# Shigangli/Ok-Topk

Measured on NVIDIA H100. Metric: train_samples_per_sec_vgg16_oktopk_density0.001, higher is better.
Workload: dtype fp32

## Files before the change

oktopk_b200/config.py:

```python
from __future__ import annotations

import dataclasses
from dataclasses import dataclass, field
from typing import Dict, Optional, Sequence


@dataclass
class OkTopkConfig:
    compressor: str = "oktopk"
    density: float = 0.01
    sparse: bool = True

    bucket_elems: int = 64 * 1024 * 1024

    warmup_iters: int = 0
    local_recompute_interval: int = 32
    global_recompute_interval: int = 32
    repartition_interval: int = 64
    topkaopt_recompute_interval: int = 32

    overselect_guard_num: int = 4
    overselect_guard_den: int = 3
    overselect_guard_factor: float = 1.03
    overselect_guard_loops: int = 5
    overselect_cap: float = 0.0
    overselect_cap_factor: float = 1.19
    overselect_cap_rungs: int = 40
    local_adapt_low: float = 2.0 / 3.0
    local_adapt_high: float = 5.0 / 4.0
    local_adapt_factor: float = 1.012
    global_adapt_low: float = 2.0 / 3.0
    global_adapt_high: float = 4.0 / 3.0
    global_adapt_inc: float = 1.008
    global_adapt_dec: float = 1.008

    throttle: int = 4
    balanced_allgather: bool = False
    dsa_dense_fallback_frac: float = 1.0 / 3.0

    gaussian_low: float = 3.0 / 4.0
    gaussian_high: float = 5.0 / 4.0
    gaussian_factor: float = 1.02
    gaussian_loops: int = 20
    gaussian_mode: str = "vgg"

    sigma_scale: float = 2.5
    norm_clip: Optional[float] = None
    dynamic_densities: Optional[Sequence[float]] = None

    backend: str = "auto"
    fused: bool = True
    deterministic: bool = False
    slot_factor: float = 0.0
    gather_factor: float = 0.0
    dense_switch_density: float = 0.05
    max_redo: int = 12
    redo_factor: float = 1.5
    land_grads: bool = True
    nvls: str = "auto"
    comm_ctas: int = 0
    pull_mode: str = "tma"
    overlap: bool = True
    gselect_mode: str = "auto"
    peer_timeout_s: float = 60.0

    def k_for(self, numel: int, density: Optional[float] = None) -> int:
        d = self.density if density is None else density
        return int(numel * d)

    def replace(self, **kw) -> "OkTopkConfig":
        return dataclasses.replace(self, **kw)

    def to_dict(self) -> Dict:
        return dataclasses.asdict(self)


@dataclass(frozen=True)
class LossScale:
    init_scale: float = 2.0 ** 16
    growth_factor: float = 2.0
    backoff_factor: float = 0.5
    growth_interval: int = 2000

    def __post_init__(self):
        if not (self.init_scale > 0 and self.growth_factor >= 1 and 0 < self.backoff_factor <= 1
                and self.growth_interval >= 1):
            raise ValueError("LossScale: need init_scale > 0, growth_factor >= 1, 0 < backoff_factor <= 1, "
                             "growth_interval >= 1")

    @staticmethod
    def parse(spec) -> Optional["LossScale"]:
        if spec is None or isinstance(spec, LossScale):
            return spec
        if isinstance(spec, str) and spec.strip().lower() == "dynamic":
            return LossScale()
        return LossScale(init_scale=float(spec), growth_factor=1.0, backoff_factor=1.0)


def _vgg() -> OkTopkConfig:
    return OkTopkConfig(
        density=0.02, warmup_iters=512,
        local_recompute_interval=32, global_recompute_interval=32, repartition_interval=64,
        overselect_guard_num=4, overselect_guard_den=3, overselect_guard_loops=5,
        local_adapt_low=2 / 3, local_adapt_high=5 / 4, local_adapt_factor=1.012,
        global_adapt_low=2 / 3, global_adapt_high=4 / 3, global_adapt_inc=1.008, global_adapt_dec=1.008,
        gaussian_mode="vgg", gaussian_factor=1.02, gaussian_loops=20,
        overselect_cap=2.0,
    )


def _lstm() -> OkTopkConfig:
    return OkTopkConfig(
        density=0.02, warmup_iters=128,
        local_recompute_interval=32, global_recompute_interval=32, repartition_interval=64,
        overselect_guard_num=3, overselect_guard_den=2, overselect_guard_loops=5,
        local_adapt_low=3 / 4, local_adapt_high=5 / 4, local_adapt_factor=1.012,
        global_adapt_low=3 / 4, global_adapt_high=5 / 4, global_adapt_inc=1.01, global_adapt_dec=1.008,
        gaussian_mode="lstm", gaussian_factor=1.012, gaussian_loops=50,
        overselect_cap=2.0,
    )


def _bert() -> OkTopkConfig:
    return OkTopkConfig(
        density=0.01, warmup_iters=0,
        local_recompute_interval=128, global_recompute_interval=128, repartition_interval=64,
        overselect_guard_loops=0,
        local_adapt_low=4 / 5, local_adapt_high=5 / 4, local_adapt_factor=1.025,
        global_adapt_low=4 / 5, global_adapt_high=5 / 4, global_adapt_inc=1.036, global_adapt_dec=1.025,
        balanced_allgather=True, sigma_scale=1.0,
        gaussian_mode="bert", gaussian_factor=1.012, gaussian_loops=20,
        overselect_cap=2.0,
    )


PRESETS = {
    "vgg16": _vgg, "vgg": _vgg, "cnn": _vgg,
    "lstm_an4": _lstm, "lstman4": _lstm, "lstm": _lstm,
    "bert_base": _bert, "bert": _bert,
}


def preset(name: str, **overrides) -> OkTopkConfig:
    if name not in PRESETS:
        raise KeyError("unknown preset %r (have %s)" % (name, sorted(PRESETS)))
    return PRESETS[name]().replace(**overrides)


def sigma_scale_for_density(density: float) -> float:
    if density > 0.7:
        return 0.5
    if density > 0.05:
        return 1.5
    if density > 0.01:
        return 2.0
    return 3.0
```

oktopk_b200/csrc/bindings.cpp:

```cpp
#include <pybind11/pybind11.h>
#include <pybind11/stl.h>
#include <cuda.h>
#include <cuda_runtime.h>

#include <unistd.h>

#include <algorithm>
#include <cstring>
#include <stdexcept>
#include <string>
#include <tuple>
#include <vector>

#include "oktopk.cuh"

namespace py = pybind11;
using namespace okt;

static void ck(cudaError_t e, const char* what) {
    if (e != cudaSuccess) throw std::runtime_error(std::string(what) + ": " + cudaGetErrorString(e));
}
template <class T> static T* P_(uint64_t p) { return reinterpret_cast<T*>(p); }
static cudaStream_t S_(uint64_t s) { return reinterpret_cast<cudaStream_t>(s); }

static py::tuple symm_alloc(size_t nbytes) {
    void* p = nullptr;
    ck(cudaMalloc(&p, nbytes), "cudaMalloc(symm)");
    ck(cudaMemset(p, 0, nbytes), "cudaMemset(symm)");
    cudaIpcMemHandle_t h;
    ck(cudaIpcGetMemHandle(&h, p), "cudaIpcGetMemHandle");
    return py::make_tuple((uint64_t)p, py::bytes(reinterpret_cast<const char*>(&h), sizeof(h)));
}
static uint64_t symm_open(const std::string& handle) {
    if (handle.size() != sizeof(cudaIpcMemHandle_t)) throw std::runtime_error("bad IPC handle size");
    cudaIpcMemHandle_t h;
    std::memcpy(&h, handle.data(), sizeof(h));
    void* p = nullptr;
    ck(cudaIpcOpenMemHandle(&p, h, cudaIpcMemLazyEnablePeerAccess), "cudaIpcOpenMemHandle");
    return (uint64_t)p;
}
static void symm_close(uint64_t p) { ck(cudaIpcCloseMemHandle(P_<void>(p)), "cudaIpcCloseMemHandle"); }
static void symm_free(uint64_t p) { ck(cudaFree(P_<void>(p)), "cudaFree(symm)"); }
static uint64_t dev_alloc_zero(size_t nbytes) {
    void* p = nullptr;
    ck(cudaMalloc(&p, nbytes), "cudaMalloc");
    ck(cudaMemset(p, 0, nbytes), "cudaMemset");
    return (uint64_t)p;
}
static void dev_free(uint64_t p) {
    if (p) ck(cudaFree(P_<void>(p)), "cudaFree");
}
static void memset_async(uint64_t p, int value, size_t nbytes, uint64_t stream) {
    ck(cudaMemsetAsync(P_<void>(p), value, nbytes, S_(stream)), "cudaMemsetAsync");
}
static int can_access_peer(int dev, int peer) {
    int ok = 0;
    ck(cudaDeviceCanAccessPeer(&ok, dev, peer), "cudaDeviceCanAccessPeer");
    return ok;
}


namespace drv {
template <class F> static F sym(const char* name) {
    void* fn = nullptr;
    cudaDriverEntryPointQueryResult q;
    cudaError_t e = cudaGetDriverEntryPoint(name, &fn, cudaEnableDefault, &q);
    if (e != cudaSuccess || fn == nullptr || q != cudaDriverEntryPointSuccess)
        throw std::runtime_error(std::string("driver entry point not available: ") + name);
    return reinterpret_cast<F>(fn);
}
static void ckd(CUresult r, const char* what) {
    if (r != CUDA_SUCCESS) throw std::runtime_error(std::string(what) + ": CUresult " + std::to_string((int)r));
}
}

static CUmemAllocationProp vmm_prop(int dev) {
    CUmemAllocationProp prop;
    std::memset(&prop, 0, sizeof(prop));
    prop.type = CU_MEM_ALLOCATION_TYPE_PINNED;
    prop.location.type = CU_MEM_LOCATION_TYPE_DEVICE;
    prop.location.id = dev;
    prop.requestedHandleTypes = CU_MEM_HANDLE_TYPE_POSIX_FILE_DESCRIPTOR;
    return prop;
}

static py::dict vmm_probe(int dev, int ndev) {
    py::dict d;
    d["vmm"] = 0; d["posix_fd"] = 0; d["multicast"] = 0; d["granularity"] = 0; d["mc_granularity"] = 0;
    try {
        auto getattr_ = drv::sym<CUresult (*)(int*, CUdevice_attribute, CUdevice)>("cuDeviceGetAttribute");
        int v = 0;
        if (getattr_(&v, CU_DEVICE_ATTRIBUTE_VIRTUAL_MEMORY_MANAGEMENT_SUPPORTED, dev) == CUDA_SUCCESS) d["vmm"] = v;
        if (getattr_(&v, CU_DEVICE_ATTRIBUTE_HANDLE_TYPE_POSIX_FILE_DESCRIPTOR_SUPPORTED, dev) == CUDA_SUCCESS) d["posix_fd"] = v;
        if (getattr_(&v, CU_DEVICE_ATTRIBUTE_MULTICAST_SUPPORTED, dev) == CUDA_SUCCESS) d["multicast"] = v;
        auto gran = drv::sym<CUresult (*)(size_t*, const CUmemAllocationProp*, CUmemAllocationGranularity_flags)>("cuMemGetAllocationGranularity");
        CUmemAllocationProp prop = vmm_prop(dev);
        size_t g = 0;
        if (gran(&g, &prop, CU_MEM_ALLOC_GRANULARITY_RECOMMENDED) == CUDA_SUCCESS) d["granularity"] = g;
        if (d["multicast"].cast<int>() && ndev > 1) {
            auto mgran = drv::sym<CUresult (*)(size_t*, const CUmulticastObjectProp*, CUmulticastGranularity_flags)>("cuMulticastGetGranularity");
            CUmulticastObjectProp mp;
            std::memset(&mp, 0, sizeof(mp));
            mp.numDevices = ndev; mp.size = 1 << 21; mp.handleTypes = CU_MEM_HANDLE_TYPE_POSIX_FILE_DESCRIPTOR;
            size_t mg = 0;
            if (mgran(&mg, &mp, CU_MULTICAST_GRANULARITY_RECOMMENDED) == CUDA_SUCCESS) d["mc_granularity"] = mg;
        }
    } catch (const std::exception& e) {
        d["error"] = std::string(e.what());
    }
    return d;
}

static py::tuple vmm_create(size_t nbytes, int dev) {
    auto create = drv::sym<CUresult (*)(CUmemGenericAllocationHandle*, size_t, const CUmemAllocationProp*, unsigned long long)>("cuMemCreate");
    auto exp = drv::sym<CUresult (*)(void*, CUmemGenericAllocationHandle, CUmemAllocationHandleType, unsigned long long)>("cuMemExportToShareableHandle");
    CUmemAllocationProp prop = vmm_prop(dev);
    CUmemGenericAllocationHandle h = 0;
    drv::ckd(create(&h, nbytes, &prop, 0), "cuMemCreate");
    int fd = -1;
    drv::ckd(exp(&fd, h, CU_MEM_HANDLE_TYPE_POSIX_FILE_DESCRIPTOR, 0), "cuMemExportToShareableHandle");
    return py::make_tuple((uint64_t)h, fd);
}
static uint64_t vmm_import(int fd) {
    auto imp = drv::sym<CUresult (*)(CUmemGenericAllocationHandle*, void*, CUmemAllocationHandleType)>("cuMemImportFromShareableHandle");
    CUmemGenericAllocationHandle h = 0;
    drv::ckd(imp(&h, reinterpret_cast<void*>(static_cast<uintptr_t>(fd)), CU_MEM_HANDLE_TYPE_POSIX_FILE_DESCRIPTOR), "cuMemImportFromShareableHandle");
    return (uint64_t)h;
}
static uint64_t vmm_map(uint64_t handle, size_t nbytes, int dev, size_t align) {
    auto reserve = drv::sym<CUresult (*)(CUdeviceptr*, size_t, size_t, CUdeviceptr, unsigned long long)>("cuMemAddressReserve");
    auto map = drv::sym<CUresult (*)(CUdeviceptr, size_t, size_t, CUmemGenericAllocationHandle, unsigned long long)>("cuMemMap");
    auto access = drv::sym<CUresult (*)(CUdeviceptr, size_t, const CUmemAccessDesc*, size_t)>("cuMemSetAccess");
    CUdeviceptr va = 0;
    drv::ckd(reserve(&va, nbytes, align, 0, 0), "cuMemAddressReserve");
    drv::ckd(map(va, nbytes, 0, (CUmemGenericAllocationHandle)handle, 0), "cuMemMap");
    CUmemAccessDesc ad;
    std::memset(&ad, 0, sizeof(ad));
    ad.location.type = CU_MEM_LOCATION_TYPE_DEVICE;
    ad.location.id = dev;
    ad.flags = CU_MEM_ACCESS_FLAGS_PROT_READWRITE;
    drv::ckd(access(va, nbytes, &ad, 1), "cuMemSetAccess");
    return (uint64_t)va;
}
static void vmm_unmap(uint64_t va, size_t nbytes) {
    auto unmap = drv::sym<CUresult (*)(CUdeviceptr, size_t)>("cuMemUnmap");
    auto afree = drv::sym<CUresult (*)(CUdeviceptr, size_t)>("cuMemAddressFree");
    unmap((CUdeviceptr)va, nbytes);
    afree((CUdeviceptr)va, nbytes);
}
static void vmm_release(uint64_t handle) {
    auto rel = drv::sym<CUresult (*)(CUmemGenericAllocationHandle)>("cuMemRelease");
    rel((CUmemGenericAllocationHandle)handle);
}
static py::tuple mc_create(size_t nbytes, int ndev) {
    auto create = drv::sym<CUresult (*)(CUmemGenericAllocationHandle*, const CUmulticastObjectProp*)>("cuMulticastCreate");
    auto exp = drv::sym<CUresult (*)(void*, CUmemGenericAllocationHandle, CUmemAllocationHandleType, unsigned long long)>("cuMemExportToShareableHandle");
    CUmulticastObjectProp mp;
    std::memset(&mp, 0, sizeof(mp));
    mp.numDevices = ndev; mp.size = nbytes; mp.handleTypes = CU_MEM_HANDLE_TYPE_POSIX_FILE_DESCRIPTOR;
    CUmemGenericAllocationHandle h = 0;
    drv::ckd(create(&h, &mp), "cuMulticastCreate");
    int fd = -1;
    drv::ckd(exp(&fd, h, CU_MEM_HANDLE_TYPE_POSIX_FILE_DESCRIPTOR, 0), "cuMemExportToShareableHandle(mc)");
    return py::make_tuple((uint64_t)h, fd);
}
static void mc_add_device(uint64_t mc, int dev) {
    auto add = drv::sym<CUresult (*)(CUmemGenericAllocationHandle, CUdevice)>("cuMulticastAddDevice");
    drv::ckd(add((CUmemGenericAllocationHandle)mc, dev), "cuMulticastAddDevice");
}
static void mc_bind(uint64_t mc, uint64_t mem, size_t nbytes) {
    auto bind = drv::sym<CUresult (*)(CUmemGenericAllocationHandle, size_t, CUmemGenericAllocationHandle, size_t, size_t, unsigned long long)>("cuMulticastBindMem");
    drv::ckd(bind((CUmemGenericAllocationHandle)mc, 0, (CUmemGenericAllocationHandle)mem, 0, nbytes, 0), "cuMulticastBindMem");
}

static size_t state_bytes() { return sizeof(OktState); }

static py::dict layout_info(int P, int n, int cap, int gcap) {
    SymmLayout L = make_layout(P, n, cap, gcap);
    py::dict d;
    d["total"] = L.total; d["rs_mbox"] = L.rs_mbox; d["rs_thr"] = L.rs_thr; d["ag_mbox"] = L.ag_mbox;
    d["cut_mbox"] = L.cut_mbox; d["cut_data"] = L.cut_data; d["send_idx"] = L.send_idx; d["send_val"] = L.send_val;
    d["gat_idx"] = L.gat_idx; d["gat_val"] = L.gat_val; d["cap"] = L.cap; d["gcap"] = L.gcap; d["scap"] = L.scap;
    d["done_mbox"] = L.done_mbox; d["tree_mbox"] = L.tree_mbox; d["scale_mbox"] = L.scale_mbox;
    d["chunk"] = kChunk; d["maxp"] = OKT_MAXP; d["threads"] = kThreads;
    return d;
}

static py::dict read_state(uint64_t st, int P, uint64_t stream) {
    static thread_local std::vector<char> host(offsetof(OktState, hist));
    ck(cudaMemcpyAsync(host.data(), P_<void>(st), host.size(), cudaMemcpyDeviceToHost, S_(stream)), "read_state");
    ck(cudaStreamSynchronize(S_(stream)), "read_state sync");
    const OktState* s = reinterpret_cast<const OktState*>(host.data());
    py::dict d;
    d["local_thr"] = s->local_thr; d["local_thr_used"] = s->local_thr_used; d["global_thr"] = s->global_thr;
    d["epoch"] = s->epoch;
    std::vector<int> e(s->edges, s->edges + P + 1);
    d["edges"] = e;
    d["local_count"] = s->stat_local_count; d["global_count"] = s->stat_global_count;
    d["recv_total"] = s->stat_recv_total; d["gather_total"] = s->stat_gather_total;
    d["overflow_send"] = s->stat_overflow_send; d["overflow_gather"] = s->stat_overflow_gather;
    d["redo"] = s->stat_redo; d["dense_fallback"] = s->stat_dense_fallback; d["pack_thr"] = s->pack_thr;
    d["cum_overflow_send"] = s->cum_overflow_send; d["cum_overflow_gather"] = s->cum_overflow_gather;
    d["cum_redo"] = s->cum_redo;
    d["fault"] = s->fault;
    auto us = [&](int a, int b) { return s->t_phase[b] >= s->t_phase[a] ? (double)(s->t_phase[b] - s->t_phase[a]) * 1e-3 : 0.0; };
    py::dict ph;
    ph["local"] = us(5, 0); ph["pack"] = us(0, 1); ph["wait_rs"] = us(1, 6); ph["reduce"] = us(6, 2); ph["gselect"] = us(2, 3);
    ph["wait_ag"] = us(3, 7); ph["final"] = us(7, 4); ph["total"] = us(5, 4);
    d["phase_us"] = ph;
    return d;
}

static py::list read_trace(uint64_t st, uint64_t stream) {
    std::vector<TraceRec> host(kTraceLen);
    ck(cudaMemcpyAsync(host.data(), reinterpret_cast<char*>(P_<OktState>(st)) + offsetof(OktState, trace),
                       sizeof(TraceRec) * kTraceLen, cudaMemcpyDeviceToHost, S_(stream)), "read_trace");
    ck(cudaStreamSynchronize(S_(stream)), "read_trace sync");
    py::list out;
    for (const TraceRec& t : host) {
        if (t.epoch == 0) continue;
        py::dict d;
        d["epoch"] = t.epoch; d["local_count"] = t.local_count; d["global_count"] = t.global_count;
        d["recv_total"] = t.recv_total; d["gather_total"] = t.gather_total; d["overflow_send"] = t.overflow_send;
        d["overflow_gather"] = t.overflow_gather; d["redo"] = t.redo; d["local_thr"] = t.local_thr;
        d["global_thr"] = t.global_thr; d["us_local"] = t.us_local; d["us_pack"] = t.us_pack;
        d["us_wait_rs"] = t.us_wait_rs; d["us_reduce"] = t.us_reduce; d["us_gselect"] = t.us_gselect;
        d["us_wait_ag"] = t.us_wait_ag; d["us_final"] = t.us_final; d["t_begin"] = t.t_begin;
        out.append(d);
    }
    return out;
}

static py::tuple host_flag_alloc() {
    int* h = nullptr;
    ck(cudaHostAlloc(reinterpret_cast<void**>(&h), sizeof(int) * 16, cudaHostAllocMapped), "cudaHostAlloc(flag)");
    for (int i = 0; i < 16; ++i) h[i] = 0;
    void* d = nullptr;
    ck(cudaHostGetDevicePointer(&d, h, 0), "cudaHostGetDevicePointer");
    return py::make_tuple((uint64_t)h, (uint64_t)d);
}
static void host_flag_free(uint64_t h) { if (h) cudaFreeHost(P_<void>(h)); }
static int host_flag_read(uint64_t h) { return h ? *reinterpret_cast<volatile int*>(h) : 0; }
static void host_flag_clear(uint64_t h) { if (h) *reinterpret_cast<volatile int*>(h) = 0; }

static void write_state(uint64_t st, float local_thr, float global_thr, const std::vector<int>& edges, uint64_t stream) {
    std::vector<char> host(offsetof(OktState, hist));
    ck(cudaMemcpyAsync(host.data(), P_<void>(st), host.size(), cudaMemcpyDeviceToHost, S_(stream)), "write_state rd");
    ck(cudaStreamSynchronize(S_(stream)), "write_state sync");
    OktState* s = reinterpret_cast<OktState*>(host.data());
    s->local_thr = local_thr;
    s->global_thr = global_thr;
    if (!edges.empty()) {
        if (edges.size() > OKT_MAXP + 1) throw std::runtime_error("too many region edges");
        for (size_t i = 0; i < edges.size(); ++i) s->edges[i] = edges[i];
    }
    ck(cudaMemcpyAsync(P_<void>(st), host.data(), host.size(), cudaMemcpyHostToDevice, S_(stream)), "write_state wr");
    ck(cudaStreamSynchronize(S_(stream)), "write_state sync2");
}

static void fill_peers(char** dst, const std::vector<uint64_t>& peers) {
    if (peers.size() > OKT_MAXP) throw std::runtime_error("world larger than OKT_MAXP");
    for (int i = 0; i < OKT_MAXP; ++i) dst[i] = nullptr;
    for (size_t i = 0; i < peers.size(); ++i) dst[i] = P_<char>(peers[i]);
}

static void oktopk_run(uint64_t g, uint64_t res, uint64_t st, const std::vector<uint64_t>& peers, int n, int rank,
                       int k, int cap, int gcap, py::dict o, int grid, uint64_t stream) {
    OktParams p;
    std::memset(&p, 0, sizeof(p));
    p.g = P_<float>(g); p.res = P_<float>(res); p.st = P_<OktState>(st);
    if (!o.contains("cand") || !o.contains("ccap")) throw std::runtime_error("oktopk_run: candidate scratch missing");
    p.cand = P_<int>(o["cand"].cast<uint64_t>()); p.ccap = o["ccap"].cast<int>();
    p.cand_mode = o.contains("cand_mode") ? o["cand_mode"].cast<int>() : 1;
    fill_peers(p.peers, peers);
    p.P = (int)peers.size(); p.rank = rank; p.n = n; p.k = k;
    p.L = make_layout(p.P, n, cap, gcap);
    auto geti = [&](const char* key, int dflt) { return o.contains(key) ? o[key].cast<int>() : dflt; };
    auto getf = [&](const char* key, double dflt) { return o.contains(key) ? o[key].cast<double>() : dflt; };
    for (int i = 0; i < OKT_MAXP; ++i) p.peer_g[i] = nullptr;
    if (o.contains("peer_g")) {
        auto pg = o["peer_g"].cast<std::vector<uint64_t>>();
        for (size_t i = 0; i < pg.size() && i < OKT_MAXP; ++i) p.peer_g[i] = P_<float>(pg[i]);
    }
    p.max_redo = geti("max_redo", 12);
    p.redo_factor = (float)getf("redo_factor", 1.5);
    p.dense_nnz_limit = geti("dense_nnz_limit", 0);
    p.host_fault = o.contains("host_fault") ? P_<int>(o["host_fault"].cast<uint64_t>()) : nullptr;
    p.skip = o.contains("skip") ? P_<const int>(o["skip"].cast<uint64_t>()) : nullptr;
    p.trace = geti("trace", 0);
    p.exact_local = geti("exact_local", 0);
    p.repartition = geti("repartition", 0);
    p.uniform_regions = geti("uniform_regions", 0);
    p.residual_mode = geti("residual_mode", RES_OKTOPK);
    p.global_mode = geti("global_mode", GLB_THRESHOLD);
    p.deterministic = geti("deterministic", 0);
    p.pull_tma = geti("pull_tma", 1);
    p.phase_begin = geti("phase_begin", 0);
    p.phase_end = geti("phase_end", PH_END);
    p.guard_loops = geti("guard_loops", 0);
    if (p.guard_loops > kGuardFineMax) p.guard_loops = kGuardFineMax;
    p.cap_limit = geti("cap_limit", 0);
    p.cap_rungs = geti("cap_rungs", 40);
    p.cap_factor = (float)getf("cap_factor", 1.19);
    p.guard_limit = geti("guard_limit", 0);
    p.guard_factor = (float)getf("guard_factor", 1.03);
    p.l_low_cnt = getf("l_low_cnt", 0.0); p.l_high_cnt = getf("l_high_cnt", 1e30);
    p.l_factor = (float)getf("l_factor", 1.012);
    p.g_low_cnt = getf("g_low_cnt", 0.0); p.g_high_cnt = getf("g_high_cnt", 1e30);
    p.g_inc = (float)getf("g_inc", 1.008); p.g_dec = (float)getf("g_dec", 1.008);
    p.prefilter = (float)getf("prefilter", 0.8);
    p.timeout_ns = (unsigned long long)(getf("timeout_s", 0.0) * 1e9);
    if (o.contains("srcs")) {
        auto t = o["srcs"].cast<std::tuple<std::vector<uint64_t>, std::vector<long long>, std::vector<long long>>>();
        const auto& ptr = std::get<0>(t);
        const auto& off = std::get<1>(t);
        const auto& len = std::get<2>(t);
        if (off.size() != ptr.size() || len.size() != ptr.size()) throw std::runtime_error("oktopk_run: srcs table size mismatch");
        if (ptr.size() > (size_t)kSrcSegMax) throw std::runtime_error("oktopk_run: more gradient sources than kSrcSegMax");
        long long end = 0;
        for (size_t i = 0; i < ptr.size(); ++i) {
            if (off[i] < end || (off[i] & 3) || len[i] <= 0 || off[i] + len[i] > n || (ptr[i] & 15))
                throw std::runtime_error("oktopk_run: gradient sources must be 16-byte aligned, in bucket order, "
                                         "non-overlapping, at offsets that are multiples of 4 elements");
            p.src[i] = P_<const float>(ptr[i]);
            p.src_off[i] = (int)off[i];
            p.src_len[i] = (int)len[i];
            end = off[i] + len[i];
        }
        p.nsrc = (int)ptr.size();
        p.zero_g = 0;
    } else {
        if (g & 15) throw std::runtime_error("oktopk_run: the bucket must be 16-byte aligned");
        p.src[0] = P_<const float>(g);
        p.src_off[0] = 0;
        p.src_len[0] = n;
        p.nsrc = 1;
        p.zero_g = 1;
    }
    if (geti("split_phases", 0)) {
        for (int ph = p.phase_begin; ph < p.phase_end; ++ph) {
            OktParams q = p;
            q.phase_begin = ph; q.phase_end = ph + 1;
            ck(launch_oktopk(q, grid, S_(stream)), "oktopk phase launch");
        }
    } else {
        ck(launch_oktopk(p, grid, S_(stream)), "oktopk fused launch");
    }
}

static void gather_run(uint64_t g, uint64_t res, uint64_t st, const std::vector<uint64_t>& peers, int n, int rank,
                       int k, int cap, int gcap, py::dict o, int grid, uint64_t stream) {
    GatherParams p;
    std::memset(&p, 0, sizeof(p));
    p.g = P_<float>(g); p.res = P_<float>(res); p.st = P_<OktState>(st);
    fill_peers(p.peers, peers);
    p.P = (int)peers.size(); p.rank = rank; p.n = n; p.k = k;
    p.L = make_layout(p.P, n, cap, gcap);
    p.reselect = o.contains("reselect") ? o["reselect"].cast<int>() : 0;
    p.clip_max_norm = o.contains("clip_max_norm") ? (float)o["clip_max_norm"].cast<double>() : 0.f;
    p.bitmap = o.contains("bitmap") ? P_<unsigned>(o["bitmap"].cast<uint64_t>()) : nullptr;
    p.cand = o.contains("cand") ? P_<int>(o["cand"].cast<uint64_t>()) : nullptr;
    p.ccap = o.contains("ccap") ? o["ccap"].cast<int>() : 0;
    p.host_fault = o.contains("host_fault") ? P_<int>(o["host_fault"].cast<uint64_t>()) : nullptr;
    p.skip = o.contains("skip") ? P_<const int>(o["skip"].cast<uint64_t>()) : nullptr;
    if (p.reselect && (p.bitmap == nullptr || p.cand == nullptr || p.ccap <= 0))
        throw std::runtime_error("gather_run: TopkA2 needs the bitmap and candidate scratch");
    p.select_mode = o["select_mode"].cast<int>();
    p.exact_now = o.contains("exact_now") ? o["exact_now"].cast<int>() : 0;
    p.gauss_mode = o.contains("gauss_mode") ? o["gauss_mode"].cast<int>() : 0;
    p.gauss_loops = o.contains("gauss_loops") ? o["gauss_loops"].cast<int>() : 20;
    p.gauss_factor = o.contains("gauss_factor") ? (float)o["gauss_factor"].cast<double>() : 1.02f;
    p.density = (float)o["density"].cast<double>();
    p.pull_tma = o.contains("pull_tma") ? o["pull_tma"].cast<int>() : 1;
    p.timeout_ns = o.contains("timeout_s") ? (unsigned long long)(o["timeout_s"].cast<double>() * 1e9) : 0ULL;
    ck(launch_gather_scheme(p, grid, S_(stream)), "gather scheme launch");
}

static void gtopk_run(uint64_t g, uint64_t res, uint64_t st, const std::vector<uint64_t>& peers, int n, int rank,
                      int k, int cap, int gcap, py::dict o, int grid, uint64_t stream) {
    TreeParams p;
    std::memset(&p, 0, sizeof(p));
    p.g = P_<float>(g); p.res = P_<float>(res); p.st = P_<OktState>(st);
    fill_peers(p.peers, peers);
    p.P = (int)peers.size(); p.rank = rank; p.n = n; p.k = k;
    if (p.P & (p.P - 1)) throw std::runtime_error("gTopk needs a power-of-two world size (VGG/allreducer.py:113)");
    p.L = make_layout(p.P, n, cap, gcap);
    p.pull_tma = o.contains("pull_tma") ? o["pull_tma"].cast<int>() : 1;
    p.timeout_ns = o.contains("timeout_s") ? (unsigned long long)(o["timeout_s"].cast<double>() * 1e9) : 0ULL;
    p.clip_max_norm = o.contains("clip_max_norm") ? (float)o["clip_max_norm"].cast<double>() : 0.f;
    p.bitmap = P_<unsigned>(o["bitmap"].cast<uint64_t>());
    p.cand = P_<int>(o["cand"].cast<uint64_t>());
    p.ccap = o["ccap"].cast<int>();
    p.sel_idx = P_<int>(o["sel_idx"].cast<uint64_t>());
    p.sel_val = P_<float>(o["sel_val"].cast<uint64_t>());
    p.selcap = o["selcap"].cast<int>();
    p.host_fault = o.contains("host_fault") ? P_<int>(o["host_fault"].cast<uint64_t>()) : nullptr;
    p.skip = o.contains("skip") ? P_<const int>(o["skip"].cast<uint64_t>()) : nullptr;
    ck(launch_gtopk(p, grid, S_(stream)), "gtopk launch");
}

static void land_grads(const std::vector<uint64_t>& srcs, const std::vector<long long>& offs, const std::vector<int>& numels,
                       uint64_t bucket, uint64_t stream) {
    const size_t T = srcs.size();
    if (offs.size() != T || numels.size() != T) throw std::runtime_error("land_grads: table size mismatch");
    constexpr int per = 8192;
    for (size_t b = 0; b < T; b += kLandMax) {
        LandParams lp;
        std::memset(&lp, 0, sizeof(lp));
        const int cnt = (int)std::min<size_t>(kLandMax, T - b);
        int blk = 0;
        for (int i = 0; i < cnt; ++i) {
            lp.src[i] = P_<const float>(srcs[b + i]);
            lp.dst_off[i] = offs[b + i];
            lp.numel[i] = numels[b + i];
            lp.blk_begin[i] = blk;
            blk += std::max(1, (numels[b + i] + per - 1) / per);
        }
        lp.blk_begin[cnt] = blk;
        lp.count = cnt;
        ck(launch_land(lp, P_<float>(bucket), S_(stream)), "land_grads");
    }
}

static void dense_run(const std::vector<uint64_t>& bufs, const std::vector<uint64_t>& flags, uint64_t epoch, int n,
                      int rank, int grid, uint64_t stream, uint64_t st, double timeout_s, uint64_t mc,
                      uint64_t host_fault, uint64_t skip) {
    DenseParams p;
    std::memset(&p, 0, sizeof(p));
    if (bufs.size() > OKT_MAXP || bufs.size() != flags.size()) throw std::runtime_error("bad peer tables");
    for (size_t i = 0; i < bufs.size(); ++i) { p.bufs[i] = P_<float>(bufs[i]); p.flags[i] = P_<uint64_t>(flags[i]); }
    p.epoch = P_<unsigned long long>(epoch);
    p.n = n; p.P = (int)bufs.size(); p.rank = rank; p.scale = 1.0f / (float)p.P;
    p.fault = st ? &P_<OktState>(st)->fault : nullptr;
    p.timeout_ns = (unsigned long long)(timeout_s * 1e9);
    p.mc = P_<float>(mc);
    p.host_fault = P_<int>(host_fault);
    p.skip = P_<const int>(skip);
    ck(launch_dense_allreduce(p, grid, S_(stream)), "dense allreduce launch");
}

static void kth_abs(uint64_t x, int n, int k, uint64_t st, uint64_t out, int grid, uint64_t stream) {
    ck(launch_kth_abs(P_<float>(x), n, k, P_<OktState>(st), P_<float>(out), grid, S_(stream)), "kth_abs launch");
}

static void fused_sgd(uint64_t p, uint64_t g, uint64_t mom, int n, double momentum, double dampening, double wd,
                      int nesterov, int first, int zero_grad, uint64_t stream, uint64_t scal_ptr, uint64_t fault_ptr,
                      uint64_t skip_ptr) {
    if (scal_ptr == 0) throw std::runtime_error("fused_sgd: scal_ptr must point at the group's device scalars");
    ck(launch_fused_sgd(P_<float>(p), P_<float>(g), P_<float>(mom), n, (float)momentum, (float)dampening, (float)wd,
                        nesterov, first, zero_grad, P_<float>(scal_ptr), P_<int>(fault_ptr), P_<int>(skip_ptr),
                        S_(stream)),
       "fused_sgd");
}
static void fused_bert_adam(uint64_t p, uint64_t g, uint64_t m, uint64_t v, int n, double b1, double b2, double eps,
                            double wd, int zero_grad, uint64_t stream, uint64_t scal_ptr, uint64_t fault_ptr,
                            uint64_t skip_ptr) {
    if (scal_ptr == 0) throw std::runtime_error("fused_bert_adam: scal_ptr must point at the group's device scalars");
    ck(launch_fused_bert_adam(P_<float>(p), P_<float>(g), P_<float>(m), P_<float>(v), n, (float)b1, (float)b2,
                              (float)eps, (float)wd, zero_grad, P_<float>(scal_ptr), P_<int>(fault_ptr), P_<int>(skip_ptr),
                              S_(stream)),
       "fused_bert_adam");
}
static void fused_adam(uint64_t p, uint64_t g, uint64_t m, uint64_t v, int n, double beta1, double beta2, double eps,
                       double wd, int decoupled, int zero_grad, uint64_t stream, uint64_t scal_ptr, uint64_t fault_ptr,
                       uint64_t skip_ptr) {
    if (scal_ptr == 0) throw std::runtime_error("fused_adam: scal_ptr must point at the group's device scalars");
    ck(launch_fused_adam(P_<float>(p), P_<float>(g), P_<float>(m), P_<float>(v), n, beta1, beta2, (float)eps, (float)wd,
                         decoupled, zero_grad, P_<float>(scal_ptr), P_<int>(fault_ptr), P_<int>(skip_ptr), S_(stream)),
       "fused_adam");
}
static BnDtype bn_dtype(int dtype, const char* what) {
    if (dtype < 0 || dtype > 2) throw std::runtime_error(std::string(what) + ": dtype must be 0 (fp32), 1 (bf16) or 2 (fp16)");
    return static_cast<BnDtype>(dtype);
}
static void bn_forward(uint64_t x, uint64_t y, uint64_t arg, uint64_t partial, uint64_t gamma, uint64_t beta, uint64_t cbias,
                       uint64_t save_mean, uint64_t save_invstd, uint64_t rmean, uint64_t rvar, uint64_t nbt, double momentum,
                       double eps, int relu, int M, int C, int W, int slot, int max_ctas, uint64_t stream, int dtype,
                       uint64_t res) {
    if (C % 4 != 0) throw std::runtime_error("bn_forward: channel count must be a multiple of 4");
    if (slot < 0) throw std::runtime_error("bn_forward: negative slot");
    if (res != 0 && (W != 0 || !relu)) throw std::runtime_error("bn_forward: a residual needs relu = 1 and no pool");
    ck(launch_bn_forward(P_<const void>(x), P_<void>(y), P_<unsigned char>(arg), P_<float>(partial), P_<const float>(gamma),
                         P_<const float>(beta), P_<const float>(cbias), P_<float>(save_mean), P_<float>(save_invstd),
                         P_<float>(rmean), P_<float>(rvar), P_<long long>(nbt), (float)momentum, (float)eps, relu, M, C, W, slot,
                         max_ctas, bn_dtype(dtype, "bn_forward"), S_(stream), P_<const void>(res)), "bn_forward");
}
static void bn_backward(uint64_t x, uint64_t dy, uint64_t arg, uint64_t dx, uint64_t partial, uint64_t gamma, uint64_t beta,
                        uint64_t save_mean, uint64_t save_invstd, uint64_t dgamma, uint64_t dbeta, int relu, int M, int C, int W,
                        int slot, int max_ctas, uint64_t stream, int dtype, uint64_t res, uint64_t dres) {
    if (slot < 0) throw std::runtime_error("bn_backward: negative slot");
    if ((res == 0) != (dres == 0)) throw std::runtime_error("bn_backward: res and dres go together");
    if (res != 0 && (W != 0 || !relu)) throw std::runtime_error("bn_backward: a residual needs relu = 1 and no pool");
    ck(launch_bn_backward(P_<const void>(x), P_<const void>(dy), P_<const unsigned char>(arg), P_<void>(dx), P_<float>(partial),
                          P_<const float>(gamma), P_<const float>(beta), P_<const float>(save_mean), P_<const float>(save_invstd),
                          P_<float>(dgamma), P_<float>(dbeta), relu, M, C, W, slot, max_ctas, bn_dtype(dtype, "bn_backward"),
                          S_(stream), P_<const void>(res), P_<void>(dres)), "bn_backward");
}
static void ln_check(const char* what, int R, int H, long long p_keep_thr, uint64_t seed, uint64_t mean, uint64_t rstd,
                     std::initializer_list<uint64_t> vec_ptrs) {
    if (R <= 0 || !ln_supported_h(H)) throw std::runtime_error(std::string(what) + ": needs R > 0 and H in 128, 256, ..., 1024");
    if (p_keep_thr < 0 || p_keep_thr > (1LL << 32)) throw std::runtime_error(std::string(what) + ": p_keep_thr out of range");
    if (p_keep_thr < (1LL << 32) && seed == 0) throw std::runtime_error(std::string(what) + ": dropout needs the seed");
    if (mean == 0 || rstd == 0) throw std::runtime_error(std::string(what) + ": mean and rstd are needed");
    for (uint64_t p : vec_ptrs)
        if (p == 0 || (p & 15)) throw std::runtime_error(std::string(what) + ": tensors must be non-null and 16-byte aligned");
}
static void ln_forward(uint64_t x, uint64_t a, uint64_t y, uint64_t gamma, uint64_t beta, uint64_t mean, uint64_t rstd,
                       uint64_t seed, int R, int H, long long p_keep_thr, double scale, double eps, int a_dtype,
                       uint64_t stream) {
    ln_check("ln_forward", R, H, p_keep_thr, seed, mean, rstd, {x, a, y, gamma, beta});
    ck(launch_ln_forward(P_<const float>(x), P_<const void>(a), P_<float>(y), P_<const float>(gamma), P_<const float>(beta),
                         P_<float>(mean), P_<float>(rstd), P_<const unsigned long long>(seed), R, H, p_keep_thr, (float)scale,
                         (float)eps, bn_dtype(a_dtype, "ln_forward"), S_(stream)), "ln_forward");
}
static void ln_backward(uint64_t x, uint64_t a, uint64_t dy, uint64_t gamma, uint64_t mean, uint64_t rstd, uint64_t seed,
                        uint64_t dx, uint64_t da, uint64_t partial, uint64_t dgamma, uint64_t dbeta, int R, int H,
                        long long p_keep_thr, double scale, int a_dtype, uint64_t stream) {
    ln_check("ln_backward", R, H, p_keep_thr, seed, mean, rstd, {x, a, dy, gamma, dx, da, partial, dgamma, dbeta});
    ck(launch_ln_backward(P_<const float>(x), P_<const void>(a), P_<const float>(dy), P_<const float>(gamma),
                          P_<const float>(mean), P_<const float>(rstd), P_<const unsigned long long>(seed), P_<float>(dx),
                          P_<void>(da), P_<float>(partial), P_<float>(dgamma), P_<float>(dbeta), R, H, p_keep_thr,
                          (float)scale, bn_dtype(a_dtype, "ln_backward"), S_(stream)), "ln_backward");
}
static void xent_check(const char* what, int R, long long V, std::initializer_list<uint64_t> ptrs, uint64_t x, uint64_t t) {
    if (R <= 0 || V <= 0) throw std::runtime_error(std::string(what) + ": needs R > 0 and V > 0");
    for (uint64_t p : ptrs)
        if (p == 0) throw std::runtime_error(std::string(what) + ": null pointer");
    if ((x & 15) || (t & 7)) throw std::runtime_error(std::string(what) + ": logits must be 16-byte aligned, targets 8-byte");
}
static void xent_forward(uint64_t x, uint64_t t, uint64_t lse, uint64_t rowloss, uint64_t loss, int R, long long V,
                         long long ignore_index, int dtype, uint64_t stream) {
    xent_check("xent_forward", R, V, {x, t, lse, rowloss, loss}, x, t);
    ck(launch_xent_forward(P_<const void>(x), P_<const long long>(t), P_<float>(lse), P_<float>(rowloss), P_<float>(loss),
                           R, V, ignore_index, bn_dtype(dtype, "xent_forward"), S_(stream)), "xent_forward");
}
static void xent_backward(uint64_t x, uint64_t t, uint64_t lse, uint64_t g, uint64_t dx, int R, long long V,
                          long long ignore_index, int dtype, uint64_t stream) {
    xent_check("xent_backward", R, V, {x, t, lse, g, dx}, x, t);
    if (dx & 15) throw std::runtime_error("xent_backward: the gradient must be 16-byte aligned");
    ck(launch_xent_backward(P_<const void>(x), P_<const long long>(t), P_<const float>(lse), P_<const float>(g), P_<void>(dx),
                            R, V, ignore_index, bn_dtype(dtype, "xent_backward"), S_(stream)), "xent_backward");
}
static void mlm_select(uint64_t labels, uint64_t rows, uint64_t tgt, uint64_t slot, uint64_t count, uint64_t overflow,
                       int R, int M, long long ignore_index, uint64_t stream) {
    if (R <= 0 || M <= 0) throw std::runtime_error("mlm_select: needs R > 0 and M > 0");
    if (!labels || !rows || !tgt || !slot || !count) throw std::runtime_error("mlm_select: null pointer");
    if ((labels & 7) || (tgt & 7) || (count & 7) || (overflow & 7) || (rows & 3) || (slot & 3))
        throw std::runtime_error("mlm_select: misaligned pointer");
    ck(launch_mlm_select(P_<const long long>(labels), R, ignore_index, M, P_<int>(rows), P_<long long>(tgt),
                         P_<int>(slot), P_<long long>(count), P_<long long>(overflow), S_(stream)), "mlm_select");
}
static void mlm_copy_check(const char* what, int nrows, int H, uint64_t src, uint64_t idx, uint64_t dst, BnDtype dt) {
    if (nrows <= 0 || H <= 0) throw std::runtime_error(std::string(what) + ": needs rows > 0 and H > 0");
    if (!src || !idx || !dst) throw std::runtime_error(std::string(what) + ": null pointer");
    const uint64_t mask = dt == BnDtype::kF32 ? 3 : 1;
    if ((src & mask) || (dst & mask) || (idx & 3)) throw std::runtime_error(std::string(what) + ": misaligned pointer");
}
static void mlm_gather(uint64_t x, uint64_t rows, uint64_t out, int M, int H, int dtype, uint64_t stream) {
    const BnDtype dt = bn_dtype(dtype, "mlm_gather");
    mlm_copy_check("mlm_gather", M, H, x, rows, out, dt);
    ck(launch_mlm_gather(P_<const void>(x), P_<const int>(rows), P_<void>(out), M, H, dt, S_(stream)), "mlm_gather");
}
static void mlm_scatter(uint64_t dout, uint64_t slot, uint64_t dx, int R, int H, int dtype, uint64_t stream) {
    const BnDtype dt = bn_dtype(dtype, "mlm_scatter");
    mlm_copy_check("mlm_scatter", R, H, dout, slot, dx, dt);
    ck(launch_mlm_scatter(P_<const void>(dout), P_<const int>(slot), P_<void>(dx), R, H, dt, S_(stream)), "mlm_scatter");
}
static void lstm_check(const char* what, int T, int N, int H, int u, int rows, BnDtype dtype,
                       std::initializer_list<uint64_t> ptrs, std::initializer_list<uint64_t> vec_ptrs) {
    if (T <= 0 || N <= 0 || H <= 0 || H % 4 || u <= 0 || rows <= 0 || rows > N)
        throw std::runtime_error(std::string(what) + ": needs T, N > 0, H > 0 a multiple of 4, u > 0 and 0 < rows <= N");
    for (uint64_t p : ptrs)
        if (p == 0) throw std::runtime_error(std::string(what) + ": null pointer");
    const uint64_t mask = dtype == BnDtype::kF32 ? 15 : 7;
    for (uint64_t p : vec_ptrs)
        if (p & mask)
            throw std::runtime_error(std::string(what) + ": W_hh and the staged operand must be " +
                                     std::to_string(mask + 1) + "-byte aligned");
}
static void lstm_forward(uint64_t gx, uint64_t whh, uint64_t len, uint64_t y, uint64_t gates, uint64_t cs, uint64_t bar,
                         int T, int N, int H, int u, int rows, uint64_t stream, int dtype) {
    const BnDtype dt = bn_dtype(dtype, "lstm_forward");
    lstm_check("lstm_forward", T, N, H, u, rows, dt, {gx, whh, len, y, gates, cs, bar}, {whh, y});
    ck(launch_lstm_forward(P_<const void>(gx), P_<const void>(whh), P_<const int>(len), P_<void>(y), P_<float>(gates),
                           P_<float>(cs), P_<unsigned long long>(bar), T, N, H, u, rows, S_(stream), dt), "lstm_forward");
}
static void lstm_backward(uint64_t dy, uint64_t gates, uint64_t cs, uint64_t whh, uint64_t len, uint64_t dg, uint64_t bar,
                          int T, int N, int H, int u, int rows, uint64_t stream, int dtype) {
    const BnDtype dt = bn_dtype(dtype, "lstm_backward");
    lstm_check("lstm_backward", T, N, H, u, rows, dt, {dy, gates, cs, whh, len, dg, bar}, {dg});
    ck(launch_lstm_backward(P_<const void>(dy), P_<const float>(gates), P_<const float>(cs), P_<const void>(whh),
                            P_<const int>(len), P_<void>(dg), P_<unsigned long long>(bar), T, N, H, u, rows, S_(stream), dt),
       "lstm_backward");
}
static void maxpool2_fwd(uint64_t x, uint64_t y, uint64_t arg, int N, int H, int W, int C, uint64_t stream) {
    if ((C % 4) || (H % 2) || (W % 2)) throw std::runtime_error("maxpool2_fwd: needs C % 4 == 0 and even H, W");
    ck(launch_maxpool2_fwd(P_<const float>(x), P_<float>(y), P_<unsigned char>(arg), N, H, W, C, S_(stream)), "maxpool2_fwd");
}
static void maxpool2_bwd(uint64_t dy, uint64_t arg, uint64_t dx, int N, int H, int W, int C, uint64_t stream) {
    ck(launch_maxpool2_bwd(P_<const float>(dy), P_<const unsigned char>(arg), P_<float>(dx), N, H, W, C, S_(stream)), "maxpool2_bwd");
}
static void momentum_correct(uint64_t g, uint64_t buf, int n, double momentum, uint64_t stream) {
    ck(launch_momentum_correct(P_<float>(g), P_<float>(buf), n, (float)momentum, S_(stream)), "momentum_correct");
}
static void clip_by_norm(uint64_t x, int n, uint64_t scratch, double max_norm, uint64_t stream) {
    ck(launch_l2norm_sq(P_<float>(x), n, P_<float>(scratch), S_(stream)), "l2norm");
    ck(launch_scale(P_<float>(x), n, P_<float>(scratch), (float)max_norm, S_(stream)), "clip scale");
}

static void unscale_check(const std::vector<uint64_t>& srcs, const std::vector<long long>& lens, uint64_t ls, uint64_t sync,
                          uint64_t st, uint64_t host_fault, const std::vector<uint64_t>& peers, size_t mbox_off, int rank,
                          double timeout_s, uint64_t stream) {
    ScaleParams p;
    std::memset(&p, 0, sizeof(p));
    if (srcs.empty() || srcs.size() != lens.size()) throw std::runtime_error("unscale_check: bad source table");
    if (srcs.size() > (size_t)kSrcSegMax) throw std::runtime_error("unscale_check: more gradient sources than kSrcSegMax");
    if (peers.size() > OKT_MAXP) throw std::runtime_error("world larger than OKT_MAXP");
    int blk = 0;
    for (size_t i = 0; i < srcs.size(); ++i) {
        if ((srcs[i] & 15) || lens[i] <= 0 || lens[i] > (1LL << 31) - 1)
            throw std::runtime_error("unscale_check: sources must be 16-byte aligned and non-empty");
        p.src[i] = P_<float>(srcs[i]);
        p.len[i] = (int)lens[i];
        p.blk_begin[i] = blk;
        blk += (int)((lens[i] + kScalePerCta - 1) / kScalePerCta);
    }
    p.blk_begin[srcs.size()] = blk;
    p.nseg = (int)srcs.size();
    p.ls = P_<LossScaleDev>(ls);
    p.sync = P_<ScaleSync>(sync);
    p.fault = &P_<OktState>(st)->fault;
    p.host_fault = P_<int>(host_fault);
    for (size_t i = 0; i < peers.size(); ++i) p.peers[i] = P_<char>(peers[i]);
    p.mbox_off = mbox_off;
    p.P = (int)peers.size(); p.rank = rank;
    p.timeout_ns = (unsigned long long)(timeout_s * 1e9);
    ck(launch_unscale_check(p, S_(stream)), "unscale_check");
}

PYBIND11_MODULE(_C, m) {
    m.doc() = "oktopk_b200 native extension (sm_90a kernels + symmetric peer memory)";
    m.def("symm_alloc", &symm_alloc);
    m.def("symm_open", &symm_open);
    m.def("symm_close", &symm_close);
    m.def("symm_free", &symm_free);
    m.def("dev_alloc_zero", &dev_alloc_zero);
    m.def("dev_free", &dev_free);
    m.def("memset_async", &memset_async);
    m.def("can_access_peer", &can_access_peer);
    m.def("state_bytes", &state_bytes);
    m.def("layout_info", &layout_info);
    m.def("read_state", &read_state);
    m.def("write_state", &write_state);
    m.def("max_coop_grid", &okt_max_coop_grid);
    m.def("oktopk_run", &oktopk_run);
    m.def("gather_run", &gather_run);
    m.def("dense_run", &dense_run, py::arg("bufs"), py::arg("flags"), py::arg("epoch"), py::arg("n"), py::arg("rank"),
          py::arg("grid"), py::arg("stream"), py::arg("st") = 0, py::arg("timeout_s") = 0.0, py::arg("mc") = 0,
          py::arg("host_fault") = 0, py::arg("skip") = 0);
    m.def("gtopk_run", &gtopk_run);
    m.def("land_grads", &land_grads);
    m.def("read_trace", &read_trace);
    m.def("host_flag_alloc", &host_flag_alloc);
    m.def("host_flag_free", &host_flag_free);
    m.def("host_flag_read", &host_flag_read);
    m.def("host_flag_clear", &host_flag_clear);
    m.def("fault_ptr", [](uint64_t st) { return (uint64_t)&P_<OktState>(st)->fault; });
    m.def("gather_max_coop_grid", &gather_max_coop_grid);
    m.def("gtopk_max_coop_grid", &gtopk_max_coop_grid);
    m.def("vmm_probe", &vmm_probe);
    m.def("vmm_create", &vmm_create);
    m.def("vmm_import", &vmm_import);
    m.def("vmm_map", &vmm_map);
    m.def("vmm_unmap", &vmm_unmap);
    m.def("vmm_release", &vmm_release);
    m.def("mc_create", &mc_create);
    m.def("mc_add_device", &mc_add_device);
    m.def("mc_bind", &mc_bind);
    m.def("close_fd", [](int fd) { if (fd >= 0) ::close(fd); });
    m.def("clear_fault", [](uint64_t st, uint64_t stream) {
        ck(cudaMemsetAsync(&P_<OktState>(st)->fault, 0, sizeof(int), S_(stream)), "clear_fault");
    });
    m.def("kth_abs", &kth_abs);
    m.def("fused_sgd", &fused_sgd, py::arg("p"), py::arg("g"), py::arg("mom"), py::arg("n"), py::arg("momentum"),
          py::arg("dampening"), py::arg("wd"), py::arg("nesterov"), py::arg("first"), py::arg("zero_grad"),
          py::arg("stream"), py::arg("scal_ptr"), py::arg("fault_ptr") = 0, py::arg("skip_ptr") = 0);
    m.def("fused_bert_adam", &fused_bert_adam, py::arg("p"), py::arg("g"), py::arg("m"), py::arg("v"), py::arg("n"),
          py::arg("b1"), py::arg("b2"), py::arg("eps"), py::arg("wd"), py::arg("zero_grad"), py::arg("stream"),
          py::arg("scal_ptr"), py::arg("fault_ptr") = 0, py::arg("skip_ptr") = 0);
    m.def("fused_adam", &fused_adam, py::arg("p"), py::arg("g"), py::arg("m"), py::arg("v"), py::arg("n"),
          py::arg("beta1"), py::arg("beta2"), py::arg("eps"), py::arg("wd"), py::arg("decoupled"), py::arg("zero_grad"),
          py::arg("stream"), py::arg("scal_ptr"), py::arg("fault_ptr") = 0, py::arg("skip_ptr") = 0);
    m.def("momentum_correct", &momentum_correct);
    m.def("unscale_check", &unscale_check);
    m.def("scale_update", [](uint64_t ls, double growth, double backoff, int interval, uint64_t stream) {
        ck(launch_scale_update(P_<LossScaleDev>(ls), growth, backoff, interval, S_(stream)), "scale_update");
    });
    m.def("adam_scalars", [](uint64_t ls, uint64_t hyper, uint64_t scal, int groups, uint64_t stream) {
        ck(launch_adam_scalars(P_<const LossScaleDev>(ls), P_<const double>(hyper), P_<float>(scal), groups, S_(stream)),
           "adam_scalars");
    });
    m.def("carry_residual", [](uint64_t g, uint64_t res, int n, uint64_t skip, uint64_t stream) {
        ck(launch_carry_residual(P_<float>(g), P_<float>(res), n, P_<const int>(skip), S_(stream)), "carry_residual");
    });
    m.attr("LOSS_SCALE_BYTES") = sizeof(LossScaleDev);
    m.attr("SCALE_SYNC_BYTES") = sizeof(ScaleSync);
    m.attr("VERDICT_OFFSET") = offsetof(ScaleSync, verdict);
    m.def("maxpool2_fwd", &maxpool2_fwd);
    m.def("maxpool2_bwd", &maxpool2_bwd);
    m.def("bn_forward", &bn_forward, py::arg("x"), py::arg("y"), py::arg("arg"), py::arg("partial"), py::arg("gamma"),
          py::arg("beta"), py::arg("cbias"), py::arg("save_mean"), py::arg("save_invstd"), py::arg("rmean"), py::arg("rvar"),
          py::arg("nbt"), py::arg("momentum"), py::arg("eps"), py::arg("relu"), py::arg("M"), py::arg("C"), py::arg("W"),
          py::arg("slot"), py::arg("max_ctas"), py::arg("stream"), py::arg("dtype"), py::arg("res") = 0);
    m.def("bn_backward", &bn_backward, py::arg("x"), py::arg("dy"), py::arg("arg"), py::arg("dx"), py::arg("partial"),
          py::arg("gamma"), py::arg("beta"), py::arg("save_mean"), py::arg("save_invstd"), py::arg("dgamma"), py::arg("dbeta"),
          py::arg("relu"), py::arg("M"), py::arg("C"), py::arg("W"), py::arg("slot"), py::arg("max_ctas"), py::arg("stream"),
          py::arg("dtype"), py::arg("res") = 0, py::arg("dres") = 0);
    m.def("bn_tile_rows", &bn_tile_rows);
    m.def("bn_sliced", &bn_sliced, py::arg("M"), py::arg("C"), py::arg("W"));
    m.def("ln_forward", &ln_forward, py::arg("x"), py::arg("a"), py::arg("y"), py::arg("gamma"), py::arg("beta"),
          py::arg("mean"), py::arg("rstd"), py::arg("seed"), py::arg("R"), py::arg("H"), py::arg("p_keep_thr"),
          py::arg("scale"), py::arg("eps"), py::arg("a_dtype"), py::arg("stream"));
    m.def("ln_backward", &ln_backward, py::arg("x"), py::arg("a"), py::arg("dy"), py::arg("gamma"), py::arg("mean"),
          py::arg("rstd"), py::arg("seed"), py::arg("dx"), py::arg("da"), py::arg("partial"), py::arg("dgamma"),
          py::arg("dbeta"), py::arg("R"), py::arg("H"), py::arg("p_keep_thr"), py::arg("scale"), py::arg("a_dtype"),
          py::arg("stream"));
    m.def("ln_bwd_grid", &ln_bwd_grid);
    m.def("ln_supported_h", &ln_supported_h);
    m.def("xent_forward", &xent_forward, py::arg("x"), py::arg("t"), py::arg("lse"), py::arg("rowloss"), py::arg("loss"),
          py::arg("R"), py::arg("V"), py::arg("ignore_index"), py::arg("dtype"), py::arg("stream"));
    m.def("xent_backward", &xent_backward, py::arg("x"), py::arg("t"), py::arg("lse"), py::arg("g"), py::arg("dx"),
          py::arg("R"), py::arg("V"), py::arg("ignore_index"), py::arg("dtype"), py::arg("stream"));
    m.def("mlm_select", &mlm_select, py::arg("labels"), py::arg("rows"), py::arg("tgt"), py::arg("slot"), py::arg("count"),
          py::arg("overflow"), py::arg("R"), py::arg("M"), py::arg("ignore_index"), py::arg("stream"));
    m.def("mlm_gather", &mlm_gather, py::arg("x"), py::arg("rows"), py::arg("out"), py::arg("M"), py::arg("H"),
          py::arg("dtype"), py::arg("stream"));
    m.def("mlm_scatter", &mlm_scatter, py::arg("dout"), py::arg("slot"), py::arg("dx"), py::arg("R"), py::arg("H"),
          py::arg("dtype"), py::arg("stream"));
    m.def("lstm_forward", &lstm_forward, py::arg("gx"), py::arg("whh"), py::arg("len"), py::arg("y"), py::arg("gates"),
          py::arg("cs"), py::arg("bar"), py::arg("T"), py::arg("N"), py::arg("H"), py::arg("u"), py::arg("rows"),
          py::arg("stream"), py::arg("dtype") = 0);
    m.def("lstm_backward", &lstm_backward, py::arg("dy"), py::arg("gates"), py::arg("cs"), py::arg("whh"), py::arg("len"),
          py::arg("dg"), py::arg("bar"), py::arg("T"), py::arg("N"), py::arg("H"), py::arg("u"), py::arg("rows"),
          py::arg("stream"), py::arg("dtype") = 0);
    m.def("clip_by_norm", &clip_by_norm);
    m.attr("MAXP") = OKT_MAXP;
    m.attr("TRACE_LEN") = kTraceLen;
    m.attr("LAND_MAX") = kLandMax;
    m.attr("SRC_SEG_MAX") = kSrcSegMax;
    m.attr("CHUNK") = kChunk;
}
```

oktopk_b200/csrc/oktopk.cu:

```cuda
#include "devlib.cuh"

namespace okt {

__device__ __forceinline__ int region_of(const int* s_edges, int P, int i) {
    int d = 0;
#pragma unroll 1
    for (int r = 1; r < P; ++r) d += (i >= s_edges[r]) ? 1 : 0;
    return d;
}

struct SrcSeg { const float* src; int off, len; };

__device__ __forceinline__ int seg_find(const SrcSeg* s, int ns, int e) {
    int lo = 0, hi = ns - 1, r = -1;
    while (lo <= hi) {
        const int mid = (lo + hi) >> 1;
        if (s[mid].off <= e) { r = mid; lo = mid + 1; } else { hi = mid - 1; }
    }
    return r;
}

__device__ __forceinline__ float grad_at(const SrcSeg* s, int ns, int i) {
    const int q = seg_find(s, ns, i);
    return (q >= 0 && i - s[q].off < s[q].len) ? s[q].src[i - s[q].off] : 0.f;
}

__device__ __forceinline__ float4 grad4_at(const SrcSeg* s, int ns, int v) {
    float4 out = make_float4(0.f, 0.f, 0.f, 0.f);
    const int q = seg_find(s, ns, 4 * v);
    if (q < 0) return out;
    const int r = 4 * v - s[q].off, len = s[q].len;
    const float* src = s[q].src + r;
    if (r + 4 <= len) return ld_stream_f4(reinterpret_cast<const float4*>(src));
    if (r < len) out.x = src[0];
    if (r + 1 < len) out.y = src[1];
    if (r + 2 < len) out.z = src[2];
    return out;
}

__global__ void __launch_bounds__(kThreads, kCtasPerSm) oktopk_fused_kernel(const OktParams p) {
    __shared__ uint32_t s_hist[kHistBins];
    __shared__ int s_w[kWarps + 1];
    __shared__ int s_edges[OKT_MAXP + 1];
    __shared__ int s_cnt[OKT_MAXP];
    __shared__ float s_thr[OKT_MAXP];
    __shared__ int s_misc[OKT_MAXP * 2 + 4];
    __shared__ int s_soff[OKT_MAXP + 1];
    __shared__ float s_lthr[kGuardMax];
    __shared__ int s_lcnt[kGuardMax];
    __shared__ ChunkSrc s_srcs[OKT_MAXP];
    __shared__ float s_sthr[OKT_MAXP];
    __shared__ Seg s_segs[OKT_MAXP];
    __shared__ __align__(128) PullSmem s_pull;
    __shared__ __align__(8) uint64_t s_pk_bar[kPackStages];
    __shared__ __align__(8) uint64_t s_pk_empty[kPackStages];
    __shared__ __align__(8) uint64_t s_sc_bar[kScanStages];
    __shared__ SrcSeg s_src[kSrcSegMax];
    __shared__ int s_tail_v[kSrcSegMax], s_tail_q[kSrcSegMax];
    __shared__ int s_ntail;
    extern __shared__ __align__(128) float4 dyn_pk[];

    if (verdict_set(p.skip)) return;
    OktState* st = p.st;
    const int tid = threadIdx.x, lane = tid & 31, warp = tid >> 5;
    const int gtid = blockIdx.x * kThreads + tid;
    const int gthreads = gridDim.x * kThreads;
    const int P = p.P, rank = p.rank, n = p.n;
    char* me = p.peers[rank];
    const uint32_t epoch = st->epoch + 1u;
    const int par = epoch & 1u;
    const float thr_in = st->local_thr;
    const bool exact_local = p.exact_local || thr_in == 0.f;
    const bool two_pass = exact_local || p.repartition;
    uint32_t pipe_it = 0;

    for (int b = tid; b < kHistBins; b += kThreads) s_hist[b] = 0;
    if (blockIdx.x == 0 && tid == 0) st->t_phase[5] = globaltimer_ns();
    const SpinGuard sg_rs{&st->fault, p.timeout_ns, FAULT_RS_TIMEOUT, p.host_fault};
    const SpinGuard sg_ag{&st->fault, p.timeout_ns, FAULT_AG_TIMEOUT, p.host_fault};
    const SpinGuard sg_cut{&st->fault, p.timeout_ns, FAULT_CUT_TIMEOUT, p.host_fault};
    const SpinGuard sg_done{&st->fault, p.timeout_ns, FAULT_DONE_TIMEOUT, p.host_fault};
    if (tid == 0) {
        mbar_init(&s_pull.bar[0], 1);
        mbar_init(&s_pull.bar[1], 1);
        for (int q = 0; q < kPackStages; ++q) { mbar_init(&s_pk_bar[q], 1); mbar_init(&s_pk_empty[q], kWarps); }
        for (int q = 0; q < kScanStages; ++q) mbar_init(&s_sc_bar[q], 1);
        mbar_fence_init();
    }
    const int n4 = n >> 2;
    const int nsrc = p.nsrc;
    for (int q = tid; q < nsrc; q += kThreads) s_src[q] = SrcSeg{p.src[q], p.src_off[q], p.src_len[q]};
    if (warp == 0) {
        int cnt = 0;
        for (int q0 = 0; q0 < nsrc; q0 += 32) {
            const int q = q0 + lane;
            const int end = q < nsrc ? p.src_off[q] + p.src_len[q] : 0;
            const bool part = q < nsrc && (end & 3) != 0 && (end >> 2) < n4;
            const unsigned m = __ballot_sync(0xffffffffu, part);
            if (part) { const int t = cnt + __popc(m & ((1u << lane) - 1u)); s_tail_v[t] = end >> 2; s_tail_q[t] = q; }
            cnt += __popc(m);
        }
        if (lane == 0) s_ntail = cnt;
    }
    __syncthreads();
    const int ntail = s_ntail;

    float4* g4 = reinterpret_cast<float4*>(p.g);
    float4* r4 = reinterpret_cast<float4*>(p.res);

    if (p.phase_begin <= PH_LOCAL && PH_LOCAL < p.phase_end && two_pass) {
        const float thr0 = thr_in;
        const LadderCfg lcl = ladder_cfg(p, !exact_local);
        ladder_build(s_lthr, s_lcnt, lcl, thr0);

        auto visit = [&](float x) {
            if (exact_local) {
                hist_add(s_hist, x, 0, 0u);
            } else {
                float ax = fabsf(x);
                if (ax > thr0) atomicAdd(&s_lcnt[ladder_rung(s_lthr, lcl.n_total, ax)], 1);
            }
        };
        const float cut = (exact_local && thr0 > 0.f) ? thr0 * p.prefilter : -1.f;
        const bool prefilter = cut > 0.f;
        constexpr int kLocTile = 4;
        for (int base = blockIdx.x * kThreads * kLocTile; base < n4; base += gridDim.x * kThreads * kLocTile) {
            float4 a[kLocTile], r[kLocTile];
            bool in[kLocTile];
#pragma unroll
            for (int u = 0; u < kLocTile; ++u) {
                const int v = base + u * kThreads + tid;
                in[u] = v < n4;
                if (in[u]) { a[u] = grad4_at(s_src, nsrc, v); r[u] = ld_stream_f4(r4 + v); }
                else { a[u] = make_float4(0.f, 0.f, 0.f, 0.f); r[u] = a[u]; }
            }
#pragma unroll
            for (int u = 0; u < kLocTile; ++u) {
                const int v = base + u * kThreads + tid;
                a[u].x += r[u].x; a[u].y += r[u].y; a[u].z += r[u].z; a[u].w += r[u].w;
                if (in[u]) st_stream_f4(r4 + v, a[u]);
                const float xs[4] = {a[u].x, a[u].y, a[u].z, a[u].w};
                if (!prefilter) {
                    if (in[u]) { visit(xs[0]); visit(xs[1]); visit(xs[2]); visit(xs[3]); }
                    continue;
                }
                unsigned bits = 0u;
                int tot = 0;
#pragma unroll
                for (int c = 0; c < 4; ++c) {
                    const bool pd = in[u] && fabsf(xs[c]) > cut;
                    if (pd) bits |= 1u << c;
                    tot += __popc(__ballot_sync(0xffffffffu, pd));
                }
                if (tot == 0) continue;
                int run = 0;
                if (lane == 0) run = atomicAdd(&st->cand_cursor, tot);
                run = __shfl_sync(0xffffffffu, run, 0);
#pragma unroll
                for (int c = 0; c < 4; ++c) {
                    const bool pd = (bits >> c) & 1u;
                    const unsigned m = __ballot_sync(0xffffffffu, pd);
                    if (pd) {
                        const int pos = run + __popc(m & ((1u << lane) - 1u));
                        if (pos < p.ccap) p.cand[pos] = 4 * v + c;
                    }
                    run += __popc(m);
                }
            }
        }
        if (blockIdx.x == 0) {
            for (int i = n4 * 4 + tid; i < n; i += kThreads) {
                float a = grad_at(s_src, nsrc, i) + p.res[i];
                p.res[i] = a;
                if (prefilter) {
                    if (fabsf(a) > cut) { int pos = atomicAdd(&st->cand_cursor, 1); if (pos < p.ccap) p.cand[pos] = i; }
                } else {
                    visit(a);
                }
            }
        }
        if (exact_local) {
            float thr;
            bool done = false;
            if (prefilter) {
                grid_sync(&st->bar);
                const int ncand = *reinterpret_cast<volatile int*>(&st->cand_cursor);
                if (ncand >= p.k && ncand <= p.ccap) {
                    Seg seg{p.res, ncand, p.cand};
                    thr = grid_kth_abs(&seg, 1, false, (uint32_t)p.k, st, s_hist, s_w, 0);
                    done = true;
                }
            }
            if (!done) {
                if (!prefilter) hist_flush(st, s_hist);
                Seg seg{p.res, n, nullptr};
                thr = grid_kth_abs(&seg, 1, false, (uint32_t)p.k, st, s_hist, s_w, prefilter ? 0 : 1);
            }
            if (blockIdx.x == 0 && tid == 0) { st->local_thr_used = thr; st->cand_cursor = 0; }
        } else {
            ladder_flush(st, s_lcnt);
            grid_sync(&st->bar);
            if (blockIdx.x == 0 && tid == 0) {
                int cnt;
                st->local_thr_used = ladder_pick(st, lcl, thr0, p.guard_limit, p.cap_limit, &cnt);
            }
        }
        grid_sync(&st->bar);

        if (p.repartition) {
            const float thr = st->local_thr_used;
            const int W = gridDim.x * kWarps;
            const int Lw = (((n + W - 1) / W) + 31) / 32 * 32;
            {
                const int gw = blockIdx.x * kWarps + warp;
                const long long lo = (long long)gw * Lw;
                const long long hi = min((long long)n, lo + Lw);
                int cnt = 0;
                for (long long base = lo; base < hi; base += 32) {
                    long long i = base + lane;
                    float x = (i < hi) ? __ldcg(p.res + i) : 0.f;
                    cnt += __popc(__ballot_sync(0xffffffffu, fabsf(x) > thr));
                }
                if (lane == 0) st->wcounts[gw] = cnt;
            }
            grid_sync(&st->bar);
            if (blockIdx.x == 0) {
                const int per = (W + kThreads - 1) / kThreads;
                int mysum = 0;
                for (int j = 0; j < per; ++j) {
                    int w = tid * per + j;
                    if (w < W) mysum += st->wcounts[w];
                }
                int M;
                int excl = block_excl_scan(mysum, s_w, &M);
                const int chunkM = M / P;
                if (M > 0) {
                    for (int j = 1; j < P; ++j) {
                        int target = chunkM * j;
                        if (excl <= target && target < excl + mysum) {
                            int run = excl;
                            for (int q = 0; q < per; ++q) {
                                int w = tid * per + q;
                                int c = (w < W) ? st->wcounts[w] : 0;
                                if (target < run + c) { s_misc[2 * j] = w; s_misc[2 * j + 1] = target - run; break; }
                                run += c;
                            }
                        }
                    }
                }
                __syncthreads();
                if (warp >= 1 && warp < P) {
                    const int j = warp;
                    int cut;
                    if (M > 0) {
                        const int gw = s_misc[2 * j];
                        int want = s_misc[2 * j + 1];
                        const long long lo = (long long)gw * Lw;
                        const long long hi = min((long long)n, lo + Lw);
                        cut = (int)lo;
                        for (long long base = lo; base < hi; base += 32) {
                            long long i = base + lane;
                            float x = (i < hi) ? __ldcg(p.res + i) : 0.f;
                            unsigned m = __ballot_sync(0xffffffffu, fabsf(x) > thr);
                            int c = __popc(m);
                            if (want < c) { cut = (int)base + (int)__fns(m, 0, want + 1); break; }
                            want -= c;
                        }
                    } else {
                        cut = (n / P) * j;
                    }
                    if (lane == 0) st->cuts[j - 1] = cut;
                }
                __syncthreads();
                if (tid < P) {
                    int* dst = cut_data(p.peers[tid], p.L, par, rank);
                    for (int j = 0; j < P - 1; ++j) st_relaxed_sys_u32(reinterpret_cast<uint32_t*>(dst + j), (uint32_t)st->cuts[j]);
                    st_release_sys_u64(cut_mbox(p.peers[tid], p.L, par, rank), make_mail(epoch, 1u));
                }
                if (tid < P) wait_mailbox(cut_mbox(me, p.L, par, tid), epoch, sg_cut);
                __syncthreads();
                if (tid < P - 1) {
                    long long sum = 0;
                    for (int s = 0; s < P; ++s)
                        sum += (long long)ld_relaxed_sys_u32(reinterpret_cast<uint32_t*>(cut_data(me, p.L, par, s) + tid));
                    s_misc[tid] = (int)(sum / P);
                }
                __syncthreads();
                if (tid == 0) {
                    int prev = 0;
                    st->edges[0] = 0;
                    for (int j = 0; j < P - 1; ++j) {
                        int c = s_misc[j];
                        c = max(prev, min(c, n));
                        st->edges[j + 1] = c;
                        prev = c;
                    }
                    st->edges[P] = n;
                }
            }
            grid_sync(&st->bar);
        }
    }

    if (tid <= P) s_edges[tid] = st->edges[tid];
    __syncthreads();
    if (tid <= P) s_soff[tid] = (tid < P) ? slot_off(p.L, s_edges, tid) : (p.L.cap > 0 ? P * p.L.cap : slot_off(p.L, s_edges, P));
    __syncthreads();
    int* const my_sidx = send_idx_base(me, p.L);
    float* const my_sval = send_val_base(me, p.L);
    auto stamp = [&](int slot) { if (blockIdx.x == 0 && tid == 0) st->t_phase[slot] = globaltimer_ns(); };
    stamp(0);

    if (p.phase_begin <= PH_PACK && PH_PACK < p.phase_end) {
        float thr_sel = two_pass ? st->local_thr_used : thr_in;
        const bool bounded = p.L.cap > 0;
        const bool can_redo = bounded && p.residual_mode == RES_OKTOPK && p.max_redo > 0;
        float redo_f = p.redo_factor > 1.f ? p.redo_factor : 1.5f;
        int attempt = 0;
        int dropped = 0;
        if (blockIdx.x == 0 && tid == 0) { st->stat_global_count = 0; st->stat_recv_total = 0; st->stat_dense_fallback = 0; }

        float4* pk_r = dyn_pk;
        float4* pk_g = dyn_pk + kPackStages * kTileV;
        const int ntiles = (n4 + kTileV - 1) / kTileV;
        const int G = gridDim.x;
        const int nmine = (ntiles > (int)blockIdx.x) ? (ntiles - (int)blockIdx.x + G - 1) / G : 0;
        int ring_it = 0;

        while (true) {
            const bool res_only = two_pass || attempt > 0;
            const bool ladder_on = !two_pass;
            const LadderCfg lc = ladder_cfg(p, ladder_on);
            ladder_build(s_lthr, s_lcnt, lc, thr_sel);
            dropped = 0;

            auto emit = [&](int i, float x, bool inrange) {
                const float ax = fabsf(x);
                const bool pred = inrange && ax > thr_sel;
                unsigned todo = __ballot_sync(0xffffffffu, pred);
                if (todo == 0) return;
                int d = 0;
                if (pred) {
                    d = region_of(s_edges, P, i);
                    atomicAdd(&s_lcnt[lc.n_total > 1 ? ladder_rung(s_lthr, lc.n_total, ax) : 0], 1);
                }
                while (todo) {
                    const int leader = __ffs(todo) - 1;
                    const int dl = __shfl_sync(0xffffffffu, d, leader);
                    const bool mine = pred && d == dl;
                    const unsigned m = __ballot_sync(0xffffffffu, mine);
                    int base = 0;
                    if (lane == leader) base = atomicAdd(&st->send_cursor[dl], __popc(m));
                    base = __shfl_sync(0xffffffffu, base, leader);
                    if (mine) {
                        const int pos = base + __popc(m & ((1u << lane) - 1u));
                        if (pos < s_soff[dl + 1] - s_soff[dl]) {
                            my_sidx[s_soff[dl] + pos] = i - s_edges[dl];
                            my_sval[s_soff[dl] + pos] = x;
                            if (p.residual_mode != RES_OKTOPK) p.res[i] = 0.f;
                        } else {
                            dropped++;
                        }
                    }
                    todo &= ~m;
                }
            };

            auto arm = [&](int j) {
                const int tile = blockIdx.x + j * G;
                const int stg = (ring_it + j) % kPackStages;
                const uint32_t bytes = (uint32_t)min(kTileV, n4 - tile * kTileV) * 16u;
                fence_proxy_async_all();
                mbar_expect_tx(&s_pk_bar[stg], res_only ? bytes : 2u * bytes);
                tma_load_1d(pk_r + stg * kTileV, r4 + (size_t)tile * kTileV, bytes, &s_pk_bar[stg]);
                if (res_only) return;
                float4* dst = pk_g + stg * kTileV;
                const int e0 = tile * kTileV * 4, e1 = e0 + (int)(bytes >> 2);
                int lo = 0, hi = nsrc;
                while (lo < hi) {
                    const int mid = (lo + hi) >> 1;
                    if (s_src[mid].off + (s_src[mid].len & ~3) <= e0) lo = mid + 1; else hi = mid;
                }
                int q = lo, e = e0;
                while (e < e1) {
                    if (q < nsrc && s_src[q].off <= e) {
                        const int stop = min(e1, s_src[q].off + (s_src[q].len & ~3));
                        if (stop > e) {
                            tma_load_1d(dst + ((e - e0) >> 2), s_src[q].src + (e - s_src[q].off), (uint32_t)(stop - e) * 4u,
                                        &s_pk_bar[stg]);
                            e = stop;
                        }
                        ++q;
                    } else {
                        const int stop = q < nsrc ? min(e1, s_src[q].off) : e1;
                        tma_load_1d(dst + ((e - e0) >> 2), p.g + e, (uint32_t)(stop - e) * 4u, &s_pk_bar[stg]);
                        e = stop;
                    }
                }
            };
            if (tid == 0)
                for (int j = 0; j < min(nmine, kPackStages - 1); ++j) {
                    const int q = ring_it + j;
                    if (q >= kPackStages) mbar_wait(&s_pk_empty[q % kPackStages], (uint32_t)(q / kPackStages - 1) & 1u);
                    arm(j);
                }
            for (int j = 0; j < nmine; ++j) {
                if (tid == 0 && j + kPackStages - 1 < nmine) {
                    const int q = ring_it + j + kPackStages - 1;
                    if (q >= kPackStages) mbar_wait(&s_pk_empty[q % kPackStages], (uint32_t)(q / kPackStages - 1) & 1u);
                    arm(j + kPackStages - 1);
                }
                const int qj = ring_it + j;
                const int stg = qj % kPackStages;
                mbar_wait(&s_pk_bar[stg], (uint32_t)(qj / kPackStages) & 1u);
                const int base = (blockIdx.x + j * G) * kTileV;
                float4 a[kPackTile];
                bool in[kPackTile];
#pragma unroll
                for (int u = 0; u < kPackTile; ++u) {
                    const int v = base + u * kThreads + tid;
                    in[u] = v < n4;
                    a[u] = make_float4(0.f, 0.f, 0.f, 0.f);
                    if (in[u]) {
                        a[u] = pk_r[stg * kTileV + u * kThreads + tid];
                        if (!res_only) {
                            float4 gq = pk_g[stg * kTileV + u * kThreads + tid];
                            for (int t = 0; t < ntail; ++t)
                                if (s_tail_v[t] == v) {
                                    const SrcSeg sg = s_src[s_tail_q[t]];
                                    const float* src = sg.src + (sg.len & ~3);
                                    const int c = sg.len & 3;
                                    gq.x = src[0];
                                    if (c > 1) gq.y = src[1];
                                    if (c > 2) gq.z = src[2];
                                }
                            a[u].x += gq.x; a[u].y += gq.y; a[u].z += gq.z; a[u].w += gq.w;
                            st_stream_f4(r4 + v, a[u]);
                        }
                        if (attempt == 0 && p.zero_g) st_stream_f4(g4 + v, make_float4(0.f, 0.f, 0.f, 0.f));
                    }
                }
                __syncwarp();
                if (lane == 0) mbar_arrive(&s_pk_empty[stg]);
                unsigned msk[kPackTile * 4];
                unsigned mybits = 0u;
                int tot = 0;
#pragma unroll
                for (int u = 0; u < kPackTile; ++u) {
                    const float xs[4] = {a[u].x, a[u].y, a[u].z, a[u].w};
#pragma unroll
                    for (int c = 0; c < 4; ++c) {
                        const bool pred = in[u] && fabsf(xs[c]) > thr_sel;
                        if (p.residual_mode == RES_LOCAL_GE && in[u] && xs[c] != 0.f && fabsf(xs[c]) == thr_sel &&
                            atomicAdd(&st->tie_cursor, 1) < (int)__ldcg(&st->sel_krem))
                            p.res[4 * (base + u * kThreads + tid) + c] = 0.f;
                        const unsigned m = __ballot_sync(0xffffffffu, pred);
                        msk[u * 4 + c] = m;
                        tot += __popc(m);
                        if (pred) mybits |= 1u << (u * 4 + c);
                    }
                }
                if (tot == 0) continue;
                if (lc.n_total > 1) {
#pragma unroll
                    for (int u = 0; u < kPackTile; ++u) {
                        const float xs[4] = {a[u].x, a[u].y, a[u].z, a[u].w};
#pragma unroll
                        for (int c = 0; c < 4; ++c)
                            if (mybits & (1u << (u * 4 + c)))
                                atomicAdd(&s_lcnt[ladder_rung(s_lthr, lc.n_total, fabsf(xs[c]))], 1);
                    }
                } else if (lane == 0) {
                    atomicAdd(&s_lcnt[0], tot);
                }
                const int e_first = 4 * (base + (warp << 5));
                const int e_last = min(n - 1, 4 * (base + (kPackTile - 1) * kThreads + (warp << 5) + 31) + 3);
                const int dlo = region_of(s_edges, P, e_first), dhi = region_of(s_edges, P, e_last);
                for (int d = dlo; d <= dhi; ++d) {
                    unsigned md[kPackTile * 4];
                    unsigned mine = mybits;
                    int cnt = 0;
                    if (dlo == dhi) {
#pragma unroll
                        for (int q = 0; q < kPackTile * 4; ++q) { md[q] = msk[q]; cnt += __popc(md[q]); }
                    } else {
                        const int lo_d = s_edges[d], hi_d = s_edges[d + 1];
                        mine = 0u;
#pragma unroll
                        for (int u = 0; u < kPackTile; ++u) {
#pragma unroll
                            for (int c = 0; c < 4; ++c) {
                                const int i = 4 * (base + u * kThreads + tid) + c;
                                const bool pd = ((mybits >> (u * 4 + c)) & 1u) && i >= lo_d && i < hi_d;
                                md[u * 4 + c] = __ballot_sync(0xffffffffu, pd);
                                cnt += __popc(md[u * 4 + c]);
                                if (pd) mine |= 1u << (u * 4 + c);
                            }
                        }
                    }
                    if (cnt == 0) continue;
                    int run = 0;
                    if (lane == 0) run = atomicAdd(&st->send_cursor[d], cnt);
                    run = __shfl_sync(0xffffffffu, run, 0);
                    const int scap_d = s_soff[d + 1] - s_soff[d];
                    int* sidx = my_sidx + s_soff[d];
                    float* sval = my_sval + s_soff[d];
                    const int off_d = s_edges[d];
                    const unsigned lt = (1u << lane) - 1u;
#pragma unroll
                    for (int u = 0; u < kPackTile; ++u) {
                        const float xs[4] = {a[u].x, a[u].y, a[u].z, a[u].w};
#pragma unroll
                        for (int c = 0; c < 4; ++c) {
                            const int q = u * 4 + c;
                            if ((mine >> q) & 1u) {
                                const int pos = run + __popc(md[q] & lt);
                                const int i = 4 * (base + u * kThreads + tid) + c;
                                if (pos < scap_d) {
                                    sidx[pos] = i - off_d;
                                    sval[pos] = xs[c];
                                    if (p.residual_mode != RES_OKTOPK) p.res[i] = 0.f;
                                } else {
                                    dropped++;
                                }
                            }
                            run += __popc(md[q]);
                        }
                    }
                }
            }
            ring_it += nmine;
            if (blockIdx.x == 0 && warp == 0 && (n & 3)) {
                int i = n4 * 4 + lane;
                bool in = i < n;
                float a = 0.f;
                if (in) {
                    a = res_only ? p.res[i] : (grad_at(s_src, nsrc, i) + p.res[i]);
                    if (!res_only) p.res[i] = a;
                    if (p.zero_g) p.g[i] = 0.f;
                }
                emit(i, a, in);
            }
            if (p.residual_mode == RES_LOCAL_GE && blockIdx.x == 0 && (n & 3)) {
                for (int i = n4 * 4 + tid; i < n; i += kThreads) {
                    float x = p.res[i];
                    if (x != 0.f && fabsf(x) == thr_sel && atomicAdd(&st->tie_cursor, 1) < (int)__ldcg(&st->sel_krem))
                        p.res[i] = 0.f;
                }
            }
            ladder_flush(st, s_lcnt);
            if (!can_redo) break;
            grid_sync(&st->bar);
            bool over = false;
            for (int d = 0; d < P; ++d) over = over || (__ldcg(&st->send_cursor[d]) > s_soff[d + 1] - s_soff[d]);
            if (!over || attempt >= p.max_redo) break;
            grid_sync(&st->bar);
            if (blockIdx.x == 0 && tid == 0) {
                for (int d = 0; d < P; ++d) st->send_cursor[d] = 0;
                for (int q = 0; q < kGuardMax; ++q) st->guard_counts[q] = 0;
                st->cum_redo += 1ULL;
            }
            thr_sel = fmaxf(thr_sel, 1e-30f) * redo_f;
            redo_f = fminf(redo_f * redo_f, 1e6f);
            ++attempt;
            grid_sync(&st->bar);
        }
        {
            int dsum = warp_sum(dropped);
            if (lane == 0 && dsum) atomicAdd(&st->cum_overflow_send, (unsigned long long)dsum);
        }
        const bool publisher = can_redo ? (blockIdx.x == 0) : last_cta_ticket(&st->tick[0]);
        if (publisher) {
            if (tid == 0) {
                int cnt;
                const float t = ladder_pick(st, ladder_cfg(p, !two_pass), thr_sel, p.guard_limit, p.cap_limit, &cnt);
                st->local_thr_used = t;
                st->pack_thr = thr_sel;
                st->stat_local_count = cnt;
                st->tie_cursor = 0;
                float nt = t;
                if ((double)cnt < p.l_low_cnt) nt = t / p.l_factor;
                else if ((double)cnt > p.l_high_cnt) nt = t * p.l_factor;
                st->local_thr = nt;
                s_thr[0] = t;
                __threadfence();
            }
            __syncthreads();
            if (tid < P) {
                const int c = min(__ldcg(&st->send_cursor[tid]), s_soff[tid + 1] - s_soff[tid]);
                st_relaxed_sys_u32(reinterpret_cast<uint32_t*>(rs_thr(p.peers[tid], p.L, par, rank)), __float_as_uint(s_thr[0]));
                st_release_sys_u64(rs_mbox(p.peers[tid], p.L, par, rank), make_mail(epoch, (uint32_t)c));
            }
            __syncthreads();
        }
        stamp(1);
    }

    if (p.phase_begin <= PH_REDUCE && PH_REDUCE < p.phase_end) {
        if (tid < P) {
            s_cnt[tid] = (int)wait_mailbox(rs_mbox(me, p.L, par, tid), epoch, sg_rs);
            s_thr[tid] = __uint_as_float(ld_relaxed_sys_u32(reinterpret_cast<uint32_t*>(rs_thr(me, p.L, par, tid))));
        }
        __syncthreads();
        stamp(6);
        const int off_me = s_edges[rank];
        const int len_me = s_edges[rank + 1] - off_me;
        float* greg = p.g + off_me;
        int pulled = 0;
        auto add = [&](int s_local, int idx, float val, const float* thr_of) {
            const bool ok = fabsf(val) > thr_of[s_local] && (unsigned)idx < (unsigned)len_me;
            if (p.cand_mode) {
                float old = 1.f;
                if (ok) old = atomicAdd(greg + idx, val);
                const bool first = ok && old == 0.f;
                const int pos = warp_append_active(&st->cand_cursor, first);
                if (first && pos < p.ccap) p.cand[pos] = idx;
            } else if (ok) {
                red_add_f32(greg + idx, val);
            }
            pulled++;
        };
        const int my_soff = s_soff[rank];
        if (!p.deterministic) {
            if (tid < P) {
                const int s = (rank + tid) % P;
                s_srcs[tid].idx = send_idx_base(p.peers[s], p.L) + my_soff;
                s_srcs[tid].val = send_val_base(p.peers[s], p.L) + my_soff;
                s_srcs[tid].count = s_cnt[s];
                s_sthr[tid] = s_thr[s];
            }
            __syncthreads();
            pull_chunks(s_srcs, P, p.pull_tma != 0, &s_pull, pipe_it,
                        [&](int sl, int idx, float val) { add(sl, idx, val, s_sthr); });
        } else {
            for (int s = 0; s < P; ++s) {
                ChunkSrc src{send_idx_base(p.peers[s], p.L) + my_soff, send_val_base(p.peers[s], p.L) + my_soff, s_cnt[s]};
                float thr1 = s_thr[s];
                pull_chunks(&src, 1, p.pull_tma != 0, &s_pull, pipe_it,
                            [&](int, int idx, float val) { add(0, idx, val, &thr1); });
                grid_sync(&st->bar);
            }
        }
        int psum = warp_sum(pulled);
        if (lane == 0 && psum) atomicAdd(&st->stat_recv_total, psum);
        if (PH_REDUCE + 1 < p.phase_end) grid_sync(&st->bar);
        stamp(2);
    }

    if (p.phase_begin <= PH_GSELECT && PH_GSELECT < p.phase_end) {
        const float gthr = st->global_thr;
        const int lo = s_edges[rank], hi = s_edges[rank + 1];
        const int gcap = p.L.gcap;
        int* gi = gat_idx(me, p.L, par);
        float* gv = gat_val(me, p.L, par);
        const bool keep_in_place = p.global_mode == GLB_ALL_NONZERO;
        int dropped = 0;
        if (p.cand_mode) {
            const int ncand = min(*reinterpret_cast<volatile int*>(&st->cand_cursor), p.ccap);
            const int ncr = (ncand + 31) / 32 * 32;
            for (int c = gtid; c < ncr; c += gthreads) {
                const bool in = c < ncand;
                const int i = in ? __ldcg(p.cand + c) : 0;
                const float v = in ? (keep_in_place ? __ldcg(p.g + lo + i) : atomicExch(p.g + lo + i, 0.f)) : 0.f;
                const bool nz = in && v != 0.f;
                const bool sel = (p.global_mode == GLB_THRESHOLD) ? (nz && fabsf(v) > gthr) : nz;
                const int pos = warp_append(&st->gather_cursor, sel);
                if (sel) {
                    if (pos < gcap) { gi[pos] = lo + i; gv[pos] = v; }
                    else { dropped++; if (keep_in_place) p.g[lo + i] = 0.f; }
                }
            }
        } else {
            auto visit1 = [&](int i, bool in) {
                const float v = in ? __ldcg(p.g + i) : 0.f;
                const bool nz = in && v != 0.f;
                const bool sel = (p.global_mode == GLB_THRESHOLD) ? (nz && fabsf(v) > gthr) : nz;
                const int pos = warp_append(&st->gather_cursor, sel);
                bool lost = false;
                if (sel) {
                    if (pos < gcap) { gi[pos] = i; gv[pos] = v; }
                    else { dropped++; lost = true; }
                }
                if (nz && (!keep_in_place || lost)) p.g[i] = 0.f;
            };
            const int first = min(hi, (lo + 3) & ~3), last = max(first, hi & ~3);
            if (blockIdx.x == 0 && warp == 0) {
                visit1(lo + lane, lo + lane < first);
                visit1(last + lane, last + lane < hi);
            }
            const int nv = (last - first) >> 2;
            const float4* gv4 = reinterpret_cast<const float4*>(p.g + first);
            tma_stream_tiles<kScanStages>(gv4, nv, dyn_pk, s_sc_bar, [&](const float4* tile, int q0) {
                float4 a[kPackTile];
                unsigned nzbits = 0u, selbits = 0u, lostbits = 0u;
                int tot = 0;
#pragma unroll
                for (int u = 0; u < kPackTile; ++u) {
                    const bool in = q0 + u * kThreads + tid < nv;
                    a[u] = in ? tile[u * kThreads + tid] : make_float4(0.f, 0.f, 0.f, 0.f);
                    const float xs[4] = {a[u].x, a[u].y, a[u].z, a[u].w};
#pragma unroll
                    for (int c = 0; c < 4; ++c) {
                        const bool nz = in && xs[c] != 0.f;
                        const bool sel = (p.global_mode == GLB_THRESHOLD) ? (nz && fabsf(xs[c]) > gthr) : nz;
                        if (nz) nzbits |= 1u << (u * 4 + c);
                        if (sel) selbits |= 1u << (u * 4 + c);
                        tot += __popc(__ballot_sync(0xffffffffu, sel));
                    }
                }
                if (__ballot_sync(0xffffffffu, nzbits != 0u) == 0u) return;
                int run = 0;
                if (tot != 0) {
                    if (lane == 0) run = atomicAdd(&st->gather_cursor, tot);
                    run = __shfl_sync(0xffffffffu, run, 0);
                }
                const unsigned lt = (1u << lane) - 1u;
#pragma unroll
                for (int u = 0; u < kPackTile; ++u) {
                    const float xs[4] = {a[u].x, a[u].y, a[u].z, a[u].w};
#pragma unroll
                    for (int c = 0; c < 4; ++c) {
                        const bool sel = (selbits >> (u * 4 + c)) & 1u;
                        const unsigned m = __ballot_sync(0xffffffffu, sel);
                        if (sel) {
                            const int pos = run + __popc(m & lt);
                            if (pos < gcap) {
                                gi[pos] = first + 4 * (q0 + u * kThreads + tid) + c;
                                gv[pos] = xs[c];
                            } else {
                                dropped++;
                                lostbits |= 1u << (u * 4 + c);
                            }
                        }
                        run += __popc(m);
                    }
                    if (!keep_in_place) {
                        if ((nzbits >> (u * 4)) & 0xfu)
                            *reinterpret_cast<float4*>(p.g + first + 4 * (q0 + u * kThreads + tid)) = make_float4(0.f, 0.f, 0.f, 0.f);
                    } else if ((lostbits >> (u * 4)) & 0xfu) {
#pragma unroll
                        for (int c = 0; c < 4; ++c)
                            if ((lostbits >> (u * 4 + c)) & 1u) p.g[first + 4 * (q0 + u * kThreads + tid) + c] = 0.f;
                    }
                }
            });
        }
        int dsum = warp_sum(dropped);
        if (lane == 0 && dsum) atomicAdd(&st->cum_overflow_gather, (unsigned long long)dsum);
        stamp(3);
        if (last_cta_ticket(&st->tick[1])) {
            if (tid == 0) s_misc[0] = min(__ldcg(&st->gather_cursor), p.L.gcap);
            __syncthreads();
            if (tid < P) st_release_sys_u64(ag_mbox(p.peers[tid], p.L, par, rank), make_mail(epoch, (uint32_t)s_misc[0]));
            __syncthreads();
        }
    }

    if (p.phase_begin <= PH_FINAL && PH_FINAL < p.phase_end) {
        if (tid < P) s_cnt[tid] = (int)wait_mailbox(ag_mbox(me, p.L, par, tid), epoch, sg_ag);
        __syncthreads();
        stamp(7);
        int T = 0;
        for (int s = 0; s < P; ++s) T += s_cnt[s];
        const float fP = (float)P;
        const bool dense_path = p.global_mode == GLB_ALL_NONZERO && p.dense_nnz_limit > 0 && T >= p.dense_nnz_limit &&
                                P > 1 && p.peer_g[0] != nullptr;
        int kept_cnt = 0;
        if (dense_path) {
            const float inv = 1.f / fP;
            for (int t = 1; t < P; ++t) {
                const int s = (rank + t) % P;
                const int lo_s = s_edges[s], hi_s = s_edges[s + 1];
                const float* src = p.peer_g[s];
                const int first = min(hi_s, (lo_s + 3) & ~3), last = max(first, hi_s & ~3);
                for (int i = lo_s + gtid; i < first; i += gthreads) p.g[i] = ld_peer_f32(src + i) * inv;
                for (int i = last + gtid; i < hi_s; i += gthreads) p.g[i] = ld_peer_f32(src + i) * inv;
                const int nv = (last - first) >> 2;
                const int4* s4 = reinterpret_cast<const int4*>(src + first);
                float4* d4 = reinterpret_cast<float4*>(p.g + first);
                for (int v = gtid; v < nv; v += gthreads) {
                    const int4 r = ld_peer_i4(s4 + v);
                    st_stream_f4(d4 + v, make_float4(__int_as_float(r.x) * inv, __int_as_float(r.y) * inv,
                                                     __int_as_float(r.z) * inv, __int_as_float(r.w) * inv));
                }
            }
            grid_sync(&st->bar);
            if (blockIdx.x == 0 && tid < P) st_release_sys_u64(done_mbox(p.peers[tid], p.L, par, rank), make_mail(epoch, 1u));
            if (tid < P) wait_mailbox(done_mbox(me, p.L, par, tid), epoch, sg_done);
            __syncthreads();
            const int lo = s_edges[rank], hi = s_edges[rank + 1];
            for (int i = lo + gtid; i < hi; i += gthreads) p.g[i] = __ldcg(p.g + i) * inv;
            if (blockIdx.x == 0 && tid == 0) { st->stat_dense_fallback = 1; st->stat_global_count = T; }
        } else {
            float gsel = 0.f;
            if (p.global_mode == GLB_EXACT_TOPK) {
                if (tid < P) { s_segs[tid].ptr = gat_val(p.peers[tid], p.L, par); s_segs[tid].count = s_cnt[tid]; s_segs[tid].idx = nullptr; }
                __syncthreads();
                const uint32_t kk = (uint32_t)min(T, p.k);
                gsel = (kk > 0) ? grid_kth_abs(s_segs, P, true, kk, st, s_hist, s_w, 0) : 0.f;
                if (blockIdx.x == 0 && tid == 0) st->global_thr = gsel;
            } else if (p.global_mode == GLB_THRESHOLD && blockIdx.x == 0 && tid == 0) {
                float gt = st->global_thr;
                if ((double)T < p.g_low_cnt) gt = gt / p.g_inc;
                else if ((double)T > p.g_high_cnt) gt = gt * p.g_dec;
                st->global_thr = gt;
            }
            const float thr_used = st->local_thr_used;
            if (tid < P) {
                const int s = (rank + tid) % P;
                s_srcs[tid].idx = gat_idx(p.peers[s], p.L, par);
                s_srcs[tid].val = gat_val(p.peers[s], p.L, par);
                s_srcs[tid].count = s_cnt[s];
            }
            __syncthreads();
            const bool exact = p.global_mode == GLB_EXACT_TOPK;
            pull_chunks(s_srcs, P, p.pull_tma != 0, &s_pull, pipe_it, [&](int sl, int idx, float val) {
                if ((unsigned)idx >= (unsigned)n) return;
                bool keep = exact ? (fabsf(val) >= gsel) : true;
                if (!keep) return;
                kept_cnt++;
                p.g[idx] = val / fP;
                if (p.residual_mode == RES_OKTOPK) {
                    float r = p.res[idx];
                    if (fabsf(r) > thr_used) p.res[idx] = 0.f;
                }
            });
            int ksum = warp_sum(kept_cnt);
            if (lane == 0 && ksum) atomicAdd(&st->stat_global_count, ksum);
        }
        if (last_cta_ticket(&st->tick[2]) && tid == 0) {
            const unsigned long long t_end = globaltimer_ns();
            st->epoch = epoch;
            st->t_phase[4] = t_end;
            st->stat_gather_total = T;
            for (int d = 0; d < P; ++d) st->send_cursor[d] = 0;
            st->gather_cursor = 0;
            st->cand_cursor = 0;
            const unsigned long long os = *reinterpret_cast<volatile unsigned long long*>(&st->cum_overflow_send);
            const unsigned long long og = *reinterpret_cast<volatile unsigned long long*>(&st->cum_overflow_gather);
            const unsigned long long rd = *reinterpret_cast<volatile unsigned long long*>(&st->cum_redo);
            st->stat_overflow_send = (int)min(os - st->snap_overflow_send, 0x7fffffffULL);
            st->stat_overflow_gather = (int)min(og - st->snap_overflow_gather, 0x7fffffffULL);
            st->stat_redo = (int)(rd - st->snap_redo);
            st->snap_overflow_send = os; st->snap_overflow_gather = og; st->snap_redo = rd;
            TraceRec& tr = st->trace[epoch % kTraceLen];
            auto us = [&](int a, int b) {
                const unsigned long long ta = *reinterpret_cast<volatile unsigned long long*>(&st->t_phase[a]);
                const unsigned long long tb = *reinterpret_cast<volatile unsigned long long*>(&st->t_phase[b]);
                return tb >= ta ? (float)(tb - ta) * 1e-3f : 0.f;
            };
            tr.epoch = epoch;
            tr.local_count = st->stat_local_count;
            tr.global_count = *reinterpret_cast<volatile int*>(&st->stat_global_count);
            tr.recv_total = *reinterpret_cast<volatile int*>(&st->stat_recv_total);
            tr.gather_total = T;
            tr.overflow_send = st->stat_overflow_send;
            tr.overflow_gather = st->stat_overflow_gather;
            tr.redo = st->stat_redo;
            tr.local_thr = st->local_thr_used;
            tr.global_thr = st->global_thr;
            tr.us_local = us(5, 0); tr.us_pack = us(0, 1); tr.us_wait_rs = us(1, 6); tr.us_reduce = us(6, 2);
            tr.us_gselect = us(2, 3); tr.us_wait_ag = us(3, 7); tr.us_final = us(7, 4);
            tr.t_begin = st->t_phase[5];
        }
    }
}

__global__ void __launch_bounds__(kThreads, 2) kth_abs_kernel(const float* x, int n, int k, OktState* st, float* out) {
    __shared__ uint32_t s_hist[kHistBins];
    __shared__ int s_w[kWarps + 1];
    for (int b = threadIdx.x; b < kHistBins; b += kThreads) s_hist[b] = 0;
    __syncthreads();
    Seg seg{x, n, nullptr};
    float t = grid_kth_abs(&seg, 1, false, (uint32_t)k, st, s_hist, s_w, 0);
    if (blockIdx.x == 0 && threadIdx.x == 0) *out = t;
}

int okt_max_coop_grid(int device) {
    int sms = 0, per = 0;
    cudaDeviceGetAttribute(&sms, cudaDevAttrMultiProcessorCount, device);
    cudaFuncSetAttribute(oktopk_fused_kernel, cudaFuncAttributeMaxDynamicSharedMemorySize, kPackSmemBytes);
    cudaOccupancyMaxActiveBlocksPerMultiprocessor(&per, oktopk_fused_kernel, kThreads, kPackSmemBytes);
    if (per < 1) per = 1;
    if (per > kCtasPerSm) per = kCtasPerSm;
    return sms * per;
}

cudaError_t launch_oktopk(const OktParams& p, int grid, cudaStream_t stream) {
    static bool attr_set[64] = {false};
    int dev = 0;
    cudaGetDevice(&dev);
    if (dev >= 0 && dev < 64 && !attr_set[dev]) {
        cudaError_t e = cudaFuncSetAttribute(oktopk_fused_kernel, cudaFuncAttributeMaxDynamicSharedMemorySize, kPackSmemBytes);
        if (e != cudaSuccess) return e;
        attr_set[dev] = true;
    }
    void* args[] = {(void*)&p};
    return cudaLaunchCooperativeKernel((void*)oktopk_fused_kernel, dim3(grid), dim3(kThreads), args, kPackSmemBytes, stream);
}

cudaError_t launch_kth_abs(const float* x, int n, int k, OktState* st, float* out_thr, int grid, cudaStream_t stream) {
    void* args[] = {(void*)&x, (void*)&n, (void*)&k, (void*)&st, (void*)&out_thr};
    return cudaLaunchCooperativeKernel((void*)kth_abs_kernel, dim3(grid), dim3(kThreads), args, 0, stream);
}

}
```

oktopk_b200/csrc/oktopk.cuh:

```cuda
#pragma once
#include <cuda_runtime.h>
#include <stdint.h>
#include <stddef.h>

#ifndef OKT_MAXP
#define OKT_MAXP 16
#endif

namespace okt {

constexpr int kThreads = 512;
constexpr int kWarps = kThreads / 32;
constexpr int kChunk = 1024;
constexpr int kHistBins = 2048;
constexpr int kMaxWarpsTotal = 16384;
constexpr int kGuardMax = 64;
constexpr int kGuardFineMax = 15;
constexpr int kCtasPerSm = 1;
constexpr int kPackTile = 2;
constexpr int kPackStages = 4;
constexpr int kPackSmemBytes = kPackStages * 2 * kPackTile * kThreads * 16;
constexpr int kScanStages = 2 * kPackStages;
constexpr int kStrideGridMax = 132 * 8;

constexpr int kTraceLen = 256;
struct TraceRec {
    uint32_t epoch;
    int local_count, global_count, recv_total, gather_total, overflow_send, overflow_gather, redo;
    float local_thr, global_thr;
    float us_local, us_pack, us_wait_rs, us_reduce, us_gselect, us_wait_ag, us_final;
    unsigned long long t_begin;
};

struct OktState {
    unsigned long long bar;
    unsigned int tick[4];
    float local_thr;
    float local_thr_used;
    float global_thr;
    uint32_t epoch;
    int edges[OKT_MAXP + 1];
    int send_cursor[OKT_MAXP];
    int gather_cursor;
    int cand_cursor;
    int guard_counts[kGuardMax];
    uint32_t sel_prefix;
    uint32_t sel_krem;
    int tie_cursor;
    int cuts[OKT_MAXP];
    int stat_local_count;
    int stat_global_count;
    int stat_recv_total;
    int stat_gather_total;
    int stat_overflow_send;
    int stat_overflow_gather;
    int stat_redo;
    int stat_dense_fallback;
    int stat_mode;
    int fault;
    float pack_thr;
    unsigned long long cum_overflow_send;
    unsigned long long cum_overflow_gather;
    unsigned long long cum_redo;
    unsigned long long snap_overflow_send;
    unsigned long long snap_overflow_gather;
    unsigned long long snap_redo;
    unsigned long long t_phase[8];
    double gs_sum, gs_sumsq;
    double clip_sumsq;
    uint32_t hist[kHistBins];
    int wcounts[kMaxWarpsTotal];
    TraceRec trace[kTraceLen];
};

struct SymmLayout {
    size_t rs_mbox;
    size_t rs_thr;
    size_t ag_mbox;
    size_t cut_mbox;
    size_t cut_data;
    size_t done_mbox;
    size_t tree_mbox;
    size_t scale_mbox;
    size_t send_idx;
    size_t send_val;
    size_t gat_idx;
    size_t gat_val;
    size_t total;
    int cap;
    int scap;
    int gcap;
};

inline size_t align_up(size_t x, size_t a) { return (x + a - 1) / a * a; }

inline SymmLayout make_layout(int P, int n, int cap, int gcap) {
    SymmLayout L;
    size_t o = 0;
    L.rs_mbox = o;  o += sizeof(uint64_t) * 2 * OKT_MAXP;
    L.rs_thr = o;   o += sizeof(float) * 2 * OKT_MAXP;
    L.ag_mbox = o;  o += sizeof(uint64_t) * 2 * OKT_MAXP;
    L.cut_mbox = o; o += sizeof(uint64_t) * 2 * OKT_MAXP;
    L.cut_data = o; o += sizeof(int) * 2 * OKT_MAXP * OKT_MAXP;
    L.done_mbox = o; o += sizeof(uint64_t) * 2 * OKT_MAXP;
    L.tree_mbox = o; o += sizeof(uint64_t) * 2 * OKT_MAXP;
    L.scale_mbox = o; o += sizeof(uint64_t) * 2 * OKT_MAXP;
    o = align_up(o, 1024);
    const size_t scap = cap > 0 ? (size_t)P * cap : align_up((size_t)n, 4) + 4 * (size_t)OKT_MAXP + 1024;
    L.send_idx = o; o += sizeof(int) * scap;   o = align_up(o, 1024);
    L.send_val = o; o += sizeof(float) * scap; o = align_up(o, 1024);
    L.gat_idx = o;  o += sizeof(int) * 2 * (size_t)gcap;      o = align_up(o, 1024);
    L.gat_val = o;  o += sizeof(float) * 2 * (size_t)gcap;    o = align_up(o, 1024);
    L.total = o;
    L.cap = cap;
    L.scap = (int)scap;
    L.gcap = gcap;
    return L;
}

enum Phase : int {
    PH_LOCAL = 0,
    PH_PACK = 1,
    PH_PUBLISH_RS = 2,
    PH_REDUCE = 3,
    PH_GSELECT = 4,
    PH_PUBLISH_AG = 5,
    PH_FINAL = 6,
    PH_END = 7
};

enum ResidualMode : int { RES_OKTOPK = 0, RES_LOCAL_GT = 1, RES_LOCAL_GE = 2 };
enum GlobalMode : int { GLB_THRESHOLD = 0, GLB_EXACT_TOPK = 1, GLB_ALL_NONZERO = 2 };

constexpr int kSrcSegMax = 160;

struct OktParams {
    float* g;
    float* res;
    OktState* st;
    int* cand;
    int ccap;
    int cand_mode;
    float prefilter;
    char* peers[OKT_MAXP];
    float* peer_g[OKT_MAXP];
    SymmLayout L;
    int n, P, rank, k;
    int exact_local, repartition, uniform_regions;
    int residual_mode, global_mode;
    int deterministic, pull_tma;
    int phase_begin, phase_end;
    int guard_loops, guard_limit;
    float guard_factor;
    int cap_limit, cap_rungs;
    float cap_factor;
    double l_low_cnt, l_high_cnt;
    float l_factor;
    double g_low_cnt, g_high_cnt;
    float g_inc, g_dec;
    unsigned long long timeout_ns;
    int max_redo;
    float redo_factor;
    int dense_nnz_limit;
    int* host_fault;
    const int* skip;
    int trace;
    int zero_g;
    int nsrc;
    int src_off[kSrcSegMax];
    int src_len[kSrcSegMax];
    const float* src[kSrcSegMax];
};
static_assert(sizeof(OktParams) <= 4096, "OktParams must fit the 4 KB kernel-parameter limit");

enum GatherSelect : int { GS_THRESHOLD_REUSE = 0, GS_GAUSSIAN = 1, GS_EXACT_TOPK = 2 };

struct GatherParams {
    float* g;
    float* res;
    OktState* st;
    char* peers[OKT_MAXP];
    SymmLayout L;
    int n, P, rank, k;
    int select_mode;
    int exact_now;
    int gauss_mode;
    int gauss_loops;
    float gauss_factor;
    float density;
    int pull_tma;
    unsigned long long timeout_ns;
    int reselect;
    float clip_max_norm;
    unsigned* bitmap;
    int* cand;
    int ccap;
    int* host_fault;
    const int* skip;
};

struct TreeParams {
    float* g;
    float* res;
    OktState* st;
    char* peers[OKT_MAXP];
    SymmLayout L;
    int n, P, rank, k;
    int pull_tma;
    unsigned long long timeout_ns;
    float clip_max_norm;
    unsigned* bitmap;
    int* cand;
    int ccap;
    int* sel_idx;
    float* sel_val;
    int selcap;
    int* host_fault;
    const int* skip;
};

struct DenseParams {
    float* bufs[OKT_MAXP];
    uint64_t* flags[OKT_MAXP];
    unsigned long long* epoch;
    int n, P, rank;
    float scale;
    int* fault;
    unsigned long long timeout_ns;
    float* mc;
    int* host_fault;
    const int* skip;
};

int okt_max_coop_grid(int device);
cudaError_t launch_oktopk(const OktParams& p, int grid, cudaStream_t stream);
cudaError_t launch_gather_scheme(const GatherParams& p, int grid, cudaStream_t stream);
cudaError_t launch_gtopk(const TreeParams& p, int grid, cudaStream_t stream);
int gtopk_max_coop_grid(int device);
int gather_max_coop_grid(int device);
cudaError_t launch_dense_allreduce(const DenseParams& p, int grid, cudaStream_t stream);
cudaError_t launch_kth_abs(const float* x, int n, int k, OktState* st, float* out_thr, int grid, cudaStream_t stream);
cudaError_t launch_fused_sgd(float* p, float* g, float* mom, int n, float momentum, float dampening, float weight_decay,
                             int nesterov, int first_step, int zero_grad, const float* scal, const int* fault,
                             const int* skip, cudaStream_t stream);
cudaError_t launch_fused_bert_adam(float* p, float* g, float* m, float* v, int n, float b1, float b2, float eps,
                                   float weight_decay, int zero_grad, const float* scal, const int* fault,
                                   const int* skip, cudaStream_t stream);
cudaError_t launch_fused_adam(float* p, float* g, float* m, float* v, int n, double beta1, double beta2, float eps,
                              float weight_decay, int decoupled, int zero_grad, const float* scal, const int* fault,
                              const int* skip, cudaStream_t stream);

struct LossScaleDev {
    float scale;
    float inv_scale;
    int growth_tracker;
    int found_inf;
    long long skipped;
    long long adam_step;
};
struct ScaleSync {
    int flag;
    unsigned int ticket;
    unsigned int epoch;
    int verdict;
};
constexpr int kScaleThreads = 256;
constexpr int kScalePerCta = 8192;
struct ScaleParams {
    LossScaleDev* ls;
    ScaleSync* sync;
    int* fault;
    int* host_fault;
    char* peers[OKT_MAXP];
    size_t mbox_off;
    int P, rank;
    unsigned long long timeout_ns;
    int nseg;
    int len[kSrcSegMax];
    int blk_begin[kSrcSegMax + 1];
    float* src[kSrcSegMax];
};
static_assert(sizeof(ScaleParams) <= 4096, "ScaleParams must fit the 4 KB kernel-parameter limit");
cudaError_t launch_unscale_check(const ScaleParams& p, cudaStream_t stream);
cudaError_t launch_scale_update(LossScaleDev* ls, double growth_factor, double backoff_factor, int growth_interval,
                                cudaStream_t stream);
cudaError_t launch_adam_scalars(const LossScaleDev* ls, const double* hyper, float* scal, int groups, cudaStream_t stream);
cudaError_t launch_carry_residual(float* g, float* res, int n, const int* skip, cudaStream_t stream);
constexpr int kLandMax = 96;
struct LandParams {
    const float* src[kLandMax];
    long long dst_off[kLandMax];
    int numel[kLandMax];
    int blk_begin[kLandMax + 1];
    int count;
};
cudaError_t launch_land(const LandParams& lp, float* bucket, cudaStream_t stream);
enum class BnDtype : int { kF32 = 0, kBF16 = 1, kF16 = 2 };
int bn_tile_rows(int M, int C);
bool bn_sliced(int M, int C, int W);
cudaError_t launch_bn_forward(const void* x, void* y, unsigned char* arg, float* partial, const float* gamma, const float* beta,
                              const float* cbias, float* save_mean, float* save_invstd, float* rmean, float* rvar, long long* nbt,
                              float momentum, float eps, int relu, int M, int C, int W, int slot, int max_ctas, BnDtype dtype,
                              cudaStream_t stream, const void* res = nullptr);
cudaError_t launch_bn_backward(const void* x, const void* dy, const unsigned char* arg, void* dx, float* partial,
                               const float* gamma, const float* beta, const float* save_mean, const float* save_invstd,
                               float* dgamma, float* dbeta, int relu, int M, int C, int W, int slot, int max_ctas, BnDtype dtype,
                               cudaStream_t stream, const void* res = nullptr, void* dres = nullptr);
cudaError_t launch_maxpool2_fwd(const float* x, float* y, unsigned char* arg, int N, int H, int W, int C, cudaStream_t stream);
cudaError_t launch_maxpool2_bwd(const float* dy, const unsigned char* arg, float* dx, int N, int H, int W, int C,
                                cudaStream_t stream);
bool ln_supported_h(int H);
int ln_bwd_grid(int R);
cudaError_t launch_ln_forward(const float* x, const void* a, float* y, const float* gamma, const float* beta, float* mean,
                              float* rstd, const unsigned long long* seed, int R, int H, long long keep_thr, float scale,
                              float eps, BnDtype a_dtype, cudaStream_t stream);
cudaError_t launch_ln_backward(const float* x, const void* a, const float* dy, const float* gamma, const float* mean,
                               const float* rstd, const unsigned long long* seed, float* dx, void* da, float* partial,
                               float* dgamma, float* dbeta, int R, int H, long long keep_thr, float scale, BnDtype a_dtype,
                               cudaStream_t stream);
cudaError_t launch_xent_forward(const void* x, const long long* t, float* lse, float* rowloss, float* loss, int R,
                                long long V, long long ignore_index, BnDtype dtype, cudaStream_t stream);
cudaError_t launch_xent_backward(const void* x, const long long* t, const float* lse, const float* g, void* dx, int R,
                                 long long V, long long ignore_index, BnDtype dtype, cudaStream_t stream);
cudaError_t launch_mlm_select(const long long* labels, int R, long long ignore_index, int M, int* rows, long long* tgt,
                              int* slot, long long* count, long long* overflow, cudaStream_t stream);
cudaError_t launch_mlm_gather(const void* x, const int* rows, void* out, int M, int H, BnDtype dtype, cudaStream_t stream);
cudaError_t launch_mlm_scatter(const void* dout, const int* slot, void* dx, int R, int H, BnDtype dtype,
                               cudaStream_t stream);
cudaError_t launch_lstm_forward(const void* gx, const void* whh, const int* len, void* y, float* gates, float* cs,
                                unsigned long long* bar, int T, int N, int H, int u, int rows, cudaStream_t stream,
                                BnDtype dtype);
cudaError_t launch_lstm_backward(const void* dy, const float* gates, const float* cs, const void* whh, const int* len,
                                 void* dg, unsigned long long* bar, int T, int N, int H, int u, int rows,
                                 cudaStream_t stream, BnDtype dtype);
cudaError_t launch_momentum_correct(float* g, float* buf, int n, float momentum, cudaStream_t stream);
cudaError_t launch_l2norm_sq(const float* x, int n, float* out, cudaStream_t stream);
cudaError_t launch_scale(float* x, int n, const float* norm_sq, float max_norm, cudaStream_t stream);

}
```

oktopk_b200/optimizer.py:

```python
from __future__ import annotations

import math
import warnings
from typing import Dict, Iterable, List, Optional

import torch

from .compression import NoneCompressor, compressors, resolve_compressor
from .config import LossScale, OkTopkConfig
from .ops import ext
from .parallel.allreducer import AllReducer
from .parallel.buckets import Bucket, attach, build_buckets
from .parallel.world import World, world as _world


class _ScaleState:

    def __init__(self, ls: LossScale, device: torch.device):
        self.cfg = ls
        self.buf = torch.zeros(32, dtype=torch.uint8, device=device)
        self.f32 = self.buf[0:8].view(torch.float32)
        self.i32 = self.buf[8:16].view(torch.int32)
        self.i64 = self.buf[16:32].view(torch.int64)
        self.native = device.type == "cuda" and ext.available()
        self.reset()

    @property
    def ptr(self) -> int:
        return self.buf.data_ptr()

    @property
    def found_ptr(self) -> int:
        return self.buf.data_ptr() + 12

    def reset(self, scale: Optional[float] = None, growth_tracker: int = 0, skipped: int = 0, adam_step: int = 0) -> None:
        from .parallel.oracle import inv_scale_of
        scale = self.cfg.init_scale if scale is None else scale
        vals = torch.zeros(32, dtype=torch.uint8)
        vals[0:8].view(torch.float32).copy_(torch.tensor([scale, inv_scale_of(scale)], dtype=torch.float32))
        vals[8:16].view(torch.int32).copy_(torch.tensor([growth_tracker, 0], dtype=torch.int32))
        vals[16:32].view(torch.int64).copy_(torch.tensor([skipped, adam_step], dtype=torch.int64))
        self.buf.copy_(vals)

    def scale(self) -> torch.Tensor:
        return self.f32[0]

    def state(self) -> Dict:
        h = self.buf.cpu()
        f, i, q = h[0:8].view(torch.float32), h[8:16].view(torch.int32), h[16:32].view(torch.int64)
        return {"scale": float(f[0]), "growth_tracker": int(i[0]), "skipped_steps": int(q[0]), "adam_step": int(q[1]),
                "found_inf": int(i[1])}

    def found_host(self) -> bool:
        return bool(self.i32[1].item())

    def check_host(self, flat: torch.Tensor, world: World) -> bool:
        with torch.no_grad():
            bad = (~torch.isfinite(flat)).any().to(torch.int32).reshape(1)
            flat.mul_(self.f32[1])
            world.all_reduce_sum(bad)
            skip = bool(bad.item())
            if skip:
                self.i32[1].fill_(1)
        return skip

    def update(self) -> None:
        c = self.cfg
        if self.native:
            ext.require().scale_update(self.ptr, float(c.growth_factor), float(c.backoff_factor), int(c.growth_interval),
                                       torch.cuda.current_stream().cuda_stream)
            return
        from .parallel.oracle import update_scale
        st = self.state()
        found = bool(st["found_inf"])
        scale, tracker = update_scale(st["scale"], st["growth_tracker"], found, c)
        self.reset(scale, tracker, st["skipped_steps"] + int(found), st["adam_step"] + int(not found))


class _BucketedComm:

    def _okt_setup(self, named_parameters, allreducer: AllReducer, flatten_params: bool = True,
                   loss_scale: Optional[LossScale] = None) -> None:
        if named_parameters is not None:
            named_parameters = list(named_parameters)
            if any(not isinstance(p, tuple) for p in named_parameters):
                raise ValueError("named_parameters should be a sequence of (name, parameter) tuples, "
                                 "usually produced by model.named_parameters().")
            names = {v: k for k, v in named_parameters}
        else:
            names = {}
        i = 0
        for g in self.param_groups:
            for p in g["params"]:
                if p not in names:
                    names[p] = "allreduce.noname.%d" % i
                i += 1
        self._parameter_names = names
        self._allreducer = allreducer
        self._cfg: OkTopkConfig = allreducer.cfg
        self.local = False
        self._synced = False
        self._ls: Optional[_ScaleState] = None
        self.momentum_correction = False
        self._buckets: List[Bucket] = build_buckets(self.param_groups, names, self._cfg.bucket_elems)
        self._bucket_of: Dict[torch.nn.Parameter, Bucket] = {}
        self._flat_state: Dict[int, Dict[str, torch.Tensor]] = {}
        self._next_launch = 0
        self._hook_handles = []
        self._comm_stream = None
        self._use_streams = False
        self._land = False
        for b in self._buckets:
            dev = b.params[0].device
            grad = allreducer.register_bucket(b.name, b.numel, dev)
            attach(b, grad, flatten_params)
            if dev.type == "cuda" and self._cfg.land_grads and ext.available():
                self._land = True
            b.pending = len(b.params)
            b.dirty = False
            if dev.type == "cuda":
                self._use_streams = self._cfg.overlap
                b.event = torch.cuda.Event()
            for p in b.params:
                self._bucket_of[p] = b
                self._hook_handles.append(p.register_post_accumulate_grad_hook(self._make_hook(p)))
        if self._update is _AdamUpdate:
            if not (ext.available() and all(b.flat_param is not None and b.grad.is_cuda for b in self._buckets)):
                self._update = None
        self._direct = (self._land and self._update is not None and allreducer.compressor.name == "oktopk"
                        and all(b.flat_param is not None for b in self._buckets))
        if self._use_streams:
            self._comm_stream = torch.cuda.Stream(priority=-1)
        allreducer.add_resync_hook(self._resync_replicas)
        if loss_scale is not None:
            allreducer.enable_loss_scaling()
            self._ls = _ScaleState(loss_scale, self._buckets[0].params[0].device if self._buckets else torch.device("cpu"))
        self._lr_dev = self._hyper_dev = None
        self._lr_pin, self._lr_ev, self._lr_ring, self._lr_last = [], [], 0, None
        dev0 = self._buckets[0].params[0].device if self._buckets else torch.device("cpu")
        if dev0.type == "cuda" and ext.available() and self._update is not None:
            groups = max(len(self.param_groups), 1)
            self._lr_dev = torch.zeros(groups * self._update.n_scalars, dtype=torch.float32, device=dev0)
            stage = self._lr_dev
            if self._ls is not None and self._update is _AdamUpdate:
                stage = self._hyper_dev = torch.zeros(groups * 4, dtype=torch.float64, device=dev0)
            self._lr_pin = [torch.zeros_like(stage, device="cpu").pin_memory() for _ in range(8)]
            self._lr_ev = [None] * len(self._lr_pin)

    def _resync_replicas(self) -> None:
        w = self._allreducer.world
        if w.size == 1:
            return
        for b in self._buckets:
            if b.flat_param is not None:
                w.broadcast(b.flat_param, 0)
            else:
                for p in b.params:
                    w.broadcast(p.data, 0)
            for t in self._flat_state.get(b.index, {}).values():
                if torch.is_tensor(t):
                    w.broadcast(t, 0)

    @property
    def _okt_adam(self) -> bool:
        return self._update is _AdamUpdate

    def refresh_lr(self) -> None:
        if self._lr_dev is None or self._update is None:
            return
        vals = [self._update.scalars(self, g) for g in self.param_groups]
        if vals == self._lr_last:
            return
        self._lr_ring = (self._lr_ring + 1) % len(self._lr_pin)
        pin = self._lr_pin[self._lr_ring]
        if self._lr_ev[self._lr_ring] is not None:
            self._lr_ev[self._lr_ring].synchronize()
        n = len(vals[0]) if vals else 0
        for gi, sc in enumerate(vals):
            for j, v in enumerate(sc):
                pin[gi * n + j] = v
        (self._hyper_dev if self._hyper_dev is not None else self._lr_dev).copy_(pin, non_blocking=True)
        ev = torch.cuda.Event()
        ev.record()
        self._lr_ev[self._lr_ring] = ev
        self._lr_last = vals

    def _lr_ptr(self, gi: int) -> int:
        return self._lr_dev.data_ptr() + 4 * self._update.n_scalars * gi

    def _maybe_refresh_lr(self) -> None:
        if self._lr_dev is not None and not torch.cuda.is_current_stream_capturing():
            self.refresh_lr()

    def _make_hook(self, p):
        def hook(param):
            b = self._bucket_of[p]
            b.dirty = True
            if self.local:
                return
            b.pending -= 1
            if b.pending == 0:
                self._launch_ready()
        return hook

    def _launch_ready(self) -> None:
        while self._next_launch < len(self._buckets) and self._buckets[self._next_launch].pending <= 0:
            self._launch(self._buckets[self._next_launch])
            self._next_launch += 1

    def _land_bucket(self, b: Bucket) -> None:
        srcs, offs, numels = [], [], []
        for p, o, v in zip(b.params, b.offsets, b.grad_views):
            g = p.grad
            if g is None:
                srcs.append(0)
                offs.append(o)
                numels.append(p.numel())
            elif g.data_ptr() == v.data_ptr():
                continue
            elif g.dtype == torch.float32 and g.is_cuda and g.stride() == v.stride():
                srcs.append(g.data_ptr())
                offs.append(o)
                numels.append(g.numel())
            else:
                v.copy_(g)
            p.grad = v
        if srcs:
            ext.require().land_grads(srcs, offs, numels, b.grad.data_ptr(), torch.cuda.current_stream().cuda_stream)

    def _source_table(self, b: Bucket):
        ptrs, offs, lens, held = [], [], [], []
        for p, o, v in zip(b.params, b.offsets, b.grad_views):
            g = p.grad
            if g is None or g.numel() == 0:
                continue
            if (g.data_ptr() == v.data_ptr() or g.dtype != torch.float32 or not g.is_cuda or g.stride() != v.stride()
                    or g.data_ptr() % 16):
                return None
            ptrs.append(g.data_ptr())
            offs.append(o)
            lens.append(g.numel())
            held.append(g)
        if len(ptrs) > ext.require().SRC_SEG_MAX:
            return None
        for p, v in zip(b.params, b.grad_views):
            p.grad = v
        b.held = held
        return ptrs, offs, lens

    def _launch(self, b: Bucket) -> None:
        if b.launched:
            return
        b.launched = True
        srcs = None
        if self._direct and not self.momentum_correction and self._allreducer.reads_sources(b.name):
            srcs = self._source_table(b)
        if srcs is None and self._land:
            self._land_bucket(b)
        if self.momentum_correction:
            self._apply_momentum_correction(b)
        if self._comm_stream is not None:
            ev = torch.cuda.Event()
            ev.record(torch.cuda.current_stream())
            self._comm_stream.wait_event(ev)
            with torch.cuda.stream(self._comm_stream):
                self._allreducer.reduce_bucket(b.name, b.grad, stream=self._comm_stream, srcs=srcs, scale=self._ls)
                b.event.record(self._comm_stream)
        else:
            self._allreducer.reduce_bucket(b.name, b.grad, srcs=srcs, scale=self._ls)

    def _apply_momentum_correction(self, b: Bucket) -> None:
        fs = self._flat_state.setdefault(b.index, {})
        buf = fs.get("mc_buf")
        if buf is None:
            buf = fs["mc_buf"] = torch.zeros_like(b.grad)
        if b.grad.is_cuda and ext.available():
            ext.require().momentum_correct(b.grad.data_ptr(), buf.data_ptr(), b.numel, 0.9,
                                           torch.cuda.current_stream().cuda_stream)
        else:
            buf.mul_(0.9).add_(b.grad)
            b.grad.copy_(buf)

    @property
    def momentum_correction(self) -> bool:
        return self._momentum_correction

    @momentum_correction.setter
    def momentum_correction(self, on: bool) -> None:
        if on and getattr(self, "_ls", None) is not None:
            raise ValueError("loss_scale cannot be combined with momentum_correction: the momentum buffer would absorb "
                             "the gradient of a skipped step")
        self._momentum_correction = bool(on)

    def scale_loss(self, loss: torch.Tensor) -> torch.Tensor:
        if self._ls is None:
            return loss
        return loss * self._ls.scale()

    def loss_scale_state(self) -> Optional[Dict]:
        if self._ls is None:
            return None
        st = self._ls.state()
        return {k: st[k] for k in ("scale", "growth_tracker", "skipped_steps")}

    def _scale_state_dict(self) -> Optional[Dict]:
        if self._ls is None:
            return None
        st = self._ls.state()
        st.pop("found_inf")
        return st

    def _load_scale_state(self, sd: Optional[Dict], adam_step: int) -> None:
        if self._ls is None:
            return
        if sd is None:
            self._ls.reset(adam_step=adam_step)
        else:
            self._ls.reset(sd["scale"], sd["growth_tracker"], sd["skipped_steps"], sd.get("adam_step", adam_step))

    def synchronize(self) -> None:
        if self._synced:
            return
        for b in self._buckets:
            b.pending = 0
        self._launch_ready()
        if self._comm_stream is not None:
            cur = torch.cuda.current_stream()
            for b in self._buckets:
                cur.wait_event(b.event)
        for b in self._buckets:
            b.held = None
        self._synced = True

    def _after_step(self) -> None:
        for b in self._buckets:
            b.pending = len(b.params)
            b.launched = False
        self._next_launch = 0
        self._synced = False
        self._allreducer.poll_faults()

    def _clear_buckets(self) -> None:
        if self._direct:
            with torch.no_grad():
                for b in self._buckets:
                    b.grad.zero_()

    def zero_grad(self, set_to_none: bool = False) -> None:
        if self._land:
            for b in self._buckets:
                for p in b.params:
                    p.grad = None
                b.dirty = False
            return
        for b in self._buckets:
            if b.dirty:
                b.grad.zero_()
                b.dirty = False

    def stop(self) -> None:
        self._allreducer.stop()

    def add_train_epoch(self) -> None:
        self._allreducer.train_epoch += 1

    def get_current_density(self) -> float:
        return self._allreducer.get_current_density()

    def comm_stats(self) -> Dict:
        return self._allreducer.stats()

    def check_faults(self) -> None:
        self._allreducer.check_faults()

    def close(self) -> None:
        for h in self._hook_handles:
            h.remove()
        self._hook_handles = []
        self._allreducer.close()

    def step(self, closure=None):
        loss = None
        if closure is not None:
            with torch.enable_grad():
                loss = closure()
        if not self.local:
            self.synchronize()
        host_skip = self._ls is not None and not self._device_update() and self._ls.found_host()
        if self._update is None:
            if not host_skip:
                super().step()
            for b in self._buckets:
                b.dirty = True
        else:
            self._maybe_refresh_lr()
            if self._hyper_dev is not None and self._update is _AdamUpdate:
                ext.require().adam_scalars(self._ls.ptr, self._hyper_dev.data_ptr(), self._lr_dev.data_ptr(),
                                           len(self.param_groups), torch.cuda.current_stream().cuda_stream)
            with torch.no_grad():
                for b in self._buckets:
                    self._fused_update(b, host_skip)
            self.counter += 1
        if self._ls is not None:
            self._ls.update()
        self._after_step()
        return loss

    def _device_update(self) -> bool:
        return self._update is not None and self._lr_dev is not None and all(
            b.grad.is_cuda and b.flat_param is not None for b in self._buckets)

    def _flat_buffers(self, b: Bucket) -> Dict[str, torch.Tensor]:
        fs = self._flat_state.setdefault(b.index, {})
        for k in self._update.keys:
            if k not in fs:
                fs[k] = torch.zeros_like(b.grad)
                for p, v in zip(b.params, b.views(fs[k])):
                    self.state[p][k] = v
        return fs

    def _fused_update(self, b: Bucket, host_skip: bool = False) -> None:
        first = self._update.keys[0] not in self._flat_state.get(b.index, {})
        fs = self._flat_buffers(b)
        on_gpu = b.grad.is_cuda and b.flat_param is not None and ext.available()
        zero_grad = 0 if self._land and not self._direct else 1
        skip_ptr = self._ls.found_ptr if self._ls is not None else 0
        for gi, s, e in b.group_slices:
            def launch(fn, *hyper):
                fn(b.flat_param.data_ptr() + 4 * s, b.grad.data_ptr() + 4 * s,
                   *(fs[k].data_ptr() + 4 * s for k in self._update.keys), e - s, *hyper, zero_grad,
                   torch.cuda.current_stream().cuda_stream, self._lr_ptr(gi), self._allreducer.fault_ptr(b.name),
                   skip_ptr)
            if on_gpu or not host_skip:
                self._update.update(self, b, self.param_groups[gi], s, e, fs, first, launch if on_gpu else None)
            if not on_gpu:
                b.grad[s:e].zero_()
        b.dirty = False

    def _adopt_state(self, counter: Optional[int] = None) -> None:
        keys = self._update.keys
        have = {p for b in self._buckets for p in b.params if self.state.get(p, {}).get(keys[0]) is not None}
        if counter is None:
            steps = {float(self.state[p]["step"]) for p in have if "step" in self.state[p]}
            if len(steps) > 1:
                warnings.warn("DistributedOptimizer: the loaded Adam state has unequal step counts per parameter %s; "
                              "using torch's Adam step from now on" % sorted(steps))
                self._update = None
                self._clear_buckets()
                self._direct = False
                for b in self._buckets:
                    for k in keys:
                        self._flat_state.get(b.index, {}).pop(k, None)
                return
            counter = int(steps.pop()) if steps else 0
        self.counter = counter
        loaded = {(p, k): self.state[p][k] for p in have for k in keys}
        with torch.no_grad():
            for b in self._buckets:
                for p in b.params:
                    self.state.get(p, {}).pop("step", None)
                if not any(p in have for p in b.params):
                    for k in keys:
                        self._flat_state.get(b.index, {}).pop(k, None)
                    continue
                fs = self._flat_buffers(b)
                for k in keys:
                    for p, v in zip(b.params, b.views(fs[k])):
                        if p in have:
                            v.copy_(loaded[p, k])
                        else:
                            v.zero_()
                        self.state[p][k] = v


class _SGDUpdate:
    keys = ("momentum_buffer",)
    n_scalars = 1

    @staticmethod
    def scalars(opt, g):
        return (float(g["lr"]),)

    @staticmethod
    def update(opt, b, g, s, e, fs, first, launch):
        lr, m, damp, wd, nest = g["lr"], g.get("momentum", 0.0), g.get("dampening", 0.0), \
            g.get("weight_decay", 0.0), bool(g.get("nesterov", False))
        if opt.momentum_correction:
            m = 0.0
        if launch is not None:
            launch(ext.require().fused_sgd, m, damp, wd, int(nest), int(first))
            return
        gs, ms = b.grad[s:e], fs["momentum_buffer"][s:e]
        if b.flat_param is not None:
            _SGDUpdate.math(b.flat_param[s:e], gs, ms, lr, m, damp, wd, nest, first)
        else:
            for p, o in zip(b.params, b.offsets):
                if s <= o < e:
                    _SGDUpdate.math(p.data.view(-1), gs[o - s:o - s + p.numel()], ms[o - s:o - s + p.numel()],
                                    lr, m, damp, wd, nest, first)

    @staticmethod
    def math(p, g, mom, lr, m, damp, wd, nest, first) -> None:
        d = g.add(p, alpha=wd) if wd != 0 else g.clone()
        if m != 0:
            if first:
                mom.copy_(d)
            else:
                mom.mul_(m).add_(d, alpha=1 - damp)
            d = d.add(mom, alpha=m) if nest else mom
        p.add_(d, alpha=-lr)


class _AdamUpdate:
    keys = ("exp_avg", "exp_avg_sq")
    n_scalars = 3

    @staticmethod
    def scalars(opt, g):
        if opt._hyper_dev is not None:
            return (float(g["lr"]), float(g["weight_decay"]), float(g["betas"][0]), float(g["betas"][1]))
        lr, (b1, b2), t = float(g["lr"]), g["betas"], float(opt.counter + 1)
        return (1 - lr * g["weight_decay"], (lr / (1 - b1 ** t)) * -1, (1 - b2 ** t) ** 0.5)

    @staticmethod
    def update(opt, b, g, s, e, fs, first, launch):
        launch(ext.require().fused_adam, g["betas"][0], g["betas"][1], g["eps"], g["weight_decay"],
               int(bool(g["decoupled_weight_decay"])))


class _BertAdamUpdate:
    keys = ("next_m", "next_v")
    n_scalars = 1

    @staticmethod
    def scalars(opt, g):
        return (float(opt._scheduled_lr(g, opt.counter)),)

    @staticmethod
    def update(opt, b, g, s, e, fs, first, launch):
        if opt.clip_reduced and g["max_grad_norm"] > 0:
            for p, o in zip(b.params, b.offsets):
                if s <= o < e:
                    gv = b.grad[o:o + p.numel()]
                    nrm = float(gv.norm())
                    if nrm > g["max_grad_norm"]:
                        gv.mul_(g["max_grad_norm"] / (nrm + 1e-6))
        if launch is not None:
            launch(ext.require().fused_bert_adam, g["b1"], g["b2"], g["e"], g["weight_decay"])
            return
        lr = opt._scheduled_lr(g, opt.counter)
        gs, ms, vs = b.grad[s:e], fs["next_m"][s:e], fs["next_v"][s:e]
        ms.mul_(g["b1"]).add_(gs, alpha=1 - g["b1"])
        vs.mul_(g["b2"]).addcmul_(gs, gs, value=1 - g["b2"])
        upd = ms / (vs.sqrt() + g["e"])
        if b.flat_param is not None:
            ps = b.flat_param[s:e]
            if g["weight_decay"] > 0.0:
                upd += g["weight_decay"] * ps
            ps.add_(upd, alpha=-lr)
        else:
            for p, o in zip(b.params, b.offsets):
                if s <= o < e:
                    u = upd[o - s:o - s + p.numel()].view_as(p)
                    if g["weight_decay"] > 0.0:
                        u = u + g["weight_decay"] * p.data
                    p.data.add_(u, alpha=-lr)


class _DistributedOptimizerMixin(_BucketedComm):
    def state_dict(self):
        sd = super().state_dict()
        scale = self._scale_state_dict()
        if self._update is _AdamUpdate:
            params = [p for g in self.param_groups for p in g["params"]]
            steps = scale["adam_step"] if scale is not None else self.counter
            for i, st in list(sd["state"].items()):
                sd["state"][i] = dict(st, step=torch.tensor(float(steps), dtype=torch.float32, device=params[i].device))
        sd["oktopk"] = self._allreducer.state_dict()
        if scale is not None:
            sd["loss_scale"] = scale
        return sd

    def load_state_dict(self, state_dict):
        state_dict = dict(state_dict)
        okt = state_dict.pop("oktopk", None)
        scale = state_dict.pop("loss_scale", None)
        super().load_state_dict(state_dict)
        if self._update is not None:
            self._adopt_state()
        self._load_scale_state(scale, getattr(self, "counter", 0))
        if okt is not None:
            self._allreducer.load_state_dict(okt)
        self._clear_buckets()


def DistributedOptimizer(optimizer: torch.optim.Optimizer, named_parameters=None, compression=NoneCompressor,
                         is_sparse: bool = False, err_handler=None, layerwise_times=None, sigma_scale: float = 2.5,
                         density: float = 0.1, norm_clip: Optional[float] = None, writer=None,
                         cfg: Optional[OkTopkConfig] = None, world: Optional[World] = None,
                         backend: Optional[str] = None, flatten_params: bool = True,
                         loss_scale: Optional[LossScale] = None):
    base_cls = optimizer.__class__
    cls = type(base_cls.__name__, (_DistributedOptimizerMixin, base_cls), {})
    obj = cls.__new__(cls)
    base_cls.__init__(obj, optimizer.param_groups)
    obj.state.update(optimizer.state)
    ar = AllReducer(compression=compression, sparse=is_sparse, density=density, cfg=cfg, world=world,
                    backend=backend, err_callback=err_handler, layerwise_times=layerwise_times,
                    sigma_scale=sigma_scale, norm_clip=norm_clip, writer=writer)
    if isinstance(optimizer, torch.optim.SGD):
        obj._update = _SGDUpdate
    elif _fused_adam_applies(optimizer):
        obj._update = _AdamUpdate
    else:
        obj._update = None
    if obj._update is not None:
        obj.counter = 0
    obj._okt_setup(named_parameters, ar, flatten_params=flatten_params, loss_scale=loss_scale)
    if obj._update is not None and obj.state:
        obj._adopt_state()
        obj._load_scale_state(None, obj.counter)
    return obj


def _fused_adam_applies(opt: torch.optim.Optimizer) -> bool:
    if not isinstance(opt, torch.optim.Adam):
        return False
    for g in opt.param_groups:
        if g.get("fused") is not True or g.get("amsgrad") or g.get("maximize") or g.get("differentiable"):
            return False
        if torch.is_tensor(g["lr"]) or any(torch.is_tensor(b) for b in g["betas"]):
            return False
        if any(not p.is_cuda or p.dtype != torch.float32 for p in g["params"]):
            return False
    return True


def rank() -> int:
    return _world().rank


def size() -> int:
    return _world().size


def broadcast_parameters(model_or_params, root_rank: int = 0, world: Optional[World] = None) -> None:
    w = world or _world()
    if w.size == 1:
        return
    if isinstance(model_or_params, torch.nn.Module):
        tensors = list(model_or_params.state_dict().values())
    else:
        tensors = [p.data if isinstance(p, torch.nn.Parameter) else p for p in model_or_params]
    for t in tensors:
        if torch.is_tensor(t):
            w.broadcast(t, root_rank)
    w.barrier()


def warmup_cosine(x, warmup=0.002):
    if x < warmup:
        return x / warmup
    return 0.5 * (1.0 + math.cos(math.pi * x))


def warmup_constant(x, warmup=0.002):
    if x < warmup:
        return x / warmup
    return 1.0


def warmup_linear(x, warmup=0.002):
    if x < warmup:
        return x / warmup
    return max((x - 1.0) / (warmup - 1.0), 0.0)


def warmup_poly(x, warmup=0.002, degree=0.5):
    if x < warmup:
        return x / warmup
    return (1.0 - x) ** degree


SCHEDULES = {
    "warmup_cosine": warmup_cosine,
    "warmup_constant": warmup_constant,
    "warmup_linear": warmup_linear,
    "warmup_poly": warmup_poly,
}


class BertAdam(_BucketedComm, torch.optim.Optimizer):

    def __init__(self, params, lr=1e-3, warmup=-1, t_total=-1, schedule="warmup_linear", b1=0.9, b2=0.999, e=1e-6,
                 weight_decay=0.01, max_grad_norm=1.0, density=1.0, compressor="none", rank=-1, named_parameters=None,
                 cfg: Optional[OkTopkConfig] = None, world: Optional[World] = None, backend: Optional[str] = None,
                 clip_reduced: bool = False, flatten_params: bool = True, loss_scale: Optional[LossScale] = None,
                 **_ignored):
        if lr < 0.0:
            raise ValueError("Invalid learning rate: {} - should be >= 0.0".format(lr))
        if schedule not in SCHEDULES:
            raise ValueError("Invalid schedule parameter: {}".format(schedule))
        if not 0.0 <= warmup < 1.0 and not warmup == -1:
            raise ValueError("Invalid warmup: {} - should be in [0.0, 1.0[ or -1".format(warmup))
        if not 0.0 <= b1 < 1.0 or not 0.0 <= b2 < 1.0 or not e >= 0.0:
            raise ValueError("Invalid Adam hyper-parameters")
        defaults = dict(lr=lr, schedule=schedule, warmup=warmup, t_total=t_total, b1=b1, b2=b2, e=e,
                        weight_decay=weight_decay, max_grad_norm=max_grad_norm)
        torch.optim.Optimizer.__init__(self, params, defaults)
        self.rank = rank
        self.counter = 0
        self.clip_reduced = clip_reduced
        self._update = _BertAdamUpdate
        base = cfg if cfg is not None else OkTopkConfig(
            warmup_iters=0, local_recompute_interval=128, global_recompute_interval=128, overselect_guard_loops=0,
            local_adapt_low=4 / 5, local_adapt_high=5 / 4, local_adapt_factor=1.025, global_adapt_low=4 / 5,
            global_adapt_high=5 / 4, global_adapt_inc=1.036, global_adapt_dec=1.025, balanced_allgather=True)
        ar = AllReducer(compression=compressor, sparse=(compressor != "none"), density=density,
                        cfg=base.replace(density=density), world=world, backend=backend)
        self._okt_setup(named_parameters, ar, flatten_params=flatten_params, loss_scale=loss_scale)

    def get_lr(self) -> List[float]:
        out = []
        for g in self.param_groups:
            out.append(self._scheduled_lr(g, self.counter))
        return out if self.counter > 0 else [0]

    @staticmethod
    def _scheduled_lr(g: dict, step: int) -> float:
        if g["t_total"] != -1:
            return g["lr"] * SCHEDULES[g["schedule"]](step / g["t_total"], g["warmup"])
        return g["lr"]

    def state_dict(self):
        sd = torch.optim.Optimizer.state_dict(self)
        for i, st in list(sd["state"].items()):
            sd["state"][i] = dict(st, step=self.counter)
        sd["oktopk"] = self._allreducer.state_dict()
        sd["counter"] = self.counter
        scale = self._scale_state_dict()
        if scale is not None:
            sd["loss_scale"] = scale
        return sd

    def load_state_dict(self, state_dict):
        state_dict = dict(state_dict)
        okt = state_dict.pop("oktopk", None)
        counter = state_dict.pop("counter", 0)
        scale = state_dict.pop("loss_scale", None)
        torch.optim.Optimizer.load_state_dict(self, state_dict)
        self._adopt_state(counter)
        self._load_scale_state(scale, counter)
        if okt is not None:
            self._allreducer.load_state_dict(okt)
        self._clear_buckets()
```

oktopk_b200/parallel/allreducer.py:

```python
from __future__ import annotations

import time
from typing import Dict, Optional

import torch

from ..compression import Compressor, resolve_compressor
from ..config import OkTopkConfig
from ..ops import ext
from . import algorithms
from .state import SparseState
from .world import World, world as _world


def _capturing() -> bool:
    return torch.cuda.is_available() and torch.cuda.is_current_stream_capturing()


class AllReducer:
    def __init__(self, compression="oktopk", sparse: bool = True, density: float = 0.01, train_epoch: int = 0,
                 cfg: Optional[OkTopkConfig] = None, world: Optional[World] = None, backend: Optional[str] = None,
                 named_parameters=None, err_callback=None, layerwise_times=None, sigma_scale: float = 2.5,
                 norm_clip: Optional[float] = None, writer=None, **_ignored):
        base = cfg if cfg is not None else OkTopkConfig()
        self.compressor: Compressor = resolve_compressor(compression, base)
        over = {"sparse": bool(sparse) and self.compressor.name != "none", "compressor": self.compressor.name}
        if cfg is None:
            over.update(density=density, sigma_scale=sigma_scale, norm_clip=norm_clip)
        self.cfg = base.replace(**over)
        if backend is not None:
            self.cfg = self.cfg.replace(backend=backend)
        self.compressor.cfg = self.cfg
        self.world = world if world is not None else _world()
        self.train_epoch = train_epoch
        self.err_callback = err_callback
        self.writer = writer
        self._dist_states: Dict[str, SparseState] = {}
        self._engines: Dict[str, "object"] = {}
        self._timers: Dict[str, list] = {}
        self._running = True
        self.profile_records: list = []
        self._profiling_norms: list = []
        self._prof_calls: Dict[str, int] = {}

    def get_current_density(self) -> float:
        dd = self.cfg.dynamic_densities
        if dd:
            return float(dd[min(self.train_epoch, len(dd) - 1)])
        return float(self.cfg.density)

    def _use_cuda(self, device: torch.device) -> bool:
        if device.type != "cuda" or self.cfg.backend == "dist":
            return False
        if not ext.available():
            if self.cfg.backend == "cuda" or device.type == "cuda":
                ext.require()
            return False
        return True

    def register_bucket(self, name: str, numel: int, device: torch.device) -> torch.Tensor:
        if self._use_cuda(device):
            from .gpu_engine import CudaBucketEngine
            eng = CudaBucketEngine(numel, self.cfg, self.world, name=name)
            self._engines[name] = eng
            return eng.grad
        self._dist_states[name] = SparseState(numel, self.world.size)
        return torch.zeros(numel, dtype=torch.float32, device=device)

    def reads_sources(self, name: str) -> bool:
        from ..utils import settings
        eng = self._engines.get(name)
        if eng is None or settings.PROFILING_GRAD or settings.PROFILING_NORM:
            return False
        return eng.reads_sources(self.compressor.name, self.get_current_density())

    def reduce_bucket(self, name: str, flat: torch.Tensor, stream=None, srcs=None, scale=None) -> torch.Tensor:
        skip = 0
        if scale is not None:
            eng = self._engines.get(name)
            if eng is not None:
                eng.unscale_check(scale.ptr, stream, srcs)
                skip = eng.verdict_ptr
            elif scale.check_host(flat, self.world):
                st = self._dist_states.get(name)
                if st is None:
                    st = self._dist_states[name] = SparseState(flat.numel(), self.world.size)
                st.counter += 1
                return flat
        density = self.get_current_density()
        from ..utils import settings
        if settings.PROFILING_GRAD and self.cfg.sparse:
            self._dump_grad(name, flat, density)
        if settings.PROFILING_NORM and self.cfg.sparse:
            return self._reduce_profiled(name, flat, stream, density, skip)
        if name in self._engines:
            out = self._engines[name].reduce(self.compressor.name, density, stream=stream, g=flat, srcs=srcs,
                                             skip=skip)
            if settings.PROFILING:
                self._profile_iteration(name)
            return out
        st = self._dist_states.get(name)
        if st is None:
            st = self._dist_states[name] = SparseState(flat.numel(), self.world.size)
        t0 = time.perf_counter()
        out = algorithms.sparse_allreduce(self.compressor.name, flat, st, self.cfg, self.world, density)
        self._timers.setdefault(name, []).append(time.perf_counter() - t0)
        return out

    def _profile_iteration(self, name: str) -> None:
        eng = self._engines[name]
        if _capturing():
            return
        st = eng.stats()
        c = self._prof_calls[name] = self._prof_calls.get(name, 0) + 1
        if self.world.rank == 0:
            print("counter: %d rank: %d mode: %s local topk elements: %d localtopk threshold: %.6g global topk elements: %d "
                  "globaltopk threshold: %.6g overflow: %d/%d redo: %d" % (
                      st["counter"], self.world.rank, st["mode"], st["local_count"], st["local_thr_used"], st["global_count"],
                      st["global_thr"], st["overflow_send"], st["overflow_gather"], st.get("redo", 0)), flush=True)
        if c % 50 == 0:
            self._print_profiling(name)

    def _print_profiling(self, name: Optional[str] = None) -> Dict[str, Dict[str, float]]:
        out = {}
        for nm, eng in self._engines.items():
            if name is not None and nm != name:
                continue
            recs = eng.trace()[-50:]
            if not recs:
                continue
            keys = [k for k in recs[0] if k.startswith("us_")]
            means = {k: sum(r[k] for r in recs) / len(recs) for k in keys}
            out[nm] = means
            if self.world.rank == 0:
                print("[rank:%d]%s[%d]: " % (self.world.rank, nm[:24], eng.n) +
                      ", ".join("%s %.1f" % (k[3:], v) for k, v in means.items()) + " (us, mean of %d calls)" % len(recs),
                      flush=True)
        return out

    def _dump_grad(self, name: str, flat: torch.Tensor, density: float) -> None:
        import os
        import numpy as np
        from ..compression import gen_threshold_from_normal_distribution
        from ..utils import settings
        if _capturing():
            return
        eng = self._engines.get(name)
        st = self._dist_states.get(name)
        counter = eng.host.counter if eng is not None else (st.counter if st is not None else 0)
        spec = os.environ.get("OKTOPK_GRAD_DUMP_ITERS", "3991-3995,12991-12995")
        hit = False
        for part in spec.split(","):
            lo, _, hi = part.partition("-")
            if lo.strip() and int(lo) <= counter <= int(hi or lo):
                hit = True
        res = eng.residual if eng is not None else (st.residual if st is not None else None)
        with torch.no_grad():
            acc = flat.detach().clone()
            if res is not None and res.numel() == acc.numel():
                acc += res
            k = max(int(acc.numel() * density), 1)
            gk_thr = float(gen_threshold_from_normal_distribution(1.0 - density, float(acc.mean()), float(acc.std()))[1])
            gk_topk = int((acc.abs() > gk_thr).sum())
            ok_thr = float(eng.stats()["local_thr"]) if eng is not None else float(getattr(st, "local_thr", 0.0))
        if self.world.rank == 0:
            print("counter: %d rank: %d ok_gk_local_thrds: [%.6g %.6g] gk_localtopk_value: %d" %
                  (counter, self.world.rank, ok_thr, gk_thr, gk_topk), flush=True)
            if hit:
                d = settings.PREFIX or "."
                os.makedirs(d, exist_ok=True)
                np.save(os.path.join(d, "localgrad%d_k%d.npy" % (counter, k)), acc.cpu().numpy())
                np.save(os.path.join(d, "localthrds%d_k%d.npy" % (counter, k)), np.asarray([ok_thr, gk_thr], dtype="float32"))

    def save_profiling_norms(self, directory: str, epoch: int) -> None:
        import os
        import numpy as np
        if not self._profiling_norms:
            return
        os.makedirs(directory, exist_ok=True)
        cols = list(zip(*self._profiling_norms))
        for nm, col in zip(("gtopknorm", "randknorm", "upbound", "xnorm", "densestd"), cols):
            np.save(os.path.join(directory, "%s-rank%d-epoch%d.npy" % (nm, self.world.rank, epoch)), np.asarray(col))
        self._profiling_norms = []

    def _reduce_profiled(self, name: str, flat: torch.Tensor, stream, density: float, skip: int = 0) -> torch.Tensor:
        from ..utils.metrics import sparsification_error
        eng = self._engines.get(name)
        st = self._dist_states.get(name)
        res = eng.residual if eng is not None else (st.residual if st is not None else None)
        with torch.no_grad():
            acc = flat.detach().clone()
            if res is not None and res.numel() == acc.numel():
                acc += res
            if self.world.size > 1:
                self.world.all_reduce_sum(acc)
            acc /= self.world.size
        if eng is not None:
            out = eng.reduce(self.compressor.name, density, stream=stream, g=flat, skip=skip)
            if flat.is_cuda:
                torch.cuda.synchronize()
        else:
            if st is None:
                st = self._dist_states[name] = SparseState(flat.numel(), self.world.size)
            out = algorithms.sparse_allreduce(self.compressor.name, flat, st, self.cfg, self.world, density)
        k = max(int(flat.numel() * density), 1)
        rec = sparsification_error(acc, out, k)
        rec["bucket"], rec["density"] = name, density
        self.profile_records.append(rec)
        with torch.no_grad():
            n = acc.numel()
            rk = torch.randperm(n, device=acc.device)[:k]
            randk = torch.zeros_like(acc)
            randk[rk] = acc[rk]
            xnorm = float(acc.norm())
            self._profiling_norms.append((float((acc - out).norm()), float((acc - randk).norm()),
                                          1.0 * (n - k) / n * xnorm, xnorm, float(acc.std())))
        if self.writer is not None and hasattr(self.writer, "add_scalars"):
            self.writer.add_scalars("profiling_norm/" + name, {k2: v for k2, v in rec.items() if isinstance(v, (int, float))},
                                    len(self.profile_records))
        return out

    def run(self, flat_tensor: torch.Tensor, name: str = "flat") -> torch.Tensor:
        assert flat_tensor.dim() == 1 and flat_tensor.dtype == torch.float32
        if name not in self._engines and name not in self._dist_states and self._use_cuda(flat_tensor.device):
            from .gpu_engine import CudaBucketEngine
            self._engines[name] = CudaBucketEngine(flat_tensor.numel(), self.cfg, self.world, name=name)
        return self.reduce_bucket(name, flat_tensor)

    def add_tensor(self, name: str, tensor: torch.Tensor):
        return name

    def get_result(self, name: str):
        raise RuntimeError("results are written in place into the gradient bucket")

    def stop(self) -> None:
        self._running = False

    def stats(self, name: Optional[str] = None) -> Dict:
        out = {}
        for nm, eng in self._engines.items():
            out[nm] = eng.stats()
        for nm, st in self._dist_states.items():
            out[nm] = {"counter": st.counter, "local_thr": st.local_thr, "global_thr": st.global_thr,
                       "local_count": st.last_local_count, "global_count": st.last_global_count,
                       "volume_elems": st.last_volume_elems, "mode": st.last_mode,
                       "edges": st.region_offsets + [st.numel]}
        return out if name is None else out[name]

    def enable_loss_scaling(self) -> None:
        for eng in self._engines.values():
            eng.enable_loss_scaling()

    def fault_ptr(self, name: str) -> int:
        eng = self._engines.get(name)
        return int(eng.fault_ptr) if eng is not None else 0

    def poll_faults(self) -> None:
        if not self._engines:
            return
        if _capturing():
            return
        for eng in self._engines.values():
            if eng.poll_fault():
                self.check_faults()
                return

    def trace(self) -> Dict[str, list]:
        return {nm: eng.trace() for nm, eng in self._engines.items()}

    def resync_hooks(self) -> list:
        return getattr(self, "_resync_hooks", [])

    def add_resync_hook(self, fn) -> None:
        self._resync_hooks = self.resync_hooks() + [fn]

    def check_faults(self) -> None:
        for eng in self._engines.values():
            try:
                eng.check_fault()
            except RuntimeError:
                if self.err_callback is None:
                    raise
                self.err_callback(self.world.size, self.world.rank)
                for e2 in self._engines.values():
                    e2.reset_sparse_state()
                    e2.clear_fault()
                for fn in self.resync_hooks():
                    fn()
                return

    def state_dict(self) -> Dict:
        sd = {"train_epoch": self.train_epoch, "buckets": {}}
        for nm, eng in self._engines.items():
            sd["buckets"][nm] = eng.state_dict()
        for nm, st in self._dist_states.items():
            sd["buckets"][nm] = st.state_dict()
        return sd

    def load_state_dict(self, sd: Dict) -> None:
        self.train_epoch = sd.get("train_epoch", 0)
        for nm, b in sd.get("buckets", {}).items():
            if nm in self._engines:
                self._engines[nm].load_state_dict(b)
            elif nm in self._dist_states:
                dev = self._dist_states[nm].residual.device if self._dist_states[nm].residual is not None else None
                self._dist_states[nm].load_state_dict(b, dev)
            else:
                import warnings
                warnings.warn("checkpoint holds sparse state for bucket %r which is not registered (yet): ignored" % nm)

    def close(self) -> None:
        for eng in self._engines.values():
            eng.close()
        self._engines.clear()


def dense_allreduce(tensor: torch.Tensor, world: Optional[World] = None) -> torch.Tensor:
    return algorithms.dense_allreduce(tensor, world or _world())


def topk_sparse_allreduce(tensor: torch.Tensor, density: float, world: Optional[World] = None, state=None):
    w = world or _world()
    st = state or SparseState(tensor.numel(), w.size)
    return algorithms.topka_allreduce(tensor, st, OkTopkConfig(density=density), w, density)


def gtopk_sparse_allreduce(tensor: torch.Tensor, density: float, world: Optional[World] = None, state=None):
    w = world or _world()
    st = state or SparseState(tensor.numel(), w.size)
    return algorithms.gtopk_allreduce(tensor, st, OkTopkConfig(density=density), w, density)
```

oktopk_b200/parallel/gpu_engine.py:

```python
from __future__ import annotations

from typing import Dict, List, Optional

import torch

from ..config import OkTopkConfig
from ..ops import ext
from .state import CallPlan, SparseState, plan_call, uniform_boundaries, offsets_of
from .symm import SymmBlock, make_symm_block
from .world import World

RES_OKTOPK, RES_LOCAL_GT, RES_LOCAL_GE = 0, 1, 2
GLB_THRESHOLD, GLB_EXACT_TOPK, GLB_ALL_NONZERO = 0, 1, 2
GS_THRESHOLD_REUSE, GS_GAUSSIAN, GS_EXACT_TOPK = 0, 1, 2

_CLASSIC_RESIDUAL = {"topkSA", "topkDSA", "gaussiankSA"}


def _round_up(x: int, m: int) -> int:
    return (int(x) + m - 1) // m * m


class PeerTimeoutError(RuntimeError):
    """A rank of the peer group did not reach a handshake in time (device-side failure detection)."""


class CudaBucketEngine:
    def __init__(self, numel: int, cfg: OkTopkConfig, world: World, name: str = "bucket",
                 max_density: Optional[float] = None, dense_grid: int = 0):
        self.C = ext.require()
        C = self.C
        self.cfg = cfg
        self.world = world
        self.name = name
        self.P = world.size
        self.rank = world.rank
        if self.P > C.MAXP:
            raise ValueError("world size %d exceeds OKT_MAXP=%d" % (self.P, C.MAXP))
        self.n = int(numel)
        self.device = torch.device("cuda", torch.cuda.current_device())
        dmax = max_density if max_density is not None else cfg.density
        if cfg.dynamic_densities:
            dmax = max(dmax, max(cfg.dynamic_densities))
        kmax = max(int(self.n * dmax), 1)
        self.kmax = kmax
        chunk = C.CHUNK
        nmax = _round_up(self.n, chunk)
        if cfg.slot_factor > 0:
            self.cap = min(nmax, _round_up(max(cfg.slot_factor * kmax / self.P, chunk), chunk)) + chunk
        else:
            self.cap = 0
        if cfg.gather_factor > 0 and cfg.compressor not in _CLASSIC_RESIDUAL:
            self.gcap = min(nmax, _round_up(max(cfg.gather_factor * kmax / self.P, 2 * kmax, chunk), chunk)) + chunk
        else:
            self.gcap = nmax + chunk
        info = C.layout_info(self.P, self.n, self.cap, self.gcap)
        self.layout = info
        self.grid = C.max_coop_grid(self.device.index)
        self.gather_grid = C.gather_max_coop_grid(self.device.index)
        self.tree_grid = C.gtopk_max_coop_grid(self.device.index)
        if cfg.comm_ctas > 0:
            self.grid = min(self.grid, cfg.comm_ctas)
            self.gather_grid = min(self.gather_grid, cfg.comm_ctas)
            self.tree_grid = min(self.tree_grid, cfg.comm_ctas)
        sms = torch.cuda.get_device_properties(self.device).multi_processor_count
        self.dense_grid = dense_grid or (min(sms, cfg.comm_ctas) if cfg.comm_ctas > 0 else sms)
        self.grad_bytes = _round_up(self.n * 4, 4096)
        self.comm_off = self.grad_bytes
        self.flags_off = self.comm_off + _round_up(info["total"], 4096)
        flags_bytes = 8 * 2 * self.dense_grid * C.MAXP
        self.block = make_symm_block(self.flags_off + _round_up(flags_bytes, 4096), world, cfg.nvls)
        self.grad = self.block.tensor(0, self.n, "float32")
        self.peer_comm = [p + self.comm_off for p in self.block.ptrs]
        self.peer_grad = [p for p in self.block.ptrs]
        self.peer_flags = [p + self.flags_off for p in self.block.ptrs]
        self.mc_grad = int(getattr(self.block, "mc_ptr", 0) or 0)
        self.state_ptr = C.dev_alloc_zero(C.state_bytes())
        self.fault_ptr = C.fault_ptr(self.state_ptr)
        self.host_flag, self.host_flag_dev = C.host_flag_alloc()
        self.dense_epoch_ptr = C.dev_alloc_zero(8 * self.dense_grid)
        self.scale_sync_ptr = 0
        self.residual = torch.zeros(self.n, dtype=torch.float32, device=self.device)
        if self.cap == 0:
            self.ccap = _round_up(self.n, 32)
        else:
            self.ccap = int(min(_round_up(self.n, 32), max(self.P * self.cap, 32 * kmax + chunk)))
        self.cand = torch.zeros(self.ccap, dtype=torch.int32, device=self.device)
        self._bitmap: Optional[torch.Tensor] = None
        self._sel: Optional[tuple] = None
        self.host = SparseState(self.n, self.P)
        self._write_edges(self.host.region_offsets + [self.n])
        self.last_mode = ""
        self._res_clean = False
        self._skip = 0

    def _stream(self, stream: Optional[torch.cuda.Stream]) -> int:
        return (stream or torch.cuda.current_stream()).cuda_stream

    def _write_edges(self, edges: List[int], local_thr: float = 0.0, global_thr: float = 0.0) -> None:
        self.C.write_state(self.state_ptr, float(local_thr), float(global_thr), [int(e) for e in edges],
                           torch.cuda.current_stream().cuda_stream)

    def k_now(self, density: Optional[float] = None) -> int:
        d = self.cfg.density if density is None else density
        return max(int(self.n * d), 1)

    def _plan(self, compressor: str, density: Optional[float]) -> CallPlan:
        return plan_call(self.cfg, compressor, self.host.counter, density, self.P)

    def reads_sources(self, compressor: str, density: Optional[float] = None) -> bool:
        return compressor == "oktopk" and self._plan(compressor, density).kind == "fused"

    def enable_loss_scaling(self) -> None:
        if not self.scale_sync_ptr:
            self.scale_sync_ptr = self.C.dev_alloc_zero(self.C.SCALE_SYNC_BYTES)

    @property
    def verdict_ptr(self) -> int:
        self.enable_loss_scaling()
        return self.scale_sync_ptr + self.C.VERDICT_OFFSET

    def unscale_check(self, loss_scale_ptr: int, stream: Optional[torch.cuda.Stream] = None,
                      srcs: Optional[tuple] = None) -> None:
        self.enable_loss_scaling()
        if srcs is not None and len(srcs[0]):
            ptrs, lens = list(srcs[0]), list(srcs[2])
        else:
            ptrs, lens = [self.grad.data_ptr()], [self.n]
        self.C.unscale_check(ptrs, lens, loss_scale_ptr, self.scale_sync_ptr, self.state_ptr, self.host_flag_dev,
                             self.peer_comm, self.layout["scale_mbox"], self.rank, float(self.cfg.peer_timeout_s),
                             self._stream(stream))

    def reduce(self, compressor: str, density: Optional[float] = None,
               stream: Optional[torch.cuda.Stream] = None, g: Optional[torch.Tensor] = None,
               srcs: Optional[tuple] = None, skip: int = 0) -> torch.Tensor:
        ext_g = g is not None and g.data_ptr() != self.grad.data_ptr()
        plan = self._plan(compressor, density)
        if srcs is not None and (ext_g or compressor != "oktopk" or plan.kind != "fused"):
            raise ValueError("gradient sources are only read by an Ok-Topk call on the engine's own bucket")
        s = self._stream(stream)
        self._skip = int(skip)
        out = g if ext_g else self.grad
        if plan.kind in ("dense", "dense_switch"):
            if ext_g:
                self.grad.copy_(g)
            if plan.kind == "dense_switch":
                if self._skip:
                    self.C.carry_residual(self.grad.data_ptr(), self.residual.data_ptr(), self.n, self._skip, s)
                elif not self._res_clean:
                    self.grad.add_(self.residual)
                    self.residual.zero_()
                    self._res_clean = True
            self._dense(s)
            if ext_g:
                g.copy_(self.grad)
            self.last_mode = "dense" if plan.kind == "dense" else "dense(auto)"
        else:
            self._res_clean = False
            if plan.kind == "fused":
                self._fused(compressor, plan, density, s, out, srcs)
            elif plan.kind == "gather":
                self._gather(compressor, plan, density, s, out)
            else:
                self._tree(compressor, density, s, out)
        self.host.counter += 1
        return out

    def _dense(self, s: int) -> None:
        if self.P == 1:
            return
        self.C.dense_run(self.peer_grad, self.peer_flags, self.dense_epoch_ptr, self.n, self.rank,
                         self.dense_grid, s, self.state_ptr, float(self.cfg.peer_timeout_s), self.mc_grad,
                         self.host_flag_dev, self._skip)

    def _fused(self, compressor: str, plan: CallPlan, density: Optional[float], s: int, g: torch.Tensor,
               srcs: Optional[tuple] = None) -> None:
        cfg = self.cfg
        k = self.k_now(density)
        o: Dict = {"pull_tma": 1 if cfg.pull_mode == "tma" else 0, "deterministic": int(cfg.deterministic),
                   "split_phases": 0 if cfg.fused else 1, "timeout_s": float(cfg.peer_timeout_s),
                   "cand": self.cand.data_ptr(), "ccap": self.ccap, "host_fault": self.host_flag_dev,
                   "max_redo": int(cfg.max_redo), "redo_factor": float(cfg.redo_factor),
                   "cand_mode": int(cfg.gselect_mode == "list" or (cfg.gselect_mode == "auto" and k * 200 <= self.n))}
        if compressor == "oktopk":
            o.update(
                exact_local=int(plan.exact_local),
                repartition=int(plan.repartition),
                residual_mode=RES_OKTOPK,
                global_mode=GLB_EXACT_TOPK if plan.exact_global else GLB_THRESHOLD,
                guard_loops=cfg.overselect_guard_loops,
                guard_limit=cfg.overselect_guard_num * k // cfg.overselect_guard_den,
                guard_factor=cfg.overselect_guard_factor,
                cap_limit=int(cfg.overselect_cap * k) if cfg.overselect_cap > 0 else 0,
                cap_rungs=int(cfg.overselect_cap_rungs), cap_factor=float(cfg.overselect_cap_factor),
                l_low_cnt=cfg.local_adapt_low * k, l_high_cnt=cfg.local_adapt_high * k, l_factor=cfg.local_adapt_factor,
                g_low_cnt=cfg.global_adapt_low * k, g_high_cnt=cfg.global_adapt_high * k,
                g_inc=cfg.global_adapt_inc, g_dec=cfg.global_adapt_dec,
            )
        else:
            o.update(exact_local=1, repartition=0,
                     residual_mode=RES_LOCAL_GT if compressor == "gaussiankSA" else RES_LOCAL_GE,
                     global_mode=GLB_ALL_NONZERO, guard_loops=0, guard_limit=0)
            if compressor in ("topkDSA", "topkSA") and g.data_ptr() == self.grad.data_ptr() and self.P > 1 \
                    and cfg.dsa_dense_fallback_frac > 0:
                o["dense_nnz_limit"] = max(int(self.n * cfg.dsa_dense_fallback_frac), 1)
                o["peer_g"] = self.peer_grad
        if srcs is not None:
            o["srcs"] = srcs
        if self._skip:
            o["skip"] = self._skip
        self.C.oktopk_run(g.data_ptr(), self.residual.data_ptr(), self.state_ptr, self.peer_comm, self.n,
                          self.rank, k, self.cap, self.gcap, o, self.grid, s)
        self.last_mode = compressor

    def _gather(self, compressor: str, plan: CallPlan, density: Optional[float], s: int, g: torch.Tensor) -> None:
        cfg = self.cfg
        d = cfg.density if density is None else density
        k = self.k_now(density)
        o: Dict = {"density": d, "pull_tma": 1 if cfg.pull_mode == "tma" else 0, "timeout_s": float(cfg.peer_timeout_s),
                   "host_fault": self.host_flag_dev}
        if cfg.norm_clip is not None and compressor in ("topkA", "topkA2"):
            o["clip_max_norm"] = float((1.0 / self.P) ** 0.5 * cfg.norm_clip)
        if compressor in ("topkA", "topkA2"):
            o["select_mode"] = GS_EXACT_TOPK
            if compressor == "topkA2":
                o.update(reselect=1, bitmap=self._bitmap_ptr(), cand=self.cand.data_ptr(), ccap=self.ccap)
        elif compressor == "topkAopt":
            o["select_mode"] = GS_THRESHOLD_REUSE
            o["exact_now"] = int(plan.exact_local)
        else:
            o["select_mode"] = GS_GAUSSIAN
            o["gauss_mode"] = {"vgg": 0, "lstm": 1, "bert": 2}[cfg.gaussian_mode]
            o["gauss_loops"] = cfg.gaussian_loops
            o["gauss_factor"] = cfg.gaussian_factor
        if self._skip:
            o["skip"] = self._skip
        self.C.gather_run(g.data_ptr(), self.residual.data_ptr(), self.state_ptr, self.peer_comm, self.n,
                          self.rank, k, self.cap, self.gcap, o, self.gather_grid, s)
        self.last_mode = compressor

    def _bitmap_ptr(self) -> int:
        if self._bitmap is None:
            self._bitmap = torch.zeros((self.n + 31) // 32 + 32, dtype=torch.int32, device=self.device)
        return self._bitmap.data_ptr()

    def _tree(self, compressor: str, density: Optional[float], s: int, g: torch.Tensor) -> None:
        cfg = self.cfg
        k = self.k_now(density)
        if self._sel is None:
            selcap = int(min(_round_up(self.n, 32), 2 * self.kmax + self.C.CHUNK))
            self._sel = (torch.zeros(selcap, dtype=torch.int32, device=self.device),
                         torch.zeros(selcap, dtype=torch.float32, device=self.device), selcap)
        o: Dict = {"pull_tma": 1 if cfg.pull_mode == "tma" else 0, "timeout_s": float(cfg.peer_timeout_s),
                   "host_fault": self.host_flag_dev, "bitmap": self._bitmap_ptr(), "cand": self.cand.data_ptr(),
                   "ccap": self.ccap, "sel_idx": self._sel[0].data_ptr(), "sel_val": self._sel[1].data_ptr(),
                   "selcap": self._sel[2]}
        if cfg.norm_clip is not None:
            o["clip_max_norm"] = float((1.0 / self.P) ** 0.5 * cfg.norm_clip)
        if self._skip:
            o["skip"] = self._skip
        self.C.gtopk_run(g.data_ptr(), self.residual.data_ptr(), self.state_ptr, self.peer_comm, self.n,
                         self.rank, k, self.cap, self.gcap, o, self.tree_grid, s)
        self.last_mode = compressor

    def stats(self) -> Dict:
        d = self.C.read_state(self.state_ptr, self.P, torch.cuda.current_stream().cuda_stream)
        d["counter"] = self.host.counter
        d["mode"] = self.last_mode
        d["cap"], d["gcap"], d["grid"] = self.cap, self.gcap, self.grid
        d["lossless"] = self.cap == 0
        d["nvls"] = bool(self.mc_grad)
        d["volume_elems"] = 2 * (d["recv_total"] + d["gather_total"])
        return d

    def trace(self) -> List[Dict]:
        recs = list(self.C.read_trace(self.state_ptr, torch.cuda.current_stream().cuda_stream))
        recs.sort(key=lambda r: r["epoch"])
        return recs

    def poll_fault(self) -> int:
        return int(self.C.host_flag_read(self.host_flag))

    def check_fault(self) -> None:
        code = int(self.stats().get("fault", 0))
        if code:
            names = {1: "reduce-scatter mailbox", 2: "allgather mailbox", 3: "region-cut mailbox", 4: "dense barrier",
                     5: "gTopk tree mailbox", 6: "dense-fallback done flags",
                     7: "loss-scale verdict mailbox"}
            raise PeerTimeoutError("bucket %s: peer wait timed out in the %s (fault %d, timeout %.1fs)"
                                   % (self.name, names.get(code, "?"), code, self.cfg.peer_timeout_s))

    def clear_fault(self) -> None:
        self.C.clear_fault(self.state_ptr, torch.cuda.current_stream().cuda_stream)
        self.C.host_flag_clear(self.host_flag)

    def reset_sparse_state(self) -> None:
        self.residual.zero_()
        self.grad.zero_()
        self.host.counter = self.cfg.warmup_iters if self.host.counter >= self.cfg.warmup_iters else self.host.counter
        self._write_edges(offsets_of(uniform_boundaries(self.n, self.P)) + [self.n], 0.0, 0.0)

    def state_dict(self) -> Dict:
        d = self.stats()
        return {"numel": self.n, "world": self.P, "counter": self.host.counter, "local_thr": d["local_thr"],
                "global_thr": d["global_thr"], "boundaries": [d["edges"][i + 1] - d["edges"][i] for i in range(self.P)],
                "region_offsets": d["edges"][:-1], "residual": self.residual.detach().cpu().clone()}

    def load_state_dict(self, sd: Dict) -> None:
        assert sd["numel"] == self.n
        self.host.counter = int(sd["counter"])
        if sd.get("residual") is not None:
            self.residual.copy_(sd["residual"].to(self.device))
            self._res_clean = False
        if sd["world"] == self.P:
            edges = list(sd["region_offsets"]) + [self.n]
        else:
            edges = offsets_of(uniform_boundaries(self.n, self.P)) + [self.n]
        self._write_edges(edges, sd["local_thr"], sd["global_thr"])

    def close(self) -> None:
        if getattr(self, "_closed", False):
            return
        self._closed = True
        self.block.close()
        try:
            self.C.host_flag_free(self.host_flag)
        except Exception:
            pass
        self.host_flag = 0
        for attr in ("state_ptr", "dense_epoch_ptr", "scale_sync_ptr"):
            ptr = getattr(self, attr, 0)
            if ptr:
                try:
                    self.C.dev_free(ptr)
                except Exception:
                    pass
                setattr(self, attr, 0)
```

Measured before the change: 13820.

## Pack Ok-Topk bucket segments early while backward pass still produces gradients

Adds an early-pack path. Once enough parameters in a bucket have finished their gradients, a small segment kernel runs the residual-accumulate and threshold-pack stage for those ranges, and the final fused launch then only packs the remaining ranges. The pack loop is factored into a reusable templated pack_stream that works over a tile map of arbitrary ranges. The aim is to overlap selection work with backward compute and shorten the tail after the last gradient arrives. In exchange it adds extra launches, planner bookkeeping and competition for SMs with backward kernels.

```diff
diff --git a/oktopk_b200/config.py b/oktopk_b200/config.py
--- a/oktopk_b200/config.py
+++ b/oktopk_b200/config.py
@@ -61,6 +61,9 @@
     comm_ctas: int = 0
     pull_mode: str = "tma"
     overlap: bool = True
+    early_pack: bool = True
+    early_pack_frac: float = 0.85
+    early_pack_ctas: int = 32
     gselect_mode: str = "auto"
     peer_timeout_s: float = 60.0
 
diff --git a/oktopk_b200/csrc/bindings.cpp b/oktopk_b200/csrc/bindings.cpp
--- a/oktopk_b200/csrc/bindings.cpp
+++ b/oktopk_b200/csrc/bindings.cpp
@@ -336,6 +336,29 @@
         p.src_len[0] = n;
         p.nsrc = 1;
         p.zero_g = 1;
+    }
+    if (o.contains("pack_ranges")) {
+        auto rs = o["pack_ranges"].cast<std::vector<std::pair<long long, long long>>>();
+        if (rs.size() > (size_t)kPackRangeMax) throw std::runtime_error("oktopk_run: more pack ranges than kPackRangeMax");
+        long long end = 0;
+        for (size_t i = 0; i < rs.size(); ++i) {
+            const long long lo = rs[i].first, hi = rs[i].second;
+            if (lo < end || hi < lo || (lo & 3) || (hi & 3) || hi > ((long long)n & ~3LL))
+                throw std::runtime_error("oktopk_run: pack ranges must be ordered, disjoint, at multiples of 4 elements, "
+                                         "inside the bucket's whole vectors");
+            p.pk_lo[i] = (int)(lo >> 2);
+            p.pk_hi[i] = (int)(hi >> 2);
+            end = hi;
+        }
+        p.pk_mode = 1;
+        p.pk_nr = (int)rs.size();
+        if (geti("segment", 0)) {
+            if (rs.empty() || p.zero_g || p.L.cap > 0 || p.residual_mode != RES_OKTOPK)
+                throw std::runtime_error("oktopk_run: a segment launch takes ranges of an Ok-Topk bucket read from its "
+                                         "sources in the lossless layout");
+            ck(launch_oktopk_segment(p, geti("seg_ctas", 32), S_(stream)), "oktopk segment launch");
+            return;
+        }
     }
     if (geti("split_phases", 0)) {
         for (int ph = p.phase_begin; ph < p.phase_end; ++ph) {
@@ -748,5 +771,6 @@
     m.attr("TRACE_LEN") = kTraceLen;
     m.attr("LAND_MAX") = kLandMax;
     m.attr("SRC_SEG_MAX") = kSrcSegMax;
+    m.attr("PACK_RANGE_MAX") = kPackRangeMax;
     m.attr("CHUNK") = kChunk;
 }
diff --git a/oktopk_b200/csrc/oktopk.cu b/oktopk_b200/csrc/oktopk.cu
--- a/oktopk_b200/csrc/oktopk.cu
+++ b/oktopk_b200/csrc/oktopk.cu
@@ -36,6 +36,239 @@
     if (r + 1 < len) out.y = src[1];
     if (r + 2 < len) out.z = src[2];
     return out;
+}
+
+__device__ __forceinline__ void load_src_table(const OktParams& p, SrcSeg* s_src, int* s_tail_v, int* s_tail_q, int* s_ntail) {
+    const int tid = threadIdx.x, lane = tid & 31, warp = tid >> 5;
+    const int nsrc = p.nsrc, n4 = p.n >> 2;
+    for (int q = tid; q < nsrc; q += blockDim.x) s_src[q] = SrcSeg{p.src[q], p.src_off[q], p.src_len[q]};
+    if (warp == 0) {
+        int cnt = 0;
+        for (int q0 = 0; q0 < nsrc; q0 += 32) {
+            const int q = q0 + lane;
+            const int end = q < nsrc ? p.src_off[q] + p.src_len[q] : 0;
+            const bool part = q < nsrc && (end & 3) != 0 && (end >> 2) < n4;
+            const unsigned m = __ballot_sync(0xffffffffu, part);
+            if (part) { const int t = cnt + __popc(m & ((1u << lane) - 1u)); s_tail_v[t] = end >> 2; s_tail_q[t] = q; }
+            cnt += __popc(m);
+        }
+        if (lane == 0) *s_ntail = cnt;
+    }
+    __syncthreads();
+}
+
+struct TileMap { const int* lo; const int* hi; const int* first; int nr; };
+
+__device__ __forceinline__ TileMap tile_map_build(int nr, const int* lo_in, const int* hi_in, int* lo, int* hi, int* first) {
+    if (threadIdx.x == 0) {
+        int t = 0;
+        for (int r = 0; r < nr; ++r) {
+            lo[r] = lo_in[r]; hi[r] = hi_in[r]; first[r] = t;
+            t += (hi[r] - lo[r] + kTileV - 1) / kTileV;
+        }
+        first[nr] = t;
+    }
+    __syncthreads();
+    return TileMap{lo, hi, first, nr};
+}
+
+__device__ __forceinline__ void tile_at(const TileMap& m, int t, int* base, int* end) {
+    int r = 0;
+    while (t >= m.first[r + 1]) ++r;
+    *base = m.lo[r] + (t - m.first[r]) * kTileV;
+    *end = min(*base + kTileV, m.hi[r]);
+}
+
+struct PackRing { float4* r; float4* g; uint64_t* full; uint64_t* empty; };
+struct PackSrc { const SrcSeg* seg; int nseg; const int* tail_v; const int* tail_q; int ntail; };
+struct PackSel {
+    float thr; LadderCfg lc; const float* lthr; int* lcnt;
+    const int* edges; const int* soff; int* sidx; float* sval; int P;
+};
+
+template <int STAGES>
+__device__ __forceinline__ int pack_stream(const OktParams& p, const TileMap& tm, const PackRing& ring, int ring_it,
+                                           bool res_only, bool clear_g, const PackSrc& src, const PackSel& sel,
+                                           int& dropped) {
+    OktState* st = p.st;
+    const int tid = threadIdx.x, lane = tid & 31, warp = tid >> 5;
+    const int n = p.n;
+    float4* g4 = reinterpret_cast<float4*>(p.g);
+    float4* r4 = reinterpret_cast<float4*>(p.res);
+    const int ntiles = tm.first[tm.nr];
+    const int G = gridDim.x;
+    const int nmine = (ntiles > (int)blockIdx.x) ? (ntiles - (int)blockIdx.x + G - 1) / G : 0;
+    const SrcSeg* s_src = src.seg;
+    const int nsrc = src.nseg;
+    const float thr_sel = sel.thr;
+    const LadderCfg& lc = sel.lc;
+
+    auto arm = [&](int j) {
+        int base, end;
+        tile_at(tm, blockIdx.x + j * G, &base, &end);
+        const int stg = (ring_it + j) % STAGES;
+        const uint32_t bytes = (uint32_t)(end - base) * 16u;
+        fence_proxy_async_all();
+        mbar_expect_tx(&ring.full[stg], res_only ? bytes : 2u * bytes);
+        tma_load_1d(ring.r + stg * kTileV, r4 + (size_t)base, bytes, &ring.full[stg]);
+        if (res_only) return;
+        float4* dst = ring.g + stg * kTileV;
+        const int e0 = base * 4, e1 = e0 + (int)(bytes >> 2);
+        int lo = 0, hi = nsrc;
+        while (lo < hi) {
+            const int mid = (lo + hi) >> 1;
+            if (s_src[mid].off + (s_src[mid].len & ~3) <= e0) lo = mid + 1; else hi = mid;
+        }
+        int q = lo, e = e0;
+        while (e < e1) {
+            if (q < nsrc && s_src[q].off <= e) {
+                const int stop = min(e1, s_src[q].off + (s_src[q].len & ~3));
+                if (stop > e) {
+                    tma_load_1d(dst + ((e - e0) >> 2), s_src[q].src + (e - s_src[q].off), (uint32_t)(stop - e) * 4u,
+                                &ring.full[stg]);
+                    e = stop;
+                }
+                ++q;
+            } else {
+                const int stop = q < nsrc ? min(e1, s_src[q].off) : e1;
+                tma_load_1d(dst + ((e - e0) >> 2), p.g + e, (uint32_t)(stop - e) * 4u, &ring.full[stg]);
+                e = stop;
+            }
+        }
+    };
+    if (tid == 0)
+        for (int j = 0; j < min(nmine, STAGES - 1); ++j) {
+            const int q = ring_it + j;
+            if (q >= STAGES) mbar_wait(&ring.empty[q % STAGES], (uint32_t)(q / STAGES - 1) & 1u);
+            arm(j);
+        }
+    for (int j = 0; j < nmine; ++j) {
+        if (tid == 0 && j + STAGES - 1 < nmine) {
+            const int q = ring_it + j + STAGES - 1;
+            if (q >= STAGES) mbar_wait(&ring.empty[q % STAGES], (uint32_t)(q / STAGES - 1) & 1u);
+            arm(j + STAGES - 1);
+        }
+        const int qj = ring_it + j;
+        const int stg = qj % STAGES;
+        mbar_wait(&ring.full[stg], (uint32_t)(qj / STAGES) & 1u);
+        int base, tend;
+        tile_at(tm, blockIdx.x + j * G, &base, &tend);
+        float4 a[kPackTile];
+        bool in[kPackTile];
+#pragma unroll
+        for (int u = 0; u < kPackTile; ++u) {
+            const int v = base + u * kThreads + tid;
+            in[u] = v < tend;
+            a[u] = make_float4(0.f, 0.f, 0.f, 0.f);
+            if (in[u]) {
+                a[u] = ring.r[stg * kTileV + u * kThreads + tid];
+                if (!res_only) {
+                    float4 gq = ring.g[stg * kTileV + u * kThreads + tid];
+                    for (int t = 0; t < src.ntail; ++t)
+                        if (src.tail_v[t] == v) {
+                            const SrcSeg sg = s_src[src.tail_q[t]];
+                            const float* sp = sg.src + (sg.len & ~3);
+                            const int c = sg.len & 3;
+                            gq.x = sp[0];
+                            if (c > 1) gq.y = sp[1];
+                            if (c > 2) gq.z = sp[2];
+                        }
+                    a[u].x += gq.x; a[u].y += gq.y; a[u].z += gq.z; a[u].w += gq.w;
+                    st_stream_f4(r4 + v, a[u]);
+                }
+                if (clear_g) st_stream_f4(g4 + v, make_float4(0.f, 0.f, 0.f, 0.f));
+            }
+        }
+        __syncwarp();
+        if (lane == 0) mbar_arrive(&ring.empty[stg]);
+        unsigned msk[kPackTile * 4];
+        unsigned mybits = 0u;
+        int tot = 0;
+#pragma unroll
+        for (int u = 0; u < kPackTile; ++u) {
+            const float xs[4] = {a[u].x, a[u].y, a[u].z, a[u].w};
+#pragma unroll
+            for (int c = 0; c < 4; ++c) {
+                const bool pred = in[u] && fabsf(xs[c]) > thr_sel;
+                if (p.residual_mode == RES_LOCAL_GE && in[u] && xs[c] != 0.f && fabsf(xs[c]) == thr_sel &&
+                    atomicAdd(&st->tie_cursor, 1) < (int)__ldcg(&st->sel_krem))
+                    p.res[4 * (base + u * kThreads + tid) + c] = 0.f;
+                const unsigned m = __ballot_sync(0xffffffffu, pred);
+                msk[u * 4 + c] = m;
+                tot += __popc(m);
+                if (pred) mybits |= 1u << (u * 4 + c);
+            }
+        }
+        if (tot == 0) continue;
+        if (lc.n_total > 1) {
+#pragma unroll
+            for (int u = 0; u < kPackTile; ++u) {
+                const float xs[4] = {a[u].x, a[u].y, a[u].z, a[u].w};
+#pragma unroll
+                for (int c = 0; c < 4; ++c)
+                    if (mybits & (1u << (u * 4 + c)))
+                        atomicAdd(&sel.lcnt[ladder_rung(sel.lthr, lc.n_total, fabsf(xs[c]))], 1);
+            }
+        } else if (lane == 0) {
+            atomicAdd(&sel.lcnt[0], tot);
+        }
+        const int e_first = 4 * (base + (warp << 5));
+        const int e_last = min(n - 1, 4 * (base + (kPackTile - 1) * kThreads + (warp << 5) + 31) + 3);
+        const int dlo = region_of(sel.edges, sel.P, e_first), dhi = region_of(sel.edges, sel.P, e_last);
+        for (int d = dlo; d <= dhi; ++d) {
+            unsigned md[kPackTile * 4];
+            unsigned mine = mybits;
+            int cnt = 0;
+            if (dlo == dhi) {
+#pragma unroll
+                for (int q = 0; q < kPackTile * 4; ++q) { md[q] = msk[q]; cnt += __popc(md[q]); }
+            } else {
+                const int lo_d = sel.edges[d], hi_d = sel.edges[d + 1];
+                mine = 0u;
+#pragma unroll
+                for (int u = 0; u < kPackTile; ++u) {
+#pragma unroll
+                    for (int c = 0; c < 4; ++c) {
+                        const int i = 4 * (base + u * kThreads + tid) + c;
+                        const bool pd = ((mybits >> (u * 4 + c)) & 1u) && i >= lo_d && i < hi_d;
+                        md[u * 4 + c] = __ballot_sync(0xffffffffu, pd);
+                        cnt += __popc(md[u * 4 + c]);
+                        if (pd) mine |= 1u << (u * 4 + c);
+                    }
+                }
+            }
+            if (cnt == 0) continue;
+            int run = 0;
+            if (lane == 0) run = atomicAdd(&st->send_cursor[d], cnt);
+            run = __shfl_sync(0xffffffffu, run, 0);
+            const int scap_d = sel.soff[d + 1] - sel.soff[d];
+            int* sidx = sel.sidx + sel.soff[d];
+            float* sval = sel.sval + sel.soff[d];
+            const int off_d = sel.edges[d];
+            const unsigned lt = (1u << lane) - 1u;
+#pragma unroll
+            for (int u = 0; u < kPackTile; ++u) {
+                const float xs[4] = {a[u].x, a[u].y, a[u].z, a[u].w};
+#pragma unroll
+                for (int c = 0; c < 4; ++c) {
+                    const int q = u * 4 + c;
+                    if ((mine >> q) & 1u) {
+                        const int pos = run + __popc(md[q] & lt);
+                        const int i = 4 * (base + u * kThreads + tid) + c;
+                        if (pos < scap_d) {
+                            sidx[pos] = i - off_d;
+                            sval[pos] = xs[c];
+                            if (p.residual_mode != RES_OKTOPK) p.res[i] = 0.f;
+                        } else {
+                            dropped++;
+                        }
+                    }
+                    run += __popc(md[q]);
+                }
+            }
+        }
+    }
+    return nmine;
 }
 
 __global__ void __launch_bounds__(kThreads, kCtasPerSm) oktopk_fused_kernel(const OktParams p) {
@@ -58,6 +291,7 @@
     __shared__ SrcSeg s_src[kSrcSegMax];
     __shared__ int s_tail_v[kSrcSegMax], s_tail_q[kSrcSegMax];
     __shared__ int s_ntail;
+    __shared__ int s_rlo[kPackRangeMax], s_rhi[kPackRangeMax], s_rfirst[kPackRangeMax + 1];
     extern __shared__ __align__(128) float4 dyn_pk[];
 
     if (verdict_set(p.skip)) return;
@@ -89,23 +323,13 @@
     }
     const int n4 = n >> 2;
     const int nsrc = p.nsrc;
-    for (int q = tid; q < nsrc; q += kThreads) s_src[q] = SrcSeg{p.src[q], p.src_off[q], p.src_len[q]};
-    if (warp == 0) {
-        int cnt = 0;
-        for (int q0 = 0; q0 < nsrc; q0 += 32) {
-            const int q = q0 + lane;
-            const int end = q < nsrc ? p.src_off[q] + p.src_len[q] : 0;
-            const bool part = q < nsrc && (end & 3) != 0 && (end >> 2) < n4;
-            const unsigned m = __ballot_sync(0xffffffffu, part);
-            if (part) { const int t = cnt + __popc(m & ((1u << lane) - 1u)); s_tail_v[t] = end >> 2; s_tail_q[t] = q; }
-            cnt += __popc(m);
-        }
-        if (lane == 0) s_ntail = cnt;
-    }
-    __syncthreads();
+    load_src_table(p, s_src, s_tail_v, s_tail_q, &s_ntail);
     const int ntail = s_ntail;
-
-    float4* g4 = reinterpret_cast<float4*>(p.g);
+    const int whole[2] = {0, n4};
+    const bool ranged = p.pk_mode && !two_pass;
+    const TileMap tmap = tile_map_build(ranged ? p.pk_nr : 1, ranged ? p.pk_lo : whole, ranged ? p.pk_hi : whole + 1,
+                                        s_rlo, s_rhi, s_rfirst);
+
     float4* r4 = reinterpret_cast<float4*>(p.res);
 
     if (p.phase_begin <= PH_LOCAL && PH_LOCAL < p.phase_end && two_pass) {
@@ -320,11 +544,7 @@
         int dropped = 0;
         if (blockIdx.x == 0 && tid == 0) { st->stat_global_count = 0; st->stat_recv_total = 0; st->stat_dense_fallback = 0; }
 
-        float4* pk_r = dyn_pk;
-        float4* pk_g = dyn_pk + kPackStages * kTileV;
-        const int ntiles = (n4 + kTileV - 1) / kTileV;
-        const int G = gridDim.x;
-        const int nmine = (ntiles > (int)blockIdx.x) ? (ntiles - (int)blockIdx.x + G - 1) / G : 0;
+        const PackRing ring{dyn_pk, dyn_pk + kPackStages * kTileV, s_pk_bar, s_pk_empty};
         int ring_it = 0;
 
         while (true) {
@@ -366,170 +586,9 @@
                 }
             };
 
-            auto arm = [&](int j) {
-                const int tile = blockIdx.x + j * G;
-                const int stg = (ring_it + j) % kPackStages;
-                const uint32_t bytes = (uint32_t)min(kTileV, n4 - tile * kTileV) * 16u;
-                fence_proxy_async_all();
-                mbar_expect_tx(&s_pk_bar[stg], res_only ? bytes : 2u * bytes);
-                tma_load_1d(pk_r + stg * kTileV, r4 + (size_t)tile * kTileV, bytes, &s_pk_bar[stg]);
-                if (res_only) return;
-                float4* dst = pk_g + stg * kTileV;
-                const int e0 = tile * kTileV * 4, e1 = e0 + (int)(bytes >> 2);
-                int lo = 0, hi = nsrc;
-                while (lo < hi) {
-                    const int mid = (lo + hi) >> 1;
-                    if (s_src[mid].off + (s_src[mid].len & ~3) <= e0) lo = mid + 1; else hi = mid;
-                }
-                int q = lo, e = e0;
-                while (e < e1) {
-                    if (q < nsrc && s_src[q].off <= e) {
-                        const int stop = min(e1, s_src[q].off + (s_src[q].len & ~3));
-                        if (stop > e) {
-                            tma_load_1d(dst + ((e - e0) >> 2), s_src[q].src + (e - s_src[q].off), (uint32_t)(stop - e) * 4u,
-                                        &s_pk_bar[stg]);
-                            e = stop;
-                        }
-                        ++q;
-                    } else {
-                        const int stop = q < nsrc ? min(e1, s_src[q].off) : e1;
-                        tma_load_1d(dst + ((e - e0) >> 2), p.g + e, (uint32_t)(stop - e) * 4u, &s_pk_bar[stg]);
-                        e = stop;
-                    }
-                }
-            };
-            if (tid == 0)
-                for (int j = 0; j < min(nmine, kPackStages - 1); ++j) {
-                    const int q = ring_it + j;
-                    if (q >= kPackStages) mbar_wait(&s_pk_empty[q % kPackStages], (uint32_t)(q / kPackStages - 1) & 1u);
-                    arm(j);
-                }
-            for (int j = 0; j < nmine; ++j) {
-                if (tid == 0 && j + kPackStages - 1 < nmine) {
-                    const int q = ring_it + j + kPackStages - 1;
-                    if (q >= kPackStages) mbar_wait(&s_pk_empty[q % kPackStages], (uint32_t)(q / kPackStages - 1) & 1u);
-                    arm(j + kPackStages - 1);
-                }
-                const int qj = ring_it + j;
-                const int stg = qj % kPackStages;
-                mbar_wait(&s_pk_bar[stg], (uint32_t)(qj / kPackStages) & 1u);
-                const int base = (blockIdx.x + j * G) * kTileV;
-                float4 a[kPackTile];
-                bool in[kPackTile];
-#pragma unroll
-                for (int u = 0; u < kPackTile; ++u) {
-                    const int v = base + u * kThreads + tid;
-                    in[u] = v < n4;
-                    a[u] = make_float4(0.f, 0.f, 0.f, 0.f);
-                    if (in[u]) {
-                        a[u] = pk_r[stg * kTileV + u * kThreads + tid];
-                        if (!res_only) {
-                            float4 gq = pk_g[stg * kTileV + u * kThreads + tid];
-                            for (int t = 0; t < ntail; ++t)
-                                if (s_tail_v[t] == v) {
-                                    const SrcSeg sg = s_src[s_tail_q[t]];
-                                    const float* src = sg.src + (sg.len & ~3);
-                                    const int c = sg.len & 3;
-                                    gq.x = src[0];
-                                    if (c > 1) gq.y = src[1];
-                                    if (c > 2) gq.z = src[2];
-                                }
-                            a[u].x += gq.x; a[u].y += gq.y; a[u].z += gq.z; a[u].w += gq.w;
-                            st_stream_f4(r4 + v, a[u]);
-                        }
-                        if (attempt == 0 && p.zero_g) st_stream_f4(g4 + v, make_float4(0.f, 0.f, 0.f, 0.f));
-                    }
-                }
-                __syncwarp();
-                if (lane == 0) mbar_arrive(&s_pk_empty[stg]);
-                unsigned msk[kPackTile * 4];
-                unsigned mybits = 0u;
-                int tot = 0;
-#pragma unroll
-                for (int u = 0; u < kPackTile; ++u) {
-                    const float xs[4] = {a[u].x, a[u].y, a[u].z, a[u].w};
-#pragma unroll
-                    for (int c = 0; c < 4; ++c) {
-                        const bool pred = in[u] && fabsf(xs[c]) > thr_sel;
-                        if (p.residual_mode == RES_LOCAL_GE && in[u] && xs[c] != 0.f && fabsf(xs[c]) == thr_sel &&
-                            atomicAdd(&st->tie_cursor, 1) < (int)__ldcg(&st->sel_krem))
-                            p.res[4 * (base + u * kThreads + tid) + c] = 0.f;
-                        const unsigned m = __ballot_sync(0xffffffffu, pred);
-                        msk[u * 4 + c] = m;
-                        tot += __popc(m);
-                        if (pred) mybits |= 1u << (u * 4 + c);
-                    }
-                }
-                if (tot == 0) continue;
-                if (lc.n_total > 1) {
-#pragma unroll
-                    for (int u = 0; u < kPackTile; ++u) {
-                        const float xs[4] = {a[u].x, a[u].y, a[u].z, a[u].w};
-#pragma unroll
-                        for (int c = 0; c < 4; ++c)
-                            if (mybits & (1u << (u * 4 + c)))
-                                atomicAdd(&s_lcnt[ladder_rung(s_lthr, lc.n_total, fabsf(xs[c]))], 1);
-                    }
-                } else if (lane == 0) {
-                    atomicAdd(&s_lcnt[0], tot);
-                }
-                const int e_first = 4 * (base + (warp << 5));
-                const int e_last = min(n - 1, 4 * (base + (kPackTile - 1) * kThreads + (warp << 5) + 31) + 3);
-                const int dlo = region_of(s_edges, P, e_first), dhi = region_of(s_edges, P, e_last);
-                for (int d = dlo; d <= dhi; ++d) {
-                    unsigned md[kPackTile * 4];
-                    unsigned mine = mybits;
-                    int cnt = 0;
-                    if (dlo == dhi) {
-#pragma unroll
-                        for (int q = 0; q < kPackTile * 4; ++q) { md[q] = msk[q]; cnt += __popc(md[q]); }
-                    } else {
-                        const int lo_d = s_edges[d], hi_d = s_edges[d + 1];
-                        mine = 0u;
-#pragma unroll
-                        for (int u = 0; u < kPackTile; ++u) {
-#pragma unroll
-                            for (int c = 0; c < 4; ++c) {
-                                const int i = 4 * (base + u * kThreads + tid) + c;
-                                const bool pd = ((mybits >> (u * 4 + c)) & 1u) && i >= lo_d && i < hi_d;
-                                md[u * 4 + c] = __ballot_sync(0xffffffffu, pd);
-                                cnt += __popc(md[u * 4 + c]);
-                                if (pd) mine |= 1u << (u * 4 + c);
-                            }
-                        }
-                    }
-                    if (cnt == 0) continue;
-                    int run = 0;
-                    if (lane == 0) run = atomicAdd(&st->send_cursor[d], cnt);
-                    run = __shfl_sync(0xffffffffu, run, 0);
-                    const int scap_d = s_soff[d + 1] - s_soff[d];
-                    int* sidx = my_sidx + s_soff[d];
-                    float* sval = my_sval + s_soff[d];
-                    const int off_d = s_edges[d];
-                    const unsigned lt = (1u << lane) - 1u;
-#pragma unroll
-                    for (int u = 0; u < kPackTile; ++u) {
-                        const float xs[4] = {a[u].x, a[u].y, a[u].z, a[u].w};
-#pragma unroll
-                        for (int c = 0; c < 4; ++c) {
-                            const int q = u * 4 + c;
-                            if ((mine >> q) & 1u) {
-                                const int pos = run + __popc(md[q] & lt);
-                                const int i = 4 * (base + u * kThreads + tid) + c;
-                                if (pos < scap_d) {
-                                    sidx[pos] = i - off_d;
-                                    sval[pos] = xs[c];
-                                    if (p.residual_mode != RES_OKTOPK) p.res[i] = 0.f;
-                                } else {
-                                    dropped++;
-                                }
-                            }
-                            run += __popc(md[q]);
-                        }
-                    }
-                }
-            }
-            ring_it += nmine;
+            const PackSrc src{s_src, nsrc, s_tail_v, s_tail_q, ntail};
+            const PackSel sel{thr_sel, lc, s_lthr, s_lcnt, s_edges, s_soff, my_sidx, my_sval, P};
+            ring_it += pack_stream<kPackStages>(p, tmap, ring, ring_it, res_only, attempt == 0 && p.zero_g, src, sel, dropped);
             if (blockIdx.x == 0 && warp == 0 && (n & 3)) {
                 int i = n4 * 4 + lane;
                 bool in = i < n;
@@ -866,6 +925,43 @@
     }
 }
 
+__global__ void __launch_bounds__(kThreads) oktopk_segment_kernel(const OktParams p) {
+    __shared__ int s_edges[OKT_MAXP + 1];
+    __shared__ int s_soff[OKT_MAXP + 1];
+    __shared__ float s_lthr[kGuardMax];
+    __shared__ int s_lcnt[kGuardMax];
+    __shared__ __align__(8) uint64_t s_full[kSegStages];
+    __shared__ __align__(8) uint64_t s_empty[kSegStages];
+    __shared__ SrcSeg s_src[kSrcSegMax];
+    __shared__ int s_tail_v[kSrcSegMax], s_tail_q[kSrcSegMax];
+    __shared__ int s_ntail;
+    __shared__ int s_rlo[kPackRangeMax], s_rhi[kPackRangeMax], s_rfirst[kPackRangeMax + 1];
+    extern __shared__ __align__(128) float4 dyn_seg[];
+
+    if (verdict_set(p.skip)) return;
+    OktState* st = p.st;
+    const float thr = st->local_thr;
+    if (thr == 0.f) return;
+    const int tid = threadIdx.x, P = p.P;
+    if (tid == 0) {
+        for (int q = 0; q < kSegStages; ++q) { mbar_init(&s_full[q], 1); mbar_init(&s_empty[q], kWarps); }
+        mbar_fence_init();
+    }
+    if (tid <= P) s_edges[tid] = st->edges[tid];
+    load_src_table(p, s_src, s_tail_v, s_tail_q, &s_ntail);
+    if (tid <= P) s_soff[tid] = (tid < P) ? slot_off(p.L, s_edges, tid) : slot_off(p.L, s_edges, P);
+    const TileMap tmap = tile_map_build(p.pk_nr, p.pk_lo, p.pk_hi, s_rlo, s_rhi, s_rfirst);
+    const LadderCfg lc = ladder_cfg(p, true);
+    ladder_build(s_lthr, s_lcnt, lc, thr);
+    char* me = p.peers[p.rank];
+    const PackRing ring{dyn_seg, dyn_seg + kSegStages * kTileV, s_full, s_empty};
+    const PackSrc src{s_src, p.nsrc, s_tail_v, s_tail_q, s_ntail};
+    const PackSel sel{thr, lc, s_lthr, s_lcnt, s_edges, s_soff, send_idx_base(me, p.L), send_val_base(me, p.L), P};
+    int dropped = 0;
+    pack_stream<kSegStages>(p, tmap, ring, 0, false, false, src, sel, dropped);
+    ladder_flush(st, s_lcnt);
+}
+
 __global__ void __launch_bounds__(kThreads, 2) kth_abs_kernel(const float* x, int n, int k, OktState* st, float* out) {
     __shared__ uint32_t s_hist[kHistBins];
     __shared__ int s_w[kWarps + 1];
@@ -899,6 +995,24 @@
     return cudaLaunchCooperativeKernel((void*)oktopk_fused_kernel, dim3(grid), dim3(kThreads), args, kPackSmemBytes, stream);
 }
 
+cudaError_t launch_oktopk_segment(const OktParams& p, int max_ctas, cudaStream_t stream) {
+    constexpr int kSmem = kSegStages * 2 * kTileV * 16;
+    static bool attr_set[64] = {false};
+    int dev = 0;
+    cudaGetDevice(&dev);
+    if (dev >= 0 && dev < 64 && !attr_set[dev]) {
+        cudaError_t e = cudaFuncSetAttribute(oktopk_segment_kernel, cudaFuncAttributeMaxDynamicSharedMemorySize, kSmem);
+        if (e != cudaSuccess) return e;
+        attr_set[dev] = true;
+    }
+    int ntiles = 0;
+    for (int r = 0; r < p.pk_nr; ++r) ntiles += (p.pk_hi[r] - p.pk_lo[r] + kTileV - 1) / kTileV;
+    if (ntiles <= 0) return cudaSuccess;
+    const int grid = std::min((ntiles + kSegTiles - 1) / kSegTiles, std::max(max_ctas, 1));
+    oktopk_segment_kernel<<<grid, kThreads, kSmem, stream>>>(p);
+    return cudaGetLastError();
+}
+
 cudaError_t launch_kth_abs(const float* x, int n, int k, OktState* st, float* out_thr, int grid, cudaStream_t stream) {
     void* args[] = {(void*)&x, (void*)&n, (void*)&k, (void*)&st, (void*)&out_thr};
     return cudaLaunchCooperativeKernel((void*)kth_abs_kernel, dim3(grid), dim3(kThreads), args, 0, stream);
diff --git a/oktopk_b200/csrc/oktopk.cuh b/oktopk_b200/csrc/oktopk.cuh
--- a/oktopk_b200/csrc/oktopk.cuh
+++ b/oktopk_b200/csrc/oktopk.cuh
@@ -133,6 +133,9 @@
 enum GlobalMode : int { GLB_THRESHOLD = 0, GLB_EXACT_TOPK = 1, GLB_ALL_NONZERO = 2 };
 
 constexpr int kSrcSegMax = 160;
+constexpr int kPackRangeMax = 32;
+constexpr int kSegStages = 2;
+constexpr int kSegTiles = 4;
 
 struct OktParams {
     float* g;
@@ -170,6 +173,9 @@
     int src_off[kSrcSegMax];
     int src_len[kSrcSegMax];
     const float* src[kSrcSegMax];
+    int pk_mode, pk_nr;
+    int pk_lo[kPackRangeMax];
+    int pk_hi[kPackRangeMax];
 };
 static_assert(sizeof(OktParams) <= 4096, "OktParams must fit the 4 KB kernel-parameter limit");
 
@@ -234,6 +240,7 @@
 
 int okt_max_coop_grid(int device);
 cudaError_t launch_oktopk(const OktParams& p, int grid, cudaStream_t stream);
+cudaError_t launch_oktopk_segment(const OktParams& p, int max_ctas, cudaStream_t stream);
 cudaError_t launch_gather_scheme(const GatherParams& p, int grid, cudaStream_t stream);
 cudaError_t launch_gtopk(const TreeParams& p, int grid, cudaStream_t stream);
 int gtopk_max_coop_grid(int device);
diff --git a/oktopk_b200/optimizer.py b/oktopk_b200/optimizer.py
--- a/oktopk_b200/optimizer.py
+++ b/oktopk_b200/optimizer.py
@@ -11,6 +11,7 @@
 from .ops import ext
 from .parallel.allreducer import AllReducer
 from .parallel.buckets import Bucket, attach, build_buckets
+from .parallel.early_pack import PackPlanner
 from .parallel.world import World, world as _world
 
 
@@ -129,6 +130,16 @@
                 self._update = None
         self._direct = (self._land and self._update is not None and allreducer.compressor.name == "oktopk"
                         and all(b.flat_param is not None for b in self._buckets))
+        self._packs = {}
+        self._pos_in_bucket = {p: i for b in self._buckets for i, p in enumerate(b.params)}
+        if self._direct and self._use_streams:
+            for b in self._buckets:
+                if len(b.params) <= ext.require().SRC_SEG_MAX:
+                    self._packs[b.index] = PackPlanner(b.offsets, b.numel,
+                                                       math.ceil(self._cfg.early_pack_frac * b.numel),
+                                                       ext.require().PACK_RANGE_MAX)
+            for b in self._buckets:
+                b.packing = None
         if self._use_streams:
             self._comm_stream = torch.cuda.Stream(priority=-1)
         allreducer.add_resync_hook(self._resync_replicas)
@@ -201,7 +212,37 @@
             b.pending -= 1
             if b.pending == 0:
                 self._launch_ready()
+            elif b.index in self._packs:
+                self._pack_early(b, p)
         return hook
+
+    def _pack_early(self, b: Bucket, p) -> None:
+        if b.packing is None:
+            b.packing = (self._direct and not self.momentum_correction and self._ls is None
+                         and self._allreducer.reads_sources(b.name) and self._allreducer.packs_early(b.name))
+        if not b.packing:
+            return
+        planner = self._packs[b.index]
+        ranges = planner.ready(self._pos_in_bucket[p])
+        if ranges is None:
+            return
+        ptrs, offs, lens = [], [], []
+        for q, o, v in sorted(zip(b.params, b.offsets, b.grad_views), key=lambda t: t[1]):
+            g = q.grad
+            if not any(lo <= o < hi for lo, hi in ranges) or g is None or g.numel() == 0:
+                continue
+            if (g.data_ptr() == v.data_ptr() or g.dtype != torch.float32 or not g.is_cuda or g.stride() != v.stride()
+                    or g.data_ptr() % 16):
+                raise RuntimeError("early pack: the gradient of %s cannot be read in place; set "
+                                   "OkTopkConfig.early_pack=False" % self._parameter_names.get(q, "?"))
+            ptrs.append(g.data_ptr())
+            offs.append(o)
+            lens.append(g.numel())
+        ev = torch.cuda.Event()
+        ev.record(torch.cuda.current_stream())
+        self._comm_stream.wait_event(ev)
+        with torch.cuda.stream(self._comm_stream):
+            self._allreducer.pack_segment(b.name, ranges, (ptrs, offs, lens), stream=self._comm_stream)
 
     def _launch_ready(self) -> None:
         while self._next_launch < len(self._buckets) and self._buckets[self._next_launch].pending <= 0:
@@ -255,6 +296,12 @@
         srcs = None
         if self._direct and not self.momentum_correction and self._allreducer.reads_sources(b.name):
             srcs = self._source_table(b)
+        rest = None
+        if b.index in self._packs and self._packs[b.index].segments:
+            if srcs is None:
+                raise RuntimeError("early pack: bucket %s was partly packed from its gradients but its last call cannot "
+                                   "read them in place; set OkTopkConfig.early_pack=False" % b.name)
+            rest = self._packs[b.index].rest()
         if srcs is None and self._land:
             self._land_bucket(b)
         if self.momentum_correction:
@@ -264,7 +311,8 @@
             ev.record(torch.cuda.current_stream())
             self._comm_stream.wait_event(ev)
             with torch.cuda.stream(self._comm_stream):
-                self._allreducer.reduce_bucket(b.name, b.grad, stream=self._comm_stream, srcs=srcs, scale=self._ls)
+                self._allreducer.reduce_bucket(b.name, b.grad, stream=self._comm_stream, srcs=srcs, scale=self._ls,
+                                               pack_ranges=rest)
                 b.event.record(self._comm_stream)
         else:
             self._allreducer.reduce_bucket(b.name, b.grad, srcs=srcs, scale=self._ls)
@@ -336,6 +384,9 @@
         for b in self._buckets:
             b.pending = len(b.params)
             b.launched = False
+            if b.index in self._packs:
+                self._packs[b.index].reset()
+                b.packing = None
         self._next_launch = 0
         self._synced = False
         self._allreducer.poll_faults()
diff --git a/oktopk_b200/parallel/allreducer.py b/oktopk_b200/parallel/allreducer.py
--- a/oktopk_b200/parallel/allreducer.py
+++ b/oktopk_b200/parallel/allreducer.py
@@ -74,7 +74,18 @@
             return False
         return eng.reads_sources(self.compressor.name, self.get_current_density())
 
-    def reduce_bucket(self, name: str, flat: torch.Tensor, stream=None, srcs=None, scale=None) -> torch.Tensor:
+    def packs_early(self, name: str) -> bool:
+        from ..utils import settings
+        eng = self._engines.get(name)
+        if eng is None or settings.PROFILING or settings.PROFILING_GRAD or settings.PROFILING_NORM:
+            return False
+        return eng.packs_early(self.compressor.name, self.get_current_density())
+
+    def pack_segment(self, name: str, ranges, srcs, stream=None) -> None:
+        self._engines[name].pack_segment(self.compressor.name, ranges, srcs, self.get_current_density(), stream)
+
+    def reduce_bucket(self, name: str, flat: torch.Tensor, stream=None, srcs=None, scale=None,
+                      pack_ranges=None) -> torch.Tensor:
         skip = 0
         if scale is not None:
             eng = self._engines.get(name)
@@ -95,7 +106,7 @@
             return self._reduce_profiled(name, flat, stream, density, skip)
         if name in self._engines:
             out = self._engines[name].reduce(self.compressor.name, density, stream=stream, g=flat, srcs=srcs,
-                                             skip=skip)
+                                             skip=skip, pack_ranges=pack_ranges)
             if settings.PROFILING:
                 self._profile_iteration(name)
             return out
diff --git a/oktopk_b200/parallel/early_pack.py b/oktopk_b200/parallel/early_pack.py
--- /dev/null
+++ b/oktopk_b200/parallel/early_pack.py
@@ -0,0 +1,73 @@
+from __future__ import annotations
+
+from typing import List, Optional, Sequence, Tuple
+
+Range = Tuple[int, int]
+
+
+class PackPlanner:
+
+    def __init__(self, offsets: Sequence[int], n: int, min_elems: int, max_ranges: int):
+        order = sorted(range(len(offsets)), key=lambda i: offsets[i])
+        if any(int(offsets[i]) % 4 for i in order):
+            raise ValueError("parameter offsets must be multiples of 4 elements")
+        self.n, self.min_elems, self.max_ranges = int(n), max(int(min_elems), 1), int(max_ranges)
+        top = 4 * (self.n // 4)
+        self._pos = {i: k for k, i in enumerate(order)}
+        starts = [min(int(offsets[i]), top) for i in order]
+        ends = starts[1:] + [top]
+        if starts:
+            starts[0] = 0
+        self._span = list(zip(starts, ends))
+        self.reset()
+
+    def reset(self) -> None:
+        self._state = [0] * len(self._span)
+        self._pending = 0
+        self._segments: List[List[Range]] = []
+        self._packed_runs = 0
+
+    @property
+    def segments(self) -> List[List[Range]]:
+        return [list(s) for s in self._segments]
+
+    def _runs(self, want: int) -> List[Range]:
+        out: List[Range] = []
+        for (a, b), s in zip(self._span, self._state):
+            if s != want or a == b:
+                continue
+            if out and out[-1][1] == a:
+                out[-1] = (out[-1][0], b)
+            else:
+                out.append((a, b))
+        return out
+
+    def ready(self, i: int) -> Optional[List[Range]]:
+        k = self._pos[i]
+        if self._state[k]:
+            return None
+        self._state[k] = 1
+        self._pending += self._span[k][1] - self._span[k][0]
+        if self._pending < self.min_elems:
+            return None
+        runs = self._runs(1)
+        if self._packed_runs + len(runs) > self.max_ranges - 1:
+            return None
+        for q, s in enumerate(self._state):
+            if s == 1:
+                self._state[q] = 2
+        self._pending = 0
+        self._packed_runs += len(runs)
+        self._segments.append(runs)
+        return runs
+
+    def rest(self) -> List[Range]:
+        out: List[Range] = []
+        for (a, b), s in zip(self._span, self._state):
+            if s == 2 or a == b:
+                continue
+            if out and out[-1][1] == a:
+                out[-1] = (out[-1][0], b)
+            else:
+                out.append((a, b))
+        return out
diff --git a/oktopk_b200/parallel/gpu_engine.py b/oktopk_b200/parallel/gpu_engine.py
--- a/oktopk_b200/parallel/gpu_engine.py
+++ b/oktopk_b200/parallel/gpu_engine.py
@@ -1,5 +1,6 @@
 from __future__ import annotations
 
+import os
 from typing import Dict, List, Optional
 
 import torch
@@ -93,6 +94,7 @@
         self.last_mode = ""
         self._res_clean = False
         self._skip = 0
+        self.early_pack = bool(cfg.early_pack) and os.environ.get("OKTOPK_EARLY_PACK", "1") != "0"
 
     def _stream(self, stream: Optional[torch.cuda.Stream]) -> int:
         return (stream or torch.cuda.current_stream()).cuda_stream
@@ -110,6 +112,17 @@
 
     def reads_sources(self, compressor: str, density: Optional[float] = None) -> bool:
         return compressor == "oktopk" and self._plan(compressor, density).kind == "fused"
+
+    def packs_early(self, compressor: str, density: Optional[float] = None) -> bool:
+        if not (self.early_pack and compressor == "oktopk" and self.cap == 0 and self.cfg.fused):
+            return False
+        plan = self._plan(compressor, density)
+        return plan.kind == "fused" and not plan.exact_local and not plan.repartition
+
+    def pack_segment(self, compressor: str, ranges, srcs: tuple, density: Optional[float] = None,
+                     stream: Optional[torch.cuda.Stream] = None) -> None:
+        self._fused(compressor, self._plan(compressor, density), density, self._stream(stream), self.grad, srcs,
+                    pack_ranges=list(ranges), segment=True)
 
     def enable_loss_scaling(self) -> None:
         if not self.scale_sync_ptr:
@@ -133,7 +146,7 @@
 
     def reduce(self, compressor: str, density: Optional[float] = None,
                stream: Optional[torch.cuda.Stream] = None, g: Optional[torch.Tensor] = None,
-               srcs: Optional[tuple] = None, skip: int = 0) -> torch.Tensor:
+               srcs: Optional[tuple] = None, skip: int = 0, pack_ranges: Optional[list] = None) -> torch.Tensor:
         ext_g = g is not None and g.data_ptr() != self.grad.data_ptr()
         plan = self._plan(compressor, density)
         if srcs is not None and (ext_g or compressor != "oktopk" or plan.kind != "fused"):
@@ -158,7 +171,7 @@
         else:
             self._res_clean = False
             if plan.kind == "fused":
-                self._fused(compressor, plan, density, s, out, srcs)
+                self._fused(compressor, plan, density, s, out, srcs, pack_ranges)
             elif plan.kind == "gather":
                 self._gather(compressor, plan, density, s, out)
             else:
@@ -174,7 +187,7 @@
                          self.host_flag_dev, self._skip)
 
     def _fused(self, compressor: str, plan: CallPlan, density: Optional[float], s: int, g: torch.Tensor,
-               srcs: Optional[tuple] = None) -> None:
+               srcs: Optional[tuple] = None, pack_ranges: Optional[list] = None, segment: bool = False) -> None:
         cfg = self.cfg
         k = self.k_now(density)
         o: Dict = {"pull_tma": 1 if cfg.pull_mode == "tma" else 0, "deterministic": int(cfg.deterministic),
@@ -209,9 +222,14 @@
             o["srcs"] = srcs
         if self._skip:
             o["skip"] = self._skip
+        if pack_ranges is not None:
+            o["pack_ranges"] = [(int(a), int(b)) for a, b in pack_ranges]
+            o["segment"] = int(segment)
+            o["seg_ctas"] = int(cfg.early_pack_ctas)
         self.C.oktopk_run(g.data_ptr(), self.residual.data_ptr(), self.state_ptr, self.peer_comm, self.n,
                           self.rank, k, self.cap, self.gcap, o, self.grid, s)
-        self.last_mode = compressor
+        if not segment:
+            self.last_mode = compressor
 
     def _gather(self, compressor: str, plan: CallPlan, density: Optional[float], s: int, g: torch.Tensor) -> None:
         cfg = self.cfg
```

New measurement: 14360 (median of 6 runs). 3.9% higher.
